# GATB/leon

Hardware: AMD Instinct MI355X
Metric: compressed input MB/s (DNA encode path) (higher is better)
Workload: dtype u64

## Files before the change

### leon_amd/csrc/capi.hip

```cpp
#include "../../include/leon_dna.h"
#include "kernels.h"
#include "host_rc.h"
#include "staging.h"
#include "host_blocks.h"

#include "prim.h"

#include <algorithm>
#include <atomic>
#include <chrono>
#include <cstdio>
#include <cstdlib>
#include <cstring>
#include <functional>
#include <mutex>
#include <string>
#include <thread>
#include <vector>

using namespace leon;

namespace {

thread_local std::string g_create_error;
}
namespace leon { void set_create_error(const std::string& msg) { g_create_error = msg; } }
namespace {

const bool g_trace_alloc = getenv("LEON_TRACE_ALLOC") != nullptr;

struct DevBuf {
    void* p = nullptr;
    size_t cap = 0;
    hipError_t ensure(size_t bytes) {
        if (bytes <= cap) return hipSuccess;
        auto t0 = std::chrono::steady_clock::now();
        if (p) { hipError_t e = hipFree(p); p = nullptr; cap = 0; if (e != hipSuccess) return e; }
        size_t want = bytes + bytes / 8 + 256;
        hipError_t e = hipMalloc(&p, want);
        if (e != hipSuccess) { (void)hipGetLastError(); leon_device_trim(); e = hipMalloc(&p, want); }
        if (e == hipSuccess) cap = want;
        if (g_trace_alloc) {
            const double ms = std::chrono::duration<double, std::milli>(std::chrono::steady_clock::now() - t0).count();
            if (ms >= 1.0) fprintf(stderr, "[leon alloc] %.1f MB in %.1f ms\n", want / 1e6, ms);
        }
        return e;
    }
    void release() { if (p) (void)hipFree(p); p = nullptr; cap = 0; }
    template <typename T> T* as() const { return (T*)p; }
};
struct TmpBuf : DevBuf {
    TmpBuf() = default;
    TmpBuf(const TmpBuf&) = delete;
    TmpBuf& operator=(const TmpBuf&) = delete;
    ~TmpBuf() { release(); }
};

uint64_t splitmix_rv(uint32_t idx) {
    uint64_t s = 0x4C454F4EULL + (uint64_t)(idx + 1) * 0x9E3779B97F4A7C15ULL;
    s = (s ^ (s >> 30)) * 0xBF58476D1CE4E5B9ULL;
    s = (s ^ (s >> 27)) * 0x94D049BB133111EBULL;
    return s ^ (s >> 31);
}
uint64_t hash_seed0() {
    const uint64_t r0 = 0xAAAAAAAA55555555ULL, r3 = 0xB5B5B5B54B4B4B4BULL;
    return r0 * r3;
}

__global__ void k_iota(uint32_t* v, uint64_t n) {
    for (uint64_t i = blockIdx.x * (uint64_t)blockDim.x + threadIdx.x; i < n; i += (uint64_t)gridDim.x * blockDim.x) v[i] = (uint32_t)i;
}

}

inline hipError_t spin_sync(hipStream_t s) {
    static const bool spin = [] { const char* e = getenv("LEON_SPIN_SYNC"); return !(e && e[0] == '0'); }();
    if (!spin) return hipStreamSynchronize(s);
    const auto t0 = std::chrono::steady_clock::now();
    for (uint32_t i = 0;; i++) {
        const hipError_t e = hipStreamQuery(s);
        if (e != hipErrorNotReady) return e;
        for (int k = 0; k < 32; k++) __builtin_ia32_pause();
        if ((i & 255) == 255 && std::chrono::steady_clock::now() - t0 > std::chrono::milliseconds(20)) break;
    }
    (void)hipGetLastError();
    return hipStreamSynchronize(s);
}

struct leon_dna_ctx {
    leon_dna_cfg cfg{};
    int device = 0;
    hipStream_t stream = nullptr;
    uint64_t* h_rb = nullptr;
    std::string err;
    uint8_t* d_bloom = nullptr;
    uint64_t bloom_nchar = 0;
    BloomDev B{};
    uint16_t* d_rv16 = nullptr;
    DictDev D{};
    uint64_t dict_cap = 0;
    uint64_t n_keys = 0;
    unsigned long long* d_nkeys = nullptr;
    uint64_t n_anchors = 0;
    DevBuf anchor_kmers;
    AnchorDictWorker* anchor_worker = nullptr;
    double anchor_wait_ms = 0;
    std::vector<uint8_t> dict_device_out;
    uint64_t next_read = 0, next_block = 0;
    uint32_t shard_rank = 0, shard_world = 1;
    uint32_t xch_mode = LEON_XCH_OFF;
    leon_exchange_fn xch_fn = nullptr; void* xch_user = nullptr;
    leon_gather_fn gather_fn = nullptr; void* gather_user = nullptr;
    DevBuf xch_slot, xch_off, xch_evoff, xch_events, xch_send, xch_split, xch_res;
    DevBuf resolve_trace;
    DevBuf round_hist;
    DevBuf wcache;
    DevBuf chain_cnt, chain_own, chain_ins, chain_rows, chain_ent, chain_trace, chain_dep, chain_xdep, chain_om, chain_late;
    std::vector<hipEvent_t> chain_ev;
    DevBuf hb_recs[2], hb_recoff, hb_state;
    uint64_t* h_recs = nullptr; size_t h_recs_cap = 0;
    hipStream_t copy_stream = nullptr;
    std::vector<hipEvent_t> hb_ev;
    std::vector<HostBlockCoder> hb_coders;
    uint64_t* h_anchor[2] = {nullptr, nullptr}; size_t h_anchor_cap = 0;
    bool partial_seen = false, finished = false;
    uint64_t hdr_next_read = 0, hdr_next_block = 0;
    bool hdr_partial_seen = false;
    DevBuf hdr_first;
    const uint64_t* walk_keys = nullptr;
    uint32_t fbits_log2 = FBITS_LOG2_DEFAULT;
    bool poisoned = false;
    DevBuf in_bases, in_off, slot_off, packed, nmask, rlen, ncount;
    DevBuf status, hit_pos, hit_slot, cand_pos, cand_slot, anchor_pos, anchor_addr, flags, sort_key, ins_flag, rank;
    DevBuf ulist0, ulist1, counters, cub_tmp, sort_key2, perm, perm2, events, prev, sym_off, syms;
    DevBuf blk_begin, out_off, out_size, rc_out, rc_scratch, dst_off, payload, errflag, nerr, wbits, fbits, pbits;
    void* h_payload = nullptr; size_t h_payload_cap = 0;
    uint64_t last_n = 0, last_bases = 0;
    const void* last_d_bases = nullptr; const void* last_d_off = nullptr;
    DevBuf dc_cache;
    DevBuf dc_out, dc_pay, dc_len, dc_pool, dc_scr;
    PathCache dc_pc{};
    uint64_t dc_bloom_fp = 0;
    bool dc_filled = false;
    leon_dna_stats stats{};
    hipEvent_t ev[12]{};
    std::vector<hipEvent_t> pack_ev;
};

namespace {

int fail(leon_dna_ctx* c, int code, const std::string& msg) {
    if (c) c->err = msg; else g_create_error = msg;
    return code;
}
#define HIPCHK(c, call)                                                                         \
    do {                                                                                        \
        hipError_t e_ = (call);                                                                 \
        if (e_ != hipSuccess)                                                                   \
            return fail((c), LEON_E_HIP, std::string(#call) + ": " + hipGetErrorString(e_));    \
    } while (0)

void dict_free(DictDev& D) {
    if (D.slots) (void)hipFree(D.slots);
    if (D.tent && D.tstride == 1) (void)hipFree(D.tent);
    if (D.addr) (void)hipFree(D.addr);
    D = DictDev{};
}
int dict_alloc(leon_dna_ctx* c, DictDev& D, uint64_t cap) {
    const uint32_t W = kmer_words(c->cfg.kmer_size);
    D = DictDev{};
    hipError_t e = hipMalloc((void**)&D.slots, cap * 16 * W);
    if (e == hipSuccess && W == 1) { D.tstride = 1; e = hipMalloc((void**)&D.tent, cap * 8); }
    if (e == hipSuccess) e = hipMalloc((void**)&D.addr, cap * 4);
    if (e != hipSuccess) {
        dict_free(D);
        return fail(c, LEON_E_HIP, std::string("anchor dictionary allocation: ") + hipGetErrorString(e));
    }
    if (W == 2) { D.tent = D.slots + 3; D.tstride = 4; }
    D.mask = cap - 1;
    D.n_keys = c->d_nkeys;
    D.wbits = c->wbits.as<uint32_t>();
    D.fbits = c->fbits.as<uint32_t>();
    D.pbits = c->pbits.as<uint32_t>();
    D.fwshift = 32 - (c->fbits_log2 - 6);
    minimizer_geometry(c->cfg.kmer_size, D.mm_m, D.mm_P, D.mm_c);
    D.err = c->errflag.as<int>() + 2;
    launch_dict_init(c->stream, D, cap, W);
    return LEON_OK;
}
int dict_reserve(leon_dna_ctx* c, uint64_t keys) {
    uint64_t need = 1024;
    while (need < 4 * keys) need <<= 1;
    if (need <= c->dict_cap) return LEON_OK;
    if (need > (1ull << 32)) return fail(c, LEON_E_OVERFLOW, "anchor dictionary would exceed 2^32 slots");
    DictDev nd{};
    HIPCHK(c, hipMemsetAsync(c->d_nkeys, 0, 8, c->stream));
    int rc = dict_alloc(c, nd, need);
    if (rc) return rc;
    if (c->dict_cap) {
        launch_dict_rehash(c->stream, c->D, c->dict_cap, nd, c->cfg.kmer_size);
        HIPCHK(c, hipStreamSynchronize(c->stream));
        dict_free(c->D);
    }
    c->D = nd;
    c->dict_cap = need;
    return LEON_OK;
}

ReadsDev reads_view(leon_dna_ctx* c, const uint64_t* d_off, uint64_t n) {
    ReadsDev R{};
    R.packed = c->packed.as<uint32_t>(); R.nmask = c->nmask.as<uint32_t>(); R.slot_off = c->slot_off.as<uint64_t>();
    R.base_off = d_off; R.len = c->rlen.as<uint32_t>(); R.n_count = c->ncount.as<uint32_t>();
    R.n = n; R.k = c->cfg.kmer_size;
    return R;
}

struct Upload {
    static constexpr uint64_t kPiece = kStagePiece;
    std::atomic<uint64_t> bytes_done{0};
    std::atomic<int> failed{0};
    std::atomic<int> cancel{0};
    std::atomic<uint64_t> next_piece{0};
    std::vector<std::atomic<uint8_t>> piece_done;
    std::mutex mu;
    uint64_t prefix = 0, n_bytes = 0;
    std::vector<std::thread> th;
    explicit Upload(uint64_t bytes) : piece_done((bytes + kPiece - 1) / kPiece), n_bytes(bytes) { for (auto& f : piece_done) f.store(0); }
    void publish(uint64_t piece) {
        piece_done[piece].store(1, std::memory_order_release);
        std::lock_guard<std::mutex> g(mu);
        while (prefix < piece_done.size() && piece_done[prefix].load(std::memory_order_acquire)) prefix++;
        bytes_done.store(std::min(n_bytes, prefix * kPiece), std::memory_order_release);
    }
    ~Upload() { for (auto& t : th) if (t.joinable()) t.join(); }
};
constexpr uint32_t kRbHostChainsErr = 500;
int ensure_cub(leon_dna_ctx* c, size_t bytes) { HIPCHK(c, c->cub_tmp.ensure(bytes)); return LEON_OK; }
template <typename F> int run_prim(leon_dna_ctx* c, F&& call) {
    size_t bytes = 0;
    HIPCHK(c, call(nullptr, bytes));
    if (int rc = ensure_cub(c, bytes)) return rc;
    HIPCHK(c, call(c->cub_tmp.p, bytes));
    return LEON_OK;
}

int ensure_pack_bufs(leon_dna_ctx* c, uint64_t n, uint64_t n_slots) {
    HIPCHK(c, c->packed.ensure((n_slots * 2 + 16) * 4)); HIPCHK(c, c->nmask.ensure((n_slots + 4) * 4));
    HIPCHK(c, c->rlen.ensure(n * 4)); HIPCHK(c, c->ncount.ensure(n * 4));
    return LEON_OK;
}
int ensure_resolve_bufs(leon_dna_ctx* c, uint64_t n, uint64_t W) {
    HIPCHK(c, c->status.ensure(n));
    HIPCHK(c, c->hit_pos.ensure(n * 4)); HIPCHK(c, c->hit_slot.ensure(n * 4));
    HIPCHK(c, c->cand_pos.ensure(n * 4)); HIPCHK(c, c->cand_slot.ensure(n * 4));
    HIPCHK(c, c->anchor_pos.ensure(n * 4)); HIPCHK(c, c->anchor_addr.ensure(n * 4));
    HIPCHK(c, c->flags.ensure(n)); HIPCHK(c, c->sort_key.ensure(n * 8));
    HIPCHK(c, c->ins_flag.ensure(W * 4)); HIPCHK(c, c->rank.ensure(W * 4));
    HIPCHK(c, c->ulist0.ensure(W * 4)); HIPCHK(c, c->ulist1.ensure(W * 4));
    return LEON_OK;
}
int ensure_block_bufs(leon_dna_ctx* c, uint64_t nbl) {
// ... 224 lines not shown
        launch_rc_encode(s, c->syms.as<uint8_t>(), c->blk_begin.as<uint64_t>(), nbl, c->rc_out.as<uint8_t>(), c->out_off.as<uint64_t>(),
                         c->out_size.as<uint64_t>(), c->rc_scratch.as<uint32_t>(), c->errflag.as<int>(), max_block_syms, small_sizes, counts_apart);
        HIPCHK(c, hipGetLastError());
        HIPCHK(c, hipEventRecord(c->ev[7], s));
        int errflag = 0;
        HIPCHK(c, hipMemcpyAsync(out.sizes.data(), c->out_size.p, nbl * 8, hipMemcpyDeviceToHost, s));
        HIPCHK(c, hipMemcpyAsync(&errflag, c->errflag.p, 4, hipMemcpyDeviceToHost, s));
        HIPCHK(c, hipStreamSynchronize(s));
        if (errflag == 3) return fail(c, LEON_E_STATE, "a numeric value's byte count above 8 in the symbol stream (internal error)");
        if (errflag) return fail(c, LEON_E_OVERFLOW, errflag == 2 ? std::string("a ") + unit + " block has 2^32 symbols or more"
                                                                  : std::string("range coder output exceeded its 3 bytes/symbol bound"));
    }
    for (uint64_t b = 0; b < nbl; b++) out.dst[b + 1] = out.dst[b] + out.sizes[b];
    const uint64_t payload_bytes = out.payload_bytes = out.dst[nbl];
    if (!out.host_chains) {
        HIPCHK(c, c->payload.ensure(payload_bytes + 16));
        HIPCHK(c, hipMemcpyAsync(c->dst_off.p, out.dst.data(), (nbl + 1) * 8, hipMemcpyHostToDevice, s));
        launch_gather_payload(s, c->rc_out.as<uint8_t>(), c->out_off.as<uint64_t>(), c->dst_off.as<uint64_t>(), c->out_size.as<uint64_t>(),
                              nbl, c->payload.as<uint8_t>());
        if (int rc = ensure_host_payload(c, payload_bytes + 16, payload_bytes + payload_bytes / 4 + 4096)) return rc;
        HIPCHK(c, hipMemcpyAsync(c->h_payload, c->payload.p, payload_bytes, hipMemcpyDeviceToHost, s));
    }
    HIPCHK(c, hipEventRecord(c->ev[8], s));
    HIPCHK(c, hipStreamSynchronize(s));
    return LEON_OK;
}

int deliver_blocks(leon_dna_ctx* c, const CodedBlocks& out, const Share& sh, uint64_t n, uint64_t first_block, leon_block_sink sink, void* user) {
    const uint64_t rpb = c->cfg.reads_per_block;
    for (uint64_t b = 0; b < sh.nbl; b++) {
        const uint32_t nr = (uint32_t)std::min<uint64_t>(rpb, n - (sh.lb0 + b) * rpb);
        const uint8_t* pay = out.host_chains ? c->hb_coders[b].data() : (const uint8_t*)c->h_payload + out.dst[b];
        if (sink(user, first_block + sh.lb0 + b, pay, out.sizes[b], nr)) {
            c->poisoned = true;
            return fail(c, LEON_E_SINK, "block sink returned non-zero");
        }
    }
    return LEON_OK;
}
}

extern "C" {

int leon_dna_abi_version(void) { return LEON_DNA_ABI_VERSION; }

const char* leon_last_error(const leon_dna_ctx* ctx) { return ctx ? ctx->err.c_str() : g_create_error.c_str(); }

int leon_dna_ctx_create(const leon_dna_cfg* cfg, leon_dna_ctx** out) {
    if (!cfg || !out) return fail(nullptr, LEON_E_INVALID, "null argument");
    *out = nullptr;
    if (cfg->struct_size != sizeof(leon_dna_cfg)) return fail(nullptr, LEON_E_INVALID, "leon_dna_cfg.struct_size mismatch");
    if (cfg->kmer_size < 3 || cfg->kmer_size > 63)
        return fail(nullptr, LEON_E_INVALID, "kmer_size must be in 3..63 (one 64-bit word below 32, two words from 32 to 63)");
    if (cfg->reads_per_block == 0) return fail(nullptr, LEON_E_INVALID, "reads_per_block must be > 0");
    if (cfg->bloom_n_hash < 1 || cfg->bloom_n_hash > 10) return fail(nullptr, LEON_E_INVALID, "bloom_n_hash must be in 1..10");
    if (cfg->bloom_block_nbits < 4 || cfg->bloom_block_nbits > 16)
        return fail(nullptr, LEON_E_INVALID, "bloom_block_nbits must be in 4..16");
    {
        const uint64_t blk0 = 1ull << cfg->bloom_block_nbits;
        uint64_t tai0 = cfg->bloom_tai + 2 * blk0;
        if ((tai0 & (tai0 - 1)) == 0) tai0--;
        if (tai0 <= 2 * blk0 || cfg->bloom_tai > (1ull << 46)) return fail(nullptr, LEON_E_INVALID, "bloom_tai out of range (1 .. 2^46 bits)");
    }
    int ndev = 0;
    if (hipGetDeviceCount(&ndev) != hipSuccess || ndev == 0)
        return fail(nullptr, LEON_E_NO_DEVICE, "no HIP device: the DNA encode path has no CPU fallback");
    if (cfg->device_id < 0 || cfg->device_id >= ndev) return fail(nullptr, LEON_E_INVALID, "device_id out of range");
    leon_dna_ctx* c = new leon_dna_ctx();
    c->cfg = *cfg;
    c->cfg.random_values = nullptr;
    if (c->cfg.resolve_window == 0) c->cfg.resolve_window = 1ull << 21;
    c->device = cfg->device_id;
#define CREATE_CHK(call)                                                                                         \
    do {                                                                                                         \
        hipError_t e_ = (call);                                                                                  \
        if (e_ != hipSuccess) {                                                                                  \
            int r_ = fail(nullptr, LEON_E_HIP, std::string(#call) + ": " + hipGetErrorString(e_));               \
            leon_dna_ctx_destroy(c);                                                                             \
            return r_;                                                                                           \
        }                                                                                                        \
    } while (0)
    CREATE_CHK(hipSetDevice(c->device));
    CREATE_CHK(hipStreamCreateWithFlags(&c->stream, hipStreamNonBlocking));
    CREATE_CHK(hipHostMalloc((void**)&c->h_rb, 4096, hipHostMallocDefault));
    for (auto& e : c->ev) CREATE_CHK(hipEventCreate(&e));
    uint64_t blk = 1ull << cfg->bloom_block_nbits;
    uint64_t tai = cfg->bloom_tai + 2 * blk;
    c->bloom_nchar = 1 + tai / 8;
    if ((tai & (tai - 1)) == 0) tai--;
    uint64_t reduced = tai - 2 * blk;
    CREATE_CHK(hipMalloc((void**)&c->d_bloom, c->bloom_nchar + 16));
    CREATE_CHK(hipMemsetAsync(c->d_bloom, 0, c->bloom_nchar + 16, c->stream));
    uint16_t rv16[256];
    for (uint32_t i = 0; i < 256; i++) rv16[i] = (uint16_t)((cfg->random_values ? cfg->random_values[i] : splitmix_rv(i)) & 0xFFFF);
    CREATE_CHK(hipMalloc((void**)&c->d_rv16, sizeof(rv16)));
    CREATE_CHK(hipMemcpy(c->d_rv16, rv16, sizeof(rv16), hipMemcpyHostToDevice));
    uint32_t k = cfg->kmer_size;
    c->B.bits = c->d_bloom; c->B.reduced_tai = reduced; c->B.mod_magic = ~0ull / reduced; c->B.seed0 = hash_seed0();
    c->B.k = k; c->B.n_hash = cfg->bloom_n_hash; c->B.block_mask = (uint32_t)(blk - 1);
    CREATE_CHK(hipMalloc((void**)&c->d_nkeys, 8));
    CREATE_CHK(hipMemset(c->d_nkeys, 0, 8));
    CREATE_CHK(c->counters.ensure(64));
    CREATE_CHK(c->errflag.ensure(16));
    CREATE_CHK(hipMemsetAsync(c->errflag.p, 0, 16, c->stream));
    CREATE_CHK(c->wbits.ensure((1ull << WBITS_LOG2) / 8));
    CREATE_CHK(c->pbits.ensure((1ull << WBITS_LOG2) / 8));
    if (const char* e = getenv("LEON_FBITS_LOG2")) {
        const int v = atoi(e);
        if (v >= 12 && v <= (int)FBITS_LOG2_MAX) c->fbits_log2 = (uint32_t)v;
    }
    CREATE_CHK(c->fbits.ensure((1ull << c->fbits_log2) / 8));
    CREATE_CHK(hipMemsetAsync(c->fbits.p, 0, (1ull << c->fbits_log2) / 8, c->stream));
    CREATE_CHK(hipStreamSynchronize(c->stream));
#undef CREATE_CHK
    c->anchor_worker = new AnchorDictWorker(cfg->kmer_size);
    *out = c;
    return LEON_OK;
}

void leon_dna_ctx_destroy(leon_dna_ctx* c) {
    if (!c) return;
    delete c->anchor_worker;
    (void)hipSetDevice(c->device);
    if (c->stream) (void)hipStreamSynchronize(c->stream);
    dict_free(c->D);
    DevBuf* bufs[] = { &c->anchor_kmers, &c->in_bases, &c->in_off, &c->slot_off, &c->packed, &c->nmask, &c->rlen, &c->ncount,
                       &c->status, &c->hit_pos, &c->hit_slot, &c->cand_pos, &c->cand_slot, &c->anchor_pos, &c->anchor_addr,
                       &c->flags, &c->sort_key, &c->ins_flag, &c->rank, &c->ulist0, &c->ulist1, &c->counters, &c->cub_tmp,
                       &c->sort_key2, &c->perm, &c->perm2, &c->events, &c->prev, &c->sym_off, &c->syms, &c->blk_begin,
                       &c->out_off, &c->out_size, &c->rc_out, &c->rc_scratch, &c->dst_off, &c->payload, &c->errflag, &c->nerr, &c->wbits, &c->fbits, &c->pbits, &c->hdr_first, &c->dc_cache, &c->dc_out, &c->dc_pay, &c->dc_len, &c->dc_pool, &c->dc_scr,
                       &c->xch_slot, &c->xch_off, &c->xch_evoff, &c->xch_events, &c->xch_send, &c->xch_split, &c->xch_res, &c->round_hist, &c->resolve_trace, &c->hb_recs[0], &c->hb_recs[1], &c->hb_recoff, &c->hb_state };
    for (DevBuf* b : bufs) b->release();
    if (c->d_bloom) (void)hipFree(c->d_bloom);
    if (c->d_rv16) (void)hipFree(c->d_rv16);
    if (c->d_nkeys) (void)hipFree(c->d_nkeys);
    if (c->h_payload) (void)hipHostFree(c->h_payload);
    if (c->h_rb) (void)hipHostFree(c->h_rb);
    for (auto& b : c->h_anchor) if (b) (void)hipHostFree(b);
    if (c->h_recs) (void)hipHostFree(c->h_recs);
    for (auto& e : c->hb_ev) (void)hipEventDestroy(e);
    if (c->copy_stream) (void)hipStreamDestroy(c->copy_stream);
    for (auto& e : c->ev) if (e) (void)hipEventDestroy(e);
    for (auto& e : c->pack_ev) (void)hipEventDestroy(e);
    for (auto& e : c->chain_ev) (void)hipEventDestroy(e);
    if (c->stream) (void)hipStreamDestroy(c->stream);
    delete c;
}

int leon_dna_bloom_nbytes(const leon_dna_ctx* c, uint64_t* n) {
    if (!c || !n) return LEON_E_INVALID;
    *n = c->bloom_nchar;
    return LEON_OK;
}
int leon_dna_bloom_upload(leon_dna_ctx* c, const uint8_t* bits, uint64_t n) {
    if (!c || !bits) return LEON_E_INVALID;
    if (n != c->bloom_nchar) return fail(c, LEON_E_INVALID, "bloom_upload: size differs from leon_dna_bloom_nbytes");
    HIPCHK(c, hipSetDevice(c->device));
    HIPCHK(c, staged_h2d(c->device, c->d_bloom, bits, n));
    return LEON_OK;
}
int leon_dna_bloom_download(leon_dna_ctx* c, uint8_t* bits, uint64_t n) {
    if (!c || !bits) return LEON_E_INVALID;
    if (n != c->bloom_nchar) return fail(c, LEON_E_INVALID, "bloom_download: size differs from leon_dna_bloom_nbytes");
    HIPCHK(c, hipSetDevice(c->device));
    HIPCHK(c, hipStreamSynchronize(c->stream));
    HIPCHK(c, staged_d2h(c->device, bits, c->d_bloom, n));
    return LEON_OK;
}
int leon_dna_bloom_clear(leon_dna_ctx* c) {
    if (!c) return LEON_E_INVALID;
    HIPCHK(c, hipSetDevice(c->device));
    HIPCHK(c, hipMemsetAsync(c->d_bloom, 0, c->bloom_nchar + 16, c->stream));
    HIPCHK(c, hipStreamSynchronize(c->stream));
    return LEON_OK;
}
int leon_dna_bloom_insert_device(leon_dna_ctx* c, const uint64_t* d_kmers, uint64_t n) {
    if (!c || (!d_kmers && n)) return LEON_E_INVALID;
    HIPCHK(c, hipSetDevice(c->device));
    launch_bloom_insert(c->stream, c->B, c->d_rv16, d_kmers, n);
    HIPCHK(c, hipGetLastError());
    HIPCHK(c, hipStreamSynchronize(c->stream));
    return LEON_OK;
}
int leon_dna_bloom_insert(leon_dna_ctx* c, const uint64_t* kmers, uint64_t n) {
    if (!c || (!kmers && n)) return LEON_E_INVALID;
    if (!n) return LEON_OK;
    HIPCHK(c, hipSetDevice(c->device));
    TmpBuf tmp;
    const uint64_t bytes = n * 8 * kmer_words(c->cfg.kmer_size);
    HIPCHK(c, tmp.ensure(bytes));
    HIPCHK(c, hipMemcpy(tmp.p, kmers, bytes, hipMemcpyHostToDevice));
    return leon_dna_bloom_insert_device(c, tmp.as<uint64_t>(), n);
}
int leon_dna_bloom_device_ptr(leon_dna_ctx* c, void** p, uint64_t* n) {
    if (!c || !p || !n) return LEON_E_INVALID;
    *p = c->d_bloom; *n = c->bloom_nchar;
    return LEON_OK;
}
int leon_dna_bloom_upload_device(leon_dna_ctx* c, const uint8_t* d_bits, uint64_t n) {
    if (!c || !d_bits) return LEON_E_INVALID;
    if (n != c->bloom_nchar) return fail(c, LEON_E_INVALID, "bloom_upload_device: size differs from leon_dna_bloom_nbytes");
    HIPCHK(c, hipSetDevice(c->device));
    HIPCHK(c, hipMemcpyAsync(c->d_bloom, d_bits, n, hipMemcpyDeviceToDevice, c->stream));
    HIPCHK(c, hipStreamSynchronize(c->stream));
    return LEON_OK;
}
int leon_dna_bloom_download_device(leon_dna_ctx* c, uint8_t* d_bits, uint64_t n) {
    if (!c || !d_bits) return LEON_E_INVALID;
    if (n != c->bloom_nchar) return fail(c, LEON_E_INVALID, "bloom_download_device: size differs from leon_dna_bloom_nbytes");
    HIPCHK(c, hipSetDevice(c->device));
    HIPCHK(c, hipMemcpyAsync(d_bits, c->d_bloom, n, hipMemcpyDeviceToDevice, c->stream));
    HIPCHK(c, hipStreamSynchronize(c->stream));
    return LEON_OK;
}
static int bloom_query(leon_dna_ctx* c, const uint64_t* kmers, uint64_t n, int mode, uint8_t* out) {
    if (!c || ((!kmers || !out) && n)) return LEON_E_INVALID;
    if (!n) return LEON_OK;
    HIPCHK(c, hipSetDevice(c->device));
    TmpBuf dk, dout;
    const uint64_t bytes = n * 8 * kmer_words(c->cfg.kmer_size);
    HIPCHK(c, dk.ensure(bytes));
    HIPCHK(c, dout.ensure(n));
    HIPCHK(c, hipMemcpy(dk.p, kmers, bytes, hipMemcpyHostToDevice));
    launch_bloom_query(c->stream, c->B, c->d_rv16, dk.as<uint64_t>(), n, mode, dout.as<uint8_t>());
    HIPCHK(c, hipGetLastError());
    HIPCHK(c, hipStreamSynchronize(c->stream));
    HIPCHK(c, hipMemcpy(out, dout.p, n, hipMemcpyDeviceToHost));
    return LEON_OK;
}
int leon_dna_bloom_contains4(leon_dna_ctx* c, const uint64_t* kmers, uint64_t n, int right, uint8_t* out) {
    return bloom_query(c, kmers, n, right ? 2 : 1, out);
}
int leon_dna_bloom_contains(leon_dna_ctx* c, const uint64_t* kmers, uint64_t n, uint8_t* out) {
    return bloom_query(c, kmers, n, 0, out);
}

static uint64_t first_window(uint64_t window) { return std::min<uint64_t>(window, 1ull << 17); }
static uint64_t group_end(uint64_t a, uint64_t n, uint64_t window) {
    if (a == 0) return std::min(n, first_window(window));
    return std::min(n, a + 8 * std::min<uint64_t>(window, 1ull << 20));
}

namespace {

struct EncodeKnobs {
    uint32_t rounds_ahead, rounds_max;
    uint32_t chain_chunk;
    bool xch_lookups, walk_cache;
    long walk_cache_log2, walk_hop_log2;
    bool trace_step, trace_resolve, trace_chain;
};
long env_num(const char* name, long dflt) { const char* e = getenv(name); return e ? atol(e) : dflt; }
EncodeKnobs read_encode_knobs() {
    const char* rounds = getenv("LEON_RESOLVE_ROUNDS");
    const long ahead = env_num("LEON_RESOLVE_ROUNDS", 0), most = rounds && strchr(rounds, ':') ? atol(strchr(rounds, ':') + 1) : 0;
    const long chunk = env_num("LEON_CHAIN_CHUNK", 0), hop = env_num("LEON_WALK_HOP_LOG2", 4);
    EncodeKnobs K{};
    K.rounds_ahead = ahead >= 1 && ahead <= 32 ? (uint32_t)ahead : 3u;
    K.rounds_max = std::max<uint32_t>(K.rounds_ahead, most >= 1 && most <= 62 ? (uint32_t)most : 9u);
    K.chain_chunk = chunk >= 1 && chunk <= (1l << CHAIN_LOG2) ? (uint32_t)chunk : 1u << CHAIN_LOG2;
    K.xch_lookups = env_num("LEON_XCH_LOOKUPS", 1) != 0; K.walk_cache = env_num("LEON_WALK_CACHE", 1) != 0;
    K.walk_cache_log2 = env_num("LEON_WALK_CACHE_LOG2", 0); K.walk_hop_log2 = hop >= 1 && hop <= 8 ? hop : 4;
    K.trace_step = getenv("LEON_TRACE_STEP"); K.trace_resolve = getenv("LEON_TRACE_RESOLVE"); K.trace_chain = getenv("LEON_TRACE_CHAIN");
    return K;
}

struct EncodeBatch {
    leon_dna_ctx* const c;
    const uint8_t* const d_bases; const uint64_t* const d_off; const uint64_t n, first_read_index; const leon_block_sink sink; void* const user;
    Upload* const up; const uint64_t* const up_off;
    const uint64_t* const walk_keys = c->walk_keys;
    const EncodeKnobs knobs = read_encode_knobs();
    const std::chrono::steady_clock::time_point t_enter = std::chrono::steady_clock::now();
    const hipStream_t s = c->stream;
    const uint32_t rpb = c->cfg.reads_per_block, k = c->cfg.kmer_size;
    uint64_t n_blocks = 0, off_first = 0, off_last = 0, n_slots = 0, W = 0, KW = 0;
    ReadsDev R{}; ResolveDev V{};
    uint64_t packed_upto = 0; uint32_t n_pack_ev = 0;
    static constexpr uint32_t kRoundsMore = 2, kHist = 64;
    uint32_t* counters = nullptr; uint32_t* lists[2] = {nullptr, nullptr}; uint32_t* d_hist = nullptr; unsigned long long* d_trace = nullptr;
    size_t scan_tmp = 0;
    struct Pending { int buf = -1; uint64_t n = 0; } pending;
    int anchor_buf = 0; bool share_lookups = false;
    uint32_t hint = 0;
    uint32_t n_chain_ev = 0;
    float lk_call_ms = 0, lk_emul_ms = 0;
    Share sh{}; uint64_t nl_bases = 0; bool by_anchor = false;
    WalkCache wc{nullptr, 0, 28, 0};
    std::vector<uint64_t> slice_at, rank_r0, send_counts, send_at; size_t scan_n = 0;
    void mark(const char* what) const {
        if (knobs.trace_step) fprintf(stderr, "[leon step] %-34s %8.2f ms\n", what, std::chrono::duration<double, std::milli>(std::chrono::steady_clock::now() - t_enter).count());
    }
    float ms(int a, int b) const { float v = 0; (void)hipEventElapsedTime(&v, c->ev[a], c->ev[b]); return v; }
    int start() {
        c->stats = leon_dna_stats{}; c->walk_keys = nullptr;
        HIPCHK(c, hipMemcpyAsync(c->h_rb + 0, d_off, 8, hipMemcpyDeviceToHost, s));
        HIPCHK(c, hipMemcpyAsync(c->h_rb + 1, d_off + n, 8, hipMemcpyDeviceToHost, s));
        HIPCHK(c, spin_sync(s));
        off_first = c->h_rb[0]; off_last = c->h_rb[1];
        if (off_last < off_first) return fail(c, LEON_E_INVALID, "offsets are not monotonic");
        n_blocks = (n + rpb - 1) / rpb;
        HIPCHK(c, hipEventRecord(c->ev[0], s));
        HIPCHK(c, c->slot_off.ensure((n + 1) * 8));
        uint64_t* slot_off = c->slot_off.as<uint64_t>();
        HIPCHK(c, hipMemsetAsync(c->counters.as<uint32_t>() + 4, 0, 4, s));
        launch_read_slots(s, d_off, n, slot_off, c->counters.as<uint32_t>() + 4);
        if (int rc = run_prim(c, [&](void* t, size_t& b) { return prim::ExclusiveSum(t, b, slot_off, slot_off, n + 1, s); })) return rc;
        HIPCHK(c, hipMemcpyAsync(c->h_rb + 0, slot_off + n, 8, hipMemcpyDeviceToHost, s));
        HIPCHK(c, hipMemcpyAsync(c->h_rb + 1, c->counters.as<uint32_t>() + 4, 4, hipMemcpyDeviceToHost, s));
        HIPCHK(c, spin_sync(s));
        n_slots = c->h_rb[0];
        if ((uint32_t)c->h_rb[1]) return fail(c, LEON_E_INVALID, "offsets are not monotonic (or a read is longer than 2^31 bases)");
        mark("offsets checked, slots scanned");
        if (int rc = ensure_pack_bufs(c, n, n_slots)) return rc;
        HIPCHK(c, hipMemsetAsync(c->packed.as<uint32_t>() + n_slots * 2, 0, 64, s));
        if (int rc = pack_next_group()) return rc;
        HIPCHK(c, hipEventRecord(c->ev[1], s));
        R = reads_view(c, d_off, n);
        W = std::min<uint64_t>(c->cfg.resolve_window, n);
        if (int rc = ensure_resolve_bufs(c, n, W)) return rc;
        V.status = c->status.as<uint8_t>(); V.hit_pos = c->hit_pos.as<uint32_t>(); V.hit_slot = c->hit_slot.as<uint32_t>();
        V.cand_pos = c->cand_pos.as<uint32_t>(); V.cand_slot = c->cand_slot.as<uint32_t>();
        V.anchor_pos = c->anchor_pos.as<int32_t>(); V.anchor_addr = c->anchor_addr.as<uint32_t>(); V.flags = c->flags.as<uint8_t>();
        V.sort_key = c->sort_key.as<uint64_t>(); V.ins_flag = c->ins_flag.as<uint32_t>();
        counters = c->counters.as<uint32_t>(); lists[0] = c->ulist0.as<uint32_t>(); lists[1] = c->ulist1.as<uint32_t>();
        HIPCHK(c, prim::ExclusiveSum(nullptr, scan_tmp, V.ins_flag, c->rank.as<uint32_t>(), W, s));
        return ensure_cub(c, scan_tmp);
    }
    int pack_next_group() {
        const uint64_t a = packed_upto, b = group_end(a, n, c->cfg.resolve_window);
        if (up) {
            const uint64_t want = up_off[b];
            if (want < up_off[0] || want > up_off[n] || want < up_off[a]) return fail(c, LEON_E_INVALID, "offsets are not monotonic");
            while (up->bytes_done.load(std::memory_order_acquire) < want - up_off[0] && !up->failed.load()) std::this_thread::yield();
            if (up->failed.load()) return fail(c, LEON_E_HIP, "upload of the read bases failed");
        }
        if (int rc = event_pair(c, c->pack_ev, n_pack_ev)) return rc;
        HIPCHK(c, hipEventRecord(c->pack_ev[2 * n_pack_ev], s));
        launch_pack(s, d_bases, d_off + a, c->slot_off.as<uint64_t>() + a, b - a, c->packed.as<uint32_t>(), c->nmask.as<uint32_t>(),
                    c->rlen.as<uint32_t>() + a, c->ncount.as<uint32_t>() + a);
        HIPCHK(c, hipEventRecord(c->pack_ev[2 * n_pack_ev + 1], s));
        n_pack_ev++;
        packed_upto = b;
        return LEON_OK;
    }
    int resolve() {
        KW = kmer_words(k);
        HIPCHK(c, c->round_hist.ensure(kHist * 4)); d_hist = c->round_hist.as<uint32_t>();
        if (c->h_anchor_cap < W * 8 * KW) {
            for (auto& b : c->h_anchor) { if (b) HIPCHK(c, hipHostFree(b)); b = nullptr; }
            c->h_anchor_cap = 0;
            for (auto& b : c->h_anchor) HIPCHK(c, hipHostMalloc((void**)&b, W * 8 * KW + 64, hipHostMallocDefault));
            c->h_anchor_cap = W * 8 * KW;
        }
        if (knobs.trace_resolve) { HIPCHK(c, c->resolve_trace.ensure(12 * 8)); d_trace = c->resolve_trace.as<unsigned long long>(); HIPCHK(c, hipMemsetAsync(d_trace, 0, 12 * 8, s)); }
        share_lookups = c->shard_world > 1 && knobs.xch_lookups && ((c->xch_mode == LEON_XCH_BY_ANCHOR && c->gather_fn) || c->xch_mode == LEON_XCH_EMULATE);
        hint = (uint32_t)std::min<uint64_t>(W, 1u << 20);
        for (uint64_t w0 = 0, w1 = 0; w0 < n; w0 = w1) {
            w1 = std::min(n, w0 + (w0 == 0 ? first_window(W) : W));
            if (int rc = resolve_window(w0, w1)) return rc;
            while (w1 < n && packed_upto < std::min(n, w1 + W)) { if (int rc = pack_next_group()) return rc; }
            c->stats.resolve_windows++;
        }
        if (pending.buf >= 0) { HIPCHK(c, spin_sync(s)); hand_over(); }
        if (knobs.trace_resolve) {
            unsigned long long t[12];
            HIPCHK(c, hipMemcpy(t, d_trace, sizeof t, hipMemcpyDeviceToHost));
            const char* cls[3] = {"found an anchor of the dictionary", "went on to propose its own", "no anchor at all"};
            for (int j = 0; j < 3; j++)
                if (t[4 * j]) fprintf(stderr, "[leon resolve] k_lookup_cand, reads that %-34s: %10llu reads, per read %.1f filter probes, %.1f dictionary probes behind a filter maybe, %.1f k-mers through the bloom\n",
                                      cls[j], t[4 * j], (double)t[4 * j + 1] / t[4 * j], (double)t[4 * j + 2] / t[4 * j], (double)t[4 * j + 3] / t[4 * j]);
        }
        HIPCHK(c, hipGetLastError());
        HIPCHK(c, hipEventRecord(c->ev[2], s));
        mark("resolution launched to its end");
        return LEON_OK;
    }
    int resolve_window(uint64_t w0, uint64_t w1) {
        if (int rc = dict_reserve(c, c->n_keys + (w1 - w0))) return rc;
        HIPCHK(c, hipMemsetAsync(counters, 0, 8, s));
        HIPCHK(c, hipMemsetAsync(c->wbits.p, 0, (1ull << WBITS_LOG2) / 8, s));
        HIPCHK(c, hipMemsetAsync(c->pbits.p, 0, (1ull << WBITS_LOG2) / 8, s));
        if (!share_lookups) launch_lookup_cand(s, R, c->B, c->d_rv16, c->D, V, w0, w1, first_read_index, lists[0], counters, d_trace);
        else if (int rc = look_up_shared(w0, w1)) return rc;
        HIPCHK(c, hipMemcpyAsync(d_hist, counters, 4, hipMemcpyDeviceToDevice, s));
        uint32_t cnt0 = 0;
        if (int rc = fixpoint_rounds(w0, w1, cnt0)) return rc;
        hint = std::max<uint32_t>(2 * cnt0, 4096);
        if (cnt0 > 0) { if (int rc = settle(w0, w1)) return rc; }
        launch_finalize_reads(s, R, c->D, V, w0, w1);
        return LEON_OK;
    }
    int look_up_shared(uint64_t w0, uint64_t w1) {
        const uint32_t Wn = c->shard_world; const uint64_t P = (w1 - w0 + Wn - 1) / Wn;
        auto run_of = [&](uint32_t r, uint64_t& a, uint64_t& b) { a = std::min(w1, w0 + (uint64_t)r * P); b = std::min(w1, a + P); };
        HIPCHK(c, c->xch_res.ensure((uint64_t)Wn * P * 8)); uint64_t* xres = c->xch_res.as<uint64_t>();
        uint64_t s0 = 0, s1 = 0; run_of(c->shard_rank, s0, s1);
        launch_lookup_cand(s, R, c->B, c->d_rv16, c->D, V, s0, s1, first_read_index, lists[0], counters, d_trace, xres, w0, false);
        HIPCHK(c, hipStreamSynchronize(s));
        const auto t_l0 = std::chrono::steady_clock::now();
        if (c->xch_mode == LEON_XCH_BY_ANCHOR) {
            if (c->gather_fn(c->gather_user, xres, P * 8, Wn)) return fail(c, LEON_E_STATE, "the gather callback returned non-zero");
            HIPCHK(c, hipSetDevice(c->device));
            lk_call_ms += ms_since(t_l0);
        } else {
            for (uint32_t r = 0; r < Wn; r++) {
                if (r == c->shard_rank) continue;
                uint64_t a = 0, b = 0; run_of(r, a, b);
                launch_lookup_cand(s, R, c->B, c->d_rv16, c->D, V, a, b, first_read_index, lists[0], counters, nullptr, xres, w0, true);
            }
            HIPCHK(c, hipStreamSynchronize(s));
            lk_emul_ms += ms_since(t_l0);
        }
        launch_lookup_apply(s, R, c->D, V, w0, w1, s0, s1, first_read_index, xres, lists[0], counters);
        return LEON_OK;
    }
    int fixpoint_rounds(uint64_t w0, uint64_t w1, uint32_t& cnt0) {
        int cur = 0;
        uint32_t n_hist = 1;
        bool first_wait = true;
        for (uint32_t ahead = knobs.rounds_ahead;; ahead = kRoundsMore) {
            for (uint32_t r = 0; r < ahead && n_hist < kHist; r++) {
                const int nxt = cur ^ 1;
                const uint32_t h = std::max<uint32_t>(hint >> (2 * (n_hist - 1) < 31 ? 2 * (n_hist - 1) : 31), 4096);
                HIPCHK(c, hipMemsetAsync(counters + nxt, 0, 4, s));
                launch_check(s, R, c->D, V, first_read_index, lists[cur], counters + cur, h, lists[nxt], counters + nxt);
                HIPCHK(c, hipMemcpyAsync(d_hist + n_hist, counters + nxt, 4, hipMemcpyDeviceToDevice, s));
                launch_reset_tent(s, c->D, V, lists[cur], counters + cur, h);
                launch_propose(s, c->D, V, first_read_index, lists[nxt], counters + nxt, h);
                cur = nxt; n_hist++;
            }
            HIPCHK(c, hipMemcpyAsync(c->h_rb + 8, d_hist, n_hist * 4, hipMemcpyDeviceToHost, s));
            HIPCHK(c, hipMemcpyAsync(c->h_rb + 1, c->D.err, 4, hipMemcpyDeviceToHost, s));
            HIPCHK(c, spin_sync(s));
            if (first_wait) { hand_over(); first_wait = false; }
            if (const int derr = (int)(uint32_t)c->h_rb[1]) {
                HIPCHK(c, hipMemsetAsync(c->D.err, 0, 4, s));
                return fail(c, LEON_E_STATE, derr == 2 ? "the look-ups gathered from the other ranks do not fit this rank's reads or dictionary (were all ranks fed the same batches?)"
                                                       : "anchor dictionary: a two-word key stayed half-written (a stalled wave); batch abandoned");
            }
            const uint32_t* hist = reinterpret_cast<const uint32_t*>(c->h_rb + 8);
            cnt0 = hist[0];
            for (uint32_t r = 1; r < n_hist; r++)
                if (hist[r - 1] > 0 && hist[r] >= hist[r - 1]) return fail(c, LEON_E_STATE, "anchor resolution made no progress (internal error)");
            const uint32_t cnt = hist[n_hist - 1];
            const bool halving = n_hist >= 2 && 2ull * hist[n_hist - 1] <= hist[n_hist - 2];
            if (cnt == 0 || !halving || n_hist - 1 >= knobs.rounds_max || n_hist + kRoundsMore > kHist) {
                for (uint32_t r = 1; r < n_hist; r++) if (hist[r - 1] > 0) c->stats.resolve_rounds++;
                return cnt ? chain_tail(cnt, w0, w1, lists[cur ^ 1]) : LEON_OK;
            }
        }
    }
    int chain_tail(uint32_t left, uint64_t w0, uint64_t w1, uint32_t* clist) {
        if (int rc = event_pair(c, c->chain_ev, n_chain_ev)) return rc;
        HIPCHK(c, hipEventRecord(c->chain_ev[2 * n_chain_ev], s));
        uint32_t* rank = c->rank.as<uint32_t>();
        launch_chain_flags(s, V, w0, w1, V.ins_flag);
        HIPCHK(c, prim::ExclusiveSum(c->cub_tmp.p, scan_tmp, V.ins_flag, rank, w1 - w0, s));
        launch_chain_compact(s, V, w0, w1, rank, clist);
        const uint32_t CH = knobs.chain_chunk;
        unsigned long long* d_ctrace = nullptr;
        if (knobs.trace_chain) { HIPCHK(c, c->chain_trace.ensure(8 * 8)); d_ctrace = c->chain_trace.as<unsigned long long>(); HIPCHK(c, hipMemsetAsync(d_ctrace, 0, 8 * 8, s)); }
        for (uint32_t c0 = 0; c0 < left; c0 += CH) {
            const uint32_t nc = std::min(CH, left - c0), nG = (nc + 63) / 64;
            if (c0) launch_chain_repropose(s, c->D, V, first_read_index, clist + (c0 - CH), left - (c0 - CH), clist + c0, left - c0);
            HIPCHK(c, c->chain_cnt.ensure((uint64_t)nc * 4)); HIPCHK(c, c->chain_own.ensure((uint64_t)nc * 4));
            HIPCHK(c, c->chain_ins.ensure(((uint64_t)nG + 1) * 8)); HIPCHK(c, c->chain_rows.ensure(((uint64_t)nG + 1) * 8));
            HIPCHK(c, c->chain_dep.ensure((uint64_t)nc * 8)); HIPCHK(c, c->chain_xdep.ensure((uint64_t)nc * 8));
            HIPCHK(c, c->chain_om.ensure((uint64_t)nG * 64 * 8)); HIPCHK(c, c->chain_late.ensure((uint64_t)nG * 8));
            uint64_t* rows = c->chain_rows.as<uint64_t>();
            uint32_t* cnt = c->chain_cnt.as<uint32_t>(); uint32_t* own = c->chain_own.as<uint32_t>();
            unsigned long long* om = c->chain_om.as<unsigned long long>(); unsigned long long* late = c->chain_late.as<unsigned long long>();
            unsigned long long* dep = c->chain_dep.as<unsigned long long>(); unsigned long long* xdep = c->chain_xdep.as<unsigned long long>();
            size_t rows_tmp = 0;
            HIPCHK(c, prim::ExclusiveSum(nullptr, rows_tmp, rows, rows, nG + 1, s));
            if (rows_tmp > c->cub_tmp.cap) { HIPCHK(c, hipStreamSynchronize(s)); if (int rc = ensure_cub(c, std::max(rows_tmp, scan_tmp))) return rc; }
            launch_chain_prep(s, false, R, c->D, V, first_read_index, w0, clist + c0, nc, c0, rank, cnt, own, nullptr, nullptr, nullptr, nullptr, nullptr, nullptr);
            launch_chain_tables(s, cnt, own, nc, rows, om, late);
            HIPCHK(c, prim::ExclusiveSum(c->cub_tmp.p, rows_tmp, rows, rows, nG + 1, s));
            HIPCHK(c, hipMemcpyAsync(c->h_rb + 0, rows + nG, 8, hipMemcpyDeviceToHost, s));
            HIPCHK(c, spin_sync(s));
            const uint64_t total_rows = c->h_rb[0];
            HIPCHK(c, c->chain_ent.ensure(std::max<uint64_t>(total_rows, 1) * 64 * 4)); uint32_t* ent = c->chain_ent.as<uint32_t>();
            launch_chain_prep(s, true, R, c->D, V, first_read_index, w0, clist + c0, nc, c0, rank, cnt, own, rows, ent, om, late, dep, xdep);
            if (launch_chain_seq(s, nc, cnt, own, dep, xdep, rows, ent, c->chain_ins.as<unsigned long long>(), d_ctrace))
                return fail(c, LEON_E_HIP, "the sequential resolution pass could not be launched (its LDS request was refused)");
            launch_chain_apply(s, c->D, V, first_read_index, clist + c0, nc, c->chain_ins.as<unsigned long long>(), k);
            HIPCHK(c, hipGetLastError());
        }
        { const uint32_t c_last = (left - 1) / CH * CH; launch_chain_repropose(s, c->D, V, first_read_index, clist + c_last, left - c_last, nullptr, 0); }
        HIPCHK(c, hipEventRecord(c->chain_ev[2 * n_chain_ev + 1], s));
        n_chain_ev++;
        c->stats.resolve_chain_reads += left; c->stats.resolve_chain_windows++;
        if (knobs.trace_chain) {
            unsigned long long t[8];
            HIPCHK(c, hipStreamSynchronize(s));
            HIPCHK(c, hipMemcpy(t, d_ctrace, sizeof t, hipMemcpyDeviceToHost));
            float cms = 0; (void)hipEventElapsedTime(&cms, c->chain_ev[2 * n_chain_ev - 2], c->chain_ev[2 * n_chain_ev - 1]);
            fprintf(stderr, "[leon chain] window [%llu, %llu): %u reads left by the rounds; %llu steps of 64, %.2f ballot iterations and %.1f entry rows per step, %llu inserters; %.2f ms; per step the settler waited %.0f (tester: %.0f), settled + published %.0f ticks of s_memtime\n",
                    (unsigned long long)w0, (unsigned long long)w1, left, t[0], t[0] ? (double)t[1] / t[0] : 0.0, t[0] ? (double)t[2] / t[0] : 0.0, t[3], cms,
                    t[0] ? (double)t[4] / t[0] : 0.0, t[0] ? (double)t[5] / t[0] : 0.0, t[0] ? (double)t[6] / t[0] : 0.0);
        }
        return LEON_OK;
    }
    int settle(uint64_t w0, uint64_t w1) {
        launch_final_pos(s, R, c->D, V, w0, w1, first_read_index);
        launch_ins_flags(s, V, w0, w1);
        HIPCHK(c, prim::ExclusiveSum(c->cub_tmp.p, scan_tmp, V.ins_flag, c->rank.as<uint32_t>(), w1 - w0, s));
        HIPCHK(c, hipMemcpyAsync(c->h_rb + 0, c->rank.as<uint32_t>() + (w1 - w0 - 1), 4, hipMemcpyDeviceToHost, s));
        HIPCHK(c, hipMemcpyAsync(c->h_rb + 1, V.ins_flag + (w1 - w0 - 1), 4, hipMemcpyDeviceToHost, s));
        HIPCHK(c, hipMemcpyAsync(c->h_rb + 2, c->d_nkeys, 8, hipMemcpyDeviceToHost, s));
        HIPCHK(c, spin_sync(s));
        const uint64_t n_new = (uint64_t)(uint32_t)c->h_rb[0] + (uint32_t)c->h_rb[1];
        c->n_keys = c->h_rb[2];
        if (c->n_anchors + n_new > 0xFFFFFFFFull) return fail(c, LEON_E_OVERFLOW, "more than 2^32 anchors");
        if ((c->n_anchors + n_new) * 8 * KW > c->anchor_kmers.cap) {
            TmpBuf nb;
            HIPCHK(c, nb.ensure(std::max<uint64_t>((c->n_anchors + n_new) * 2, 1024) * 8 * KW));
            if (c->n_anchors) HIPCHK(c, hipMemcpyAsync(nb.p, c->anchor_kmers.p, c->n_anchors * 8 * KW, hipMemcpyDeviceToDevice, s));
            HIPCHK(c, hipStreamSynchronize(s));
            std::swap(static_cast<DevBuf&>(nb).p, c->anchor_kmers.p);
            std::swap(static_cast<DevBuf&>(nb).cap, c->anchor_kmers.cap);
        }
        launch_assign_addr(s, c->D, V, w0, w1, c->rank.as<uint32_t>(), c->n_anchors, c->anchor_kmers.as<uint64_t>(), k);
        if (n_new && c->shard_rank == 0 && !(c->cfg.flags & LEON_F_DICT_ON_DEVICE)) {
            HIPCHK(c, hipMemcpyAsync(c->h_anchor[anchor_buf], c->anchor_kmers.as<uint64_t>() + c->n_anchors * KW, n_new * 8 * KW, hipMemcpyDeviceToHost, s));
            pending.buf = anchor_buf; pending.n = n_new;
            anchor_buf ^= 1;
            if (w0 == 0) {
                HIPCHK(c, spin_sync(s));
                hand_over();
                mark("first window's anchors to the chain");
            }
        }
        c->n_anchors += n_new;
        return LEON_OK;
    }
    void hand_over() {
        if (pending.buf < 0) return;
        std::vector<uint64_t> fresh(c->h_anchor[pending.buf], c->h_anchor[pending.buf] + pending.n * KW);
        c->anchor_worker->push(std::move(fresh));
        pending.buf = -1;
    }
    int take_share() {
        sh = share_of(c, n);
        uint64_t off_r0 = off_first, off_r1 = off_last;
        if (c->shard_world > 1) {
            HIPCHK(c, hipMemcpy(&off_r0, d_off + sh.r0, 8, hipMemcpyDeviceToHost));
            HIPCHK(c, hipMemcpy(&off_r1, d_off + sh.r0 + sh.nl, 8, hipMemcpyDeviceToHost));
        }
        nl_bases = off_r1 - off_r0;
        R.ev_origin = sh.r0;
        c->stats.n_reads = sh.nl; c->stats.n_bases = nl_bases; c->stats.n_blocks = sh.nbl; c->stats.n_anchors = c->n_anchors;
        c->last_n = n; c->last_bases = nl_bases; c->last_d_bases = d_bases; c->last_d_off = d_off;
        by_anchor = c->shard_world > 1 && c->xch_mode != LEON_XCH_OFF;
        return LEON_OK;
    }
    int walk() {
        HIPCHK(c, c->events.ensure(nl_bases + 16));
        HIPCHK(c, hipMemsetAsync(c->events.p, 0, nl_bases + 16, s));
        start_walk_cache();
        HIPCHK(c, c->perm.ensure(n * 4));
        hipLaunchKernelGGL(k_iota, dim3((uint32_t)std::min<uint64_t>((n + 255) / 256, 8192)), dim3(256), 0, s, c->perm.as<uint32_t>(), n);
        return by_anchor ? walk_by_anchor() : walk_share();
    }
    void start_walk_cache() {
        uint64_t buckets = knobs.walk_cache ? walk_cache_buckets(c) : 0;
        if (!buckets) return;
        if (knobs.walk_cache_log2 >= 10 && knobs.walk_cache_log2 <= 31) buckets = 1ull << knobs.walk_cache_log2;
        size_t free_b = 0, total_b = 0;
        if (hipMemGetInfo(&free_b, &total_b) == hipSuccess) while (buckets > 1024 && buckets * 64 > c->wcache.cap && buckets * 64 > free_b / 8) buckets >>= 1;
        if (c->wcache.ensure(buckets * 64) != hipSuccess) { (void)hipGetLastError(); return; }
        wc.slots = c->wcache.as<uint64_t>(); wc.bucket_mask = buckets - 1; wc.hop_shift = 32 - knobs.walk_hop_log2;
        launch_walk_cache_init(s, wc, k);
    }
    int walk_share() {
        const uint64_t r0 = sh.r0, nl = sh.nl;
        HIPCHK(c, c->sort_key2.ensure(nl * 8)); HIPCHK(c, c->perm2.ensure(nl * 4));
        const uint64_t* walk_key = walk_keys ? walk_keys + r0 : V.sort_key + r0;
        const unsigned key_bits = walk_keys ? 48u : 33u;
        auto sort = [&](void* t, size_t& b) { return prim::SortPairs(t, b, walk_key, c->sort_key2.as<uint64_t>(), c->perm.as<uint32_t>() + r0, c->perm2.as<uint32_t>(), nl, 0, key_bits, s); };
        if (int rc = run_prim(c, sort)) return rc;
        HIPCHK(c, hipEventRecord(c->ev[3], s));
        HIPCHK(c, hipEventRecord(c->ev[4], s));
        launch_walk(s, R, c->B, c->d_rv16, V.anchor_pos, V.flags, c->perm2.as<uint32_t>(), nl, c->events.as<uint8_t>(), nullptr, wc);
        HIPCHK(c, hipEventRecord(c->ev[5], s));
        c->stats.walk_launches = 1; c->stats.walk_reads = nl;
        return LEON_OK;
    }
    int walk_by_anchor() {
        const uint32_t Wd = c->shard_world, me = c->shard_rank;
        if (Wd + 2 > 4096 / 8) return fail(c, LEON_E_INVALID, "set_exchange: world too large");
        if (int rc = cut_slices()) return rc;
        HIPCHK(c, hipMemsetAsync(c->errflag.as<int>() + 1, 0, 4, s));
        const auto t_x0 = std::chrono::steady_clock::now();
        if (int rc = walk_slice(me, true)) return rc;
        HIPCHK(c, hipStreamSynchronize(s));
        float walk_own = 0; (void)hipEventElapsedTime(&walk_own, c->ev[4], c->ev[5]);
        c->stats.xch_words_sent = send_at[Wd];
        if (c->xch_mode == LEON_XCH_BY_ANCHOR) {
            const uint64_t* d_recv = nullptr; uint64_t recv_total = 0;
            const auto t_call = std::chrono::steady_clock::now();
            if (c->xch_fn(c->xch_user, c->xch_send.as<uint64_t>(), send_counts.data(), Wd, &d_recv, &recv_total))
                return fail(c, LEON_E_STATE, "the exchange callback returned non-zero");
            c->stats.ms_exchange_call = ms_since(t_call);
            if (recv_total && !d_recv) return fail(c, LEON_E_STATE, "the exchange callback returned no buffer");
            c->stats.xch_words_received = recv_total;
            HIPCHK(c, hipSetDevice(c->device));
            launch_ev_scatter(s, d_recv, recv_total, c->events.as<uint8_t>(), nl_bases, c->errflag.as<int>() + 1);
            HIPCHK(c, hipStreamSynchronize(s));
            c->stats.ms_exchange = ms_since(t_x0) - walk_own;
        } else {
            auto keep_own = [&] { launch_ev_scatter(s, c->xch_send.as<uint64_t>() + send_at[me], send_counts[me], c->events.as<uint8_t>(), nl_bases, c->errflag.as<int>() + 1);
                                  c->stats.xch_words_received += send_counts[me]; };
            keep_own();
            HIPCHK(c, hipStreamSynchronize(s));
            c->stats.ms_exchange = ms_since(t_x0) - walk_own;
            const auto t_e0 = std::chrono::steady_clock::now();
            for (uint32_t sl = 0; sl < Wd; sl++) {
                if (sl == me) continue;
                if (int rc = walk_slice(sl, false)) return rc;
                keep_own();
            }
            HIPCHK(c, hipStreamSynchronize(s));
            c->stats.ms_emulated = ms_since(t_e0);
        }
        c->stats.ms_exchange_call += lk_call_ms; c->stats.ms_exchange += lk_call_ms; c->stats.ms_gather_call = lk_call_ms;
        c->stats.ms_emulated += lk_emul_ms; c->stats.ms_emulated_lookups = lk_emul_ms;
        HIPCHK(c, hipEventRecord(c->ev[9], s));
        int xerr = 0;
        HIPCHK(c, hipMemcpy(&xerr, c->errflag.as<int>() + 1, 4, hipMemcpyDeviceToHost));
        if (xerr) return fail(c, LEON_E_STATE, "the exchange delivered a word that lies outside this rank's blocks");
        return LEON_OK;
    }
    int cut_slices() {
        const uint32_t Wd = c->shard_world;
        HIPCHK(c, c->sort_key2.ensure(n * 8)); HIPCHK(c, c->perm2.ensure(n * 4));
        auto sort = [&](void* t, size_t& b) { return prim::SortPairs(t, b, V.sort_key, c->sort_key2.as<uint64_t>(), c->perm.as<uint32_t>(), c->perm2.as<uint32_t>(), n, 0, 33, s); };
        if (int rc = run_prim(c, sort)) return rc;
        unsigned long long* d_cnt = reinterpret_cast<unsigned long long*>(c->counters.as<uint32_t>() + 10);
        launch_lower_bound(s, c->sort_key2.as<uint64_t>(), n, 1ull << 32, d_cnt);
        HIPCHK(c, hipMemcpyAsync(c->h_rb + 0, d_cnt, 8, hipMemcpyDeviceToHost, s));
        HIPCHK(c, spin_sync(s));
        const uint64_t n_anch = c->h_rb[0];
        HIPCHK(c, c->xch_slot.ensure(n * 4)); HIPCHK(c, c->xch_off.ensure((n + 1) * 8));
        HIPCHK(c, prim::ExclusiveSum(nullptr, scan_n, c->xch_off.as<uint64_t>(), c->xch_off.as<uint64_t>(), n + 1, s));
        if (int rc = ensure_cub(c, scan_n)) return rc;
        HIPCHK(c, c->xch_split.ensure((Wd + 1) * 8));
        launch_slice_weights(s, c->sort_key2.as<uint64_t>(), n_anch, c->xch_off.as<uint64_t>());
        HIPCHK(c, prim::ExclusiveSum(c->cub_tmp.p, scan_n, c->xch_off.as<uint64_t>(), c->xch_off.as<uint64_t>(), n_anch + 1, s));
        launch_slice_splits(s, c->xch_off.as<uint64_t>(), n_anch, Wd, c->xch_split.as<unsigned long long>());
        HIPCHK(c, hipMemcpyAsync(c->h_rb + 0, c->xch_split.p, (Wd + 1) * 8, hipMemcpyDeviceToHost, s));
        HIPCHK(c, hipEventRecord(c->ev[3], s));
        HIPCHK(c, spin_sync(s));
        slice_at.assign(c->h_rb, c->h_rb + Wd + 1);
        rank_r0.resize(Wd + 1);
        for (uint32_t d = 0; d <= Wd; d++) rank_r0[d] = std::min<uint64_t>(n, block_start(n_blocks, d, Wd) * rpb);
        send_counts.assign(Wd, 0);
        send_at.assign(Wd + 1, 0);
        return LEON_OK;
    }
    int walk_slice(uint32_t sl, bool timed) {
        const uint32_t Wd = c->shard_world;
        const uint64_t s0 = slice_at[sl], s1 = slice_at[sl + 1], ns = s1 - s0;
        const uint32_t* slice = c->perm2.as<uint32_t>() + s0;
        HIPCHK(c, c->xch_evoff.ensure((ns + 1) * 8));
        uint64_t* evoff = c->xch_evoff.as<uint64_t>();
        HIPCHK(c, hipMemsetAsync(c->xch_slot.p, 0xFF, n * 4, s));
        launch_slice_reads(s, R, slice, ns, evoff, c->xch_slot.as<uint32_t>());
        if (int rc = run_prim(c, [&](void* t, size_t& b) { return prim::ExclusiveSum(t, b, evoff, evoff, ns + 1, s); })) return rc;
        HIPCHK(c, hipMemcpyAsync(c->h_rb + 0, evoff + ns, 8, hipMemcpyDeviceToHost, s));
        HIPCHK(c, spin_sync(s));
        const uint64_t slice_bases = c->h_rb[0];
        HIPCHK(c, c->xch_events.ensure(slice_bases + 16));
        HIPCHK(c, hipMemsetAsync(c->xch_events.p, 0, slice_bases + 16, s));
        if (timed) HIPCHK(c, hipEventRecord(c->ev[4], s));
        launch_walk(s, R, c->B, c->d_rv16, V.anchor_pos, V.flags, slice, ns, c->xch_events.as<uint8_t>(), evoff, wc);
        if (timed) { HIPCHK(c, hipEventRecord(c->ev[5], s)); c->stats.walk_launches = 1; c->stats.walk_reads = ns; }
        launch_ev_words(s, R, c->xch_slot.as<uint32_t>(), evoff, c->xch_events.as<uint8_t>(), n, rpb, n_blocks, Wd, c->xch_off.as<uint64_t>(), nullptr);
        HIPCHK(c, prim::ExclusiveSum(c->cub_tmp.p, scan_n, c->xch_off.as<uint64_t>(), c->xch_off.as<uint64_t>(), n + 1, s));
        for (uint32_t d = 0; d <= Wd; d++) HIPCHK(c, hipMemcpyAsync(c->h_rb + 1 + d, c->xch_off.as<uint64_t>() + rank_r0[d], 8, hipMemcpyDeviceToHost, s));
        HIPCHK(c, spin_sync(s));
        for (uint32_t d = 0; d <= Wd; d++) send_at[d] = c->h_rb[1 + d];
        for (uint32_t d = 0; d < Wd; d++) send_counts[d] = send_at[d + 1] - send_at[d];
        HIPCHK(c, c->xch_send.ensure(send_at[Wd] * 8 + 64));
        launch_ev_words(s, R, c->xch_slot.as<uint32_t>(), evoff, c->xch_events.as<uint8_t>(), n, rpb, n_blocks, Wd, c->xch_off.as<uint64_t>(),
                        c->xch_send.as<uint64_t>());
        HIPCHK(c, hipGetLastError());
        return LEON_OK;
    }
    int code(CodedBlocks& out) {
        HIPCHK(c, c->prev.ensure(n * 8));
        HIPCHK(c, c->nerr.ensure(sh.nl * 8));
        launch_prev_anchored(s, V.anchor_pos, n, rpb, sh.lb0, sh.nbl, c->prev.as<int64_t>());
        auto symbols = [&](uint8_t* syms) {
            launch_symbols(s, R, V.anchor_pos, V.anchor_addr, V.flags, c->prev.as<int64_t>(), c->events.as<uint8_t>(), sh.r0, sh.nl,
                           c->sym_off.as<uint64_t>(), c->nerr.as<uint32_t>(), syms);
        };
        return code_blocks(c, sh, symbols, SMALL_SIZES_DNA, true, "read", out);
    }
    int finish(int last_ev, const CodedBlocks* out = nullptr) {
        leon_dna_stats& st = c->stats;
        const float pack2 = pairs_ms(c->pack_ev, 1, n_pack_ev);
        st.ms_pack = ms(0, 1) + pack2; st.ms_resolve = ms(1, 2) - pack2; st.ms_resolve_chain = pairs_ms(c->chain_ev, 0, n_chain_ev);
        if (last_ev >= 5) { st.ms_sort = ms(2, 3); st.ms_walk = ms(4, 5); }
        if (out) {
            st.n_symbols = out->n_syms; st.payload_bytes = out->payload_bytes;
            st.ms_symbols = by_anchor ? ms(9, 6) : ms(5, 6); st.ms_rangecoder = ms(6, 7); st.ms_d2h = ms(7, 8);
        }
        st.ms_total = ms(0, last_ev);
        if (out) { if (int rc = deliver_blocks(c, *out, sh, n, c->next_block, sink, user)) return rc; }
        c->next_read += n;
        c->next_block += n_blocks;
        if (n % rpb) c->partial_seen = true;
        c->poisoned = false;
        return LEON_OK;
    }
};


}

static int encode_batch_impl(leon_dna_ctx* c, const uint8_t* d_bases, const uint64_t* d_off, uint64_t n,
                             uint64_t first_read_index, leon_block_sink sink, void* user, Upload* up, const uint64_t* up_off) {
    if (!c) return LEON_E_INVALID;
    if (c->finished) return fail(c, LEON_E_STATE, "encode_batch after finish");
    if (first_read_index != c->next_read) return fail(c, LEON_E_STATE, "first_read_index does not continue the stream");
    if (c->partial_seen && n) return fail(c, LEON_E_STATE, "a batch with a partial block must be the last one");
    if (n == 0) return LEON_OK;
    if (!d_bases || !d_off || !sink) return fail(c, LEON_E_INVALID, "null argument");
    if (n > 0xFFFFFFF0ull) return fail(c, LEON_E_INVALID, "more than 2^32 reads in one batch");
    HIPCHK(c, hipSetDevice(c->device));
    EncodeBatch B{c, d_bases, d_off, n, first_read_index, sink, user, up, up_off};
    if (int rc = B.start()) return rc;
    c->poisoned = true;
    if (int rc = B.resolve()) return rc;
    if (int rc = B.take_share()) return rc;
    if (B.sh.nl == 0 && !(B.by_anchor && c->xch_mode == LEON_XCH_BY_ANCHOR)) {
        HIPCHK(c, hipStreamSynchronize(c->stream));
        return B.finish(2);
    }
    if (int rc = B.walk()) return rc;
    if (B.sh.nl == 0) return B.finish(5);
    CodedBlocks out;
    if (int rc = B.code(out)) return rc;
    return B.finish(8, &out);
}

static int encode_batch_guarded(leon_dna_ctx* c, const uint8_t* d_bases, const uint64_t* d_off, uint64_t n,
                                uint64_t first_read_index, leon_block_sink sink, void* user, Upload* up, const uint64_t* up_off = nullptr) {
    if (!c) return LEON_E_INVALID;
    if (c->poisoned) return fail(c, LEON_E_STATE, "an earlier batch failed part-way: the stream is unusable until leon_dna_reset_stream");
    if (c->dc_pc.slots) {
        (void)hipStreamSynchronize(c->stream);
        c->dc_cache.release(); c->dc_pc = PathCache{}; c->dc_filled = false;
    }
    for (DevBuf* b : { &c->dc_out, &c->dc_pay, &c->dc_len, &c->dc_pool, &c->dc_scr }) b->release();
    const int rc = encode_batch_impl(c, d_bases, d_off, n, first_read_index, sink, user, up, up_off);
    if (rc != LEON_OK && c->poisoned) c->err += kPoisonedNote;
    return rc;
}

int leon_dna_encode_batch_device(leon_dna_ctx* c, const uint8_t* d_bases, const uint64_t* d_off, uint64_t n,
                                 uint64_t first_read_index, leon_block_sink sink, void* user) {
    return encode_batch_guarded(c, d_bases, d_off, n, first_read_index, sink, user, nullptr);
}

int leon_dna_encode_batch(leon_dna_ctx* c, const uint8_t* bases, const uint64_t* off, uint64_t n, uint64_t first_read_index,
                          leon_block_sink sink, void* user) {
    if (!c) return LEON_E_INVALID;
    if (n == 0) return leon_dna_encode_batch_device(c, nullptr, nullptr, 0, first_read_index, sink, user);
    if (!bases || !off) return fail(c, LEON_E_INVALID, "null argument");
    if (off[n] < off[0]) return fail(c, LEON_E_INVALID, "offsets are not monotonic");
    HIPCHK(c, hipSetDevice(c->device));
    const uint64_t nb = off[n] - off[0];
    HIPCHK(c, c->in_bases.ensure(nb + 64));
    HIPCHK(c, c->in_off.ensure((n + 1) * 8));
    HIPCHK(c, staged_h2d(c->device, c->in_off.p, off, (n + 1) * 8));
    if (off[0]) {
        launch_rebase_offsets(c->stream, c->in_off.as<uint64_t>(), n + 1, off[0]);
        HIPCHK(c, hipStreamSynchronize(c->stream));
    }
    Upload up(nb);
    const int dev = c->device;
    uint8_t* dst = c->in_bases.as<uint8_t>();
    const uint8_t* src = bases + off[0];
    const uint32_t n_workers = (uint32_t)std::max<uint64_t>(1, std::min<uint64_t>(stage_threads(), up.piece_done.size()));
    for (uint32_t w = 0; w < n_workers; w++)
        up.th.emplace_back([&up, dev, dst, src, nb] {
            StageLane L(dev);
            uint64_t held[2] = {~0ull, ~0ull};
            bool ok = L.ok;
            for (uint32_t turn = 0; ok && !up.cancel.load(); turn ^= 1) {
                if (held[turn] != ~0ull) {
                    if (hipEventSynchronize(L.ev[turn]) != hipSuccess) { ok = false; break; }
                    up.publish(held[turn]); held[turn] = ~0ull;
                }
                const uint64_t piece = up.next_piece.fetch_add(1);
                if (piece >= up.piece_done.size()) break;
                const uint64_t a = piece * Upload::kPiece, m = std::min<uint64_t>(Upload::kPiece, nb - a);
                memcpy(L.buf[turn], src + a, m);
                if (hipMemcpyAsync(dst + a, L.buf[turn], m, hipMemcpyHostToDevice, L.st) != hipSuccess || hipEventRecord(L.ev[turn], L.st) != hipSuccess) { ok = false; break; }
                held[turn] = piece;
            }
            for (int t = 0; t < 2 && ok; t++)
                if (held[t] != ~0ull) { if (hipEventSynchronize(L.ev[t]) != hipSuccess) ok = false; else up.publish(held[t]); }
            if (!ok && !up.cancel.load()) up.failed.store(1);
        });
    static const bool trace_up = getenv("LEON_TRACE_UPLOAD") != nullptr;
    const auto t_up0 = std::chrono::steady_clock::now();
    std::thread watcher;
    if (trace_up) watcher = std::thread([&up, nb, t_up0] {
        while (up.bytes_done.load() < nb && !up.failed.load() && !up.cancel.load()) std::this_thread::sleep_for(std::chrono::milliseconds(1));
        const double ms = std::chrono::duration<double, std::milli>(std::chrono::steady_clock::now() - t_up0).count();
        fprintf(stderr, "[leon upload] %.1f MB in %.1f ms = %.1f GB/s\n", nb / 1e6, ms, nb / 1e6 / ms);
    });
    const int rc = encode_batch_guarded(c, dst, c->in_off.as<uint64_t>(), n, first_read_index, sink, user, &up, off);
    if (rc != LEON_OK) up.cancel.store(1);
    for (auto& t : up.th) t.join();
    if (watcher.joinable()) watcher.join();
    return rc;
}


int leon_dna_reserve(leon_dna_ctx* c, uint64_t max_reads, uint64_t max_bases) {
    if (!c) return LEON_E_INVALID;
    if (max_reads == 0) return LEON_OK;
    if (max_reads > 0xFFFFFFF0ull) return fail(c, LEON_E_INVALID, "more than 2^32 reads in one batch");
    HIPCHK(c, hipSetDevice(c->device));
// ... 178 lines not shown
                const uint64_t begin[2] = { 0, nsym }, off[2] = { 0, ((3 * nsym + 7) & ~7ull) + 64 };
                HIPCHK(c, dout.ensure(off[1] + 64)); HIPCHK(c, dscr.ensure(rc_model_scratch_bytes(1)));
                HIPCHK(c, hipMemcpy(dbegin.p, begin, 16, hipMemcpyHostToDevice));
                HIPCHK(c, hipMemcpy(doff.p, off, 16, hipMemcpyHostToDevice));
                launch_anchor_symbols(s, c->anchor_kmers.as<uint64_t>(), c->n_anchors, c->cfg.kmer_size, dsyms.as<uint8_t>());
                HIPCHK(c, hipMemsetAsync(c->errflag.p, 0, 4, s));
                launch_rc_encode(s, dsyms.as<uint8_t>(), dbegin.as<uint64_t>(), 1, dout.as<uint8_t>(), doff.as<uint64_t>(), dsize.as<uint64_t>(),
                                 dscr.as<uint32_t>(), c->errflag.as<int>(), nsym);
                HIPCHK(c, hipGetLastError());
                HIPCHK(c, hipStreamSynchronize(s));
                uint64_t sz = 0; int errflag = 0;
                HIPCHK(c, hipMemcpy(&sz, dsize.p, 8, hipMemcpyDeviceToHost));
                HIPCHK(c, hipMemcpy(&errflag, c->errflag.p, 4, hipMemcpyDeviceToHost));
                if (errflag) return fail(c, LEON_E_OVERFLOW, "dictionary stream: device range coder bound hit");
                c->dict_device_out.resize(sz);
                if (sz) HIPCHK(c, hipMemcpy(c->dict_device_out.data(), dout.p, sz, hipMemcpyDeviceToHost));
            }
            c->finished = true;
        }
        c->anchor_wait_ms = std::chrono::duration<double, std::milli>(std::chrono::steady_clock::now() - t0).count();
        *payload = c->dict_device_out.data();
        *size = c->dict_device_out.size();
        *n_anchors = c->n_anchors;
        return LEON_OK;
    }
    c->anchor_worker->drain();
    c->anchor_wait_ms = std::chrono::duration<double, std::milli>(std::chrono::steady_clock::now() - t0).count();
    if (getenv("LEON_TRACE_STEP")) fprintf(stderr, "[leon step] dictionary chain busy %.1f ms, of which %.1f ms waiting for its helpers' records\n",
                                           c->anchor_worker->busy_ms(), c->anchor_worker->starved_ms());
    if (!c->finished) {
        if (c->shard_rank == 0) c->anchor_worker->coder().flush();
        c->finished = true;
    }
    *payload = c->anchor_worker->coder().data();
    *size = c->shard_rank == 0 ? c->anchor_worker->coder().size() : 0;
    *n_anchors = c->n_anchors;
    return LEON_OK;
}

int leon_dna_debug_walk_order(leon_dna_ctx* c, const uint64_t* d_keys) {
    if (!c) return LEON_E_INVALID;
    c->walk_keys = d_keys;
    return LEON_OK;
}

int leon_dna_set_shard(leon_dna_ctx* c, uint32_t rank, uint32_t world) {
    if (!c) return LEON_E_INVALID;
    if (world == 0 || rank >= world) return fail(c, LEON_E_INVALID, "set_shard: need rank < world");
    if (c->next_read) return fail(c, LEON_E_STATE, "set_shard must precede the first batch of a stream");
    c->shard_rank = rank; c->shard_world = world;
    return LEON_OK;
}

int leon_dna_set_exchange(leon_dna_ctx* c, uint32_t mode, leon_exchange_fn fn, void* user) {
    if (!c) return LEON_E_INVALID;
    if (mode > LEON_XCH_EMULATE) return fail(c, LEON_E_INVALID, "set_exchange: unknown mode");
    if (mode == LEON_XCH_BY_ANCHOR && !fn) return fail(c, LEON_E_INVALID, "set_exchange: LEON_XCH_BY_ANCHOR needs the exchange callback");
    if (c->next_read) return fail(c, LEON_E_STATE, "set_exchange must precede the first batch of a stream");
    c->xch_mode = mode; c->xch_fn = fn; c->xch_user = user;
    return LEON_OK;
}

int leon_dna_set_gather(leon_dna_ctx* c, leon_gather_fn fn, void* user) {
    if (!c) return LEON_E_INVALID;
    if (c->next_read) return fail(c, LEON_E_STATE, "set_gather must precede the first batch of a stream");
    c->gather_fn = fn; c->gather_user = user;
    return LEON_OK;
}

int leon_dna_reset_stream(leon_dna_ctx* c) {
    if (!c) return LEON_E_INVALID;
    static const bool trace_step = getenv("LEON_TRACE_STEP") != nullptr;
    const auto t_enter = std::chrono::steady_clock::now();
    struct Done { bool on; std::chrono::steady_clock::time_point t0; ~Done() { if (on) fprintf(stderr, "[leon step] %-34s %8.2f ms\n", "reset_stream", std::chrono::duration<double, std::milli>(std::chrono::steady_clock::now() - t0).count()); } } done{trace_step, t_enter};
    c->anchor_worker->reset();
    HIPCHK(c, hipSetDevice(c->device));
    HIPCHK(c, spin_sync(c->stream));
    HIPCHK(c, hipMemsetAsync(c->fbits.p, 0, (1ull << c->fbits_log2) / 8, c->stream));
    if (c->dict_cap) {
        HIPCHK(c, hipMemsetAsync(c->d_nkeys, 0, 8, c->stream));
        launch_dict_init(c->stream, c->D, c->dict_cap, kmer_words(c->cfg.kmer_size));
        HIPCHK(c, spin_sync(c->stream));
    }
    c->n_keys = 0; c->n_anchors = 0;
    c->next_read = 0; c->next_block = 0; c->partial_seen = false; c->finished = false; c->poisoned = false;
    c->hdr_next_read = 0; c->hdr_next_block = 0; c->hdr_partial_seen = false;
    c->last_n = 0; c->last_bases = 0; c->last_d_bases = c->last_d_off = nullptr;
    return LEON_OK;
}

int leon_dna_get_stats(const leon_dna_ctx* c, leon_dna_stats* out) {
    if (!c || !out) return LEON_E_INVALID;
    *out = c->stats;
    out->n_anchors = c->n_anchors;
    out->ms_anchor_wait = (float)c->anchor_wait_ms;
    out->ms_chain_busy = c->finished ? (float)c->anchor_worker->busy_ms() : 0.f;
    return LEON_OK;
}

int leon_host_anchor_dict_decode(const uint8_t* payload, uint64_t size, uint64_t n_anchors, uint32_t k, uint64_t* out) {
    if ((!payload && size) || (!out && n_anchors)) return fail(nullptr, LEON_E_INVALID, "null argument");
    if (k < 3 || k > 63) return fail(nullptr, LEON_E_INVALID, "kmer_size must be in 3..63");
    if (!decode_anchor_dict(payload, size, n_anchors, k, out)) return fail(nullptr, LEON_E_INVALID, "anchor dictionary stream does not decode");
    return LEON_OK;
}

static int decode_blocks_impl(leon_dna_ctx* c, const uint64_t* anchors, uint64_t n_anchors, const uint8_t* payloads,
                              const uint64_t* payload_off, const uint32_t* block_n_reads, const uint64_t* block_n_bases,
                              uint64_t n_blocks, uint8_t* out_bases, uint64_t out_cap, uint32_t* out_len, uint8_t* d_user_bases,
                              uint32_t* d_user_len) {
    if (!c) return LEON_E_INVALID;
    if (n_blocks == 0) return LEON_OK;
    const bool to_device = d_user_bases != nullptr;
    if (!payloads || !payload_off || !block_n_reads || !block_n_bases || (!to_device && (!out_bases || !out_len)) || (to_device && !d_user_len) ||
        (!anchors && n_anchors))
        return fail(c, LEON_E_INVALID, "null argument");
    HIPCHK(c, hipSetDevice(c->device));
    hipStream_t s = c->stream;
    static const bool trace = getenv("LEON_TRACE_DECODE") != nullptr;
    auto t_prev = std::chrono::steady_clock::now();
    auto lap = [&](const char* what) {
        if (!trace) return;
        (void)hipStreamSynchronize(s);
        const auto now = std::chrono::steady_clock::now();
        fprintf(stderr, "[leon decode] %-28s %8.1f ms\n", what, std::chrono::duration<double, std::milli>(now - t_prev).count());
        t_prev = now;
    };
    const uint32_t W = kmer_words(c->cfg.kmer_size);
    std::vector<uint64_t> read0(n_blocks + 1, 0), out0(n_blocks + 1, 0);
    for (uint64_t b = 0; b < n_blocks; b++) {
        if (payload_off[b + 1] < payload_off[b]) return fail(c, LEON_E_INVALID, "payload offsets are not monotonic");
        read0[b + 1] = read0[b] + block_n_reads[b];
        out0[b + 1] = out0[b] + block_n_bases[b];
        if (out0[b + 1] < out0[b] || out0[b + 1] > out_cap) return fail(c, LEON_E_INVALID, "output capacity below the sum of block_n_bases");
    }
    if (out0[n_blocks] > out_cap) return fail(c, LEON_E_INVALID, "output capacity below the sum of block_n_bases");
    const uint64_t pay_bytes = payload_off[n_blocks] - payload_off[0];
    TmpBuf d_anchors, d_off, d_nreads, d_read0, d_out0, d_err;
    DevBuf &d_pay = c->dc_pay, &d_out = c->dc_out, &d_len = c->dc_len, &d_scr = c->dc_scr, &d_pool = c->dc_pool;
    HIPCHK(c, d_anchors.ensure(std::max<uint64_t>(n_anchors * W, 1) * 8));
    HIPCHK(c, d_pay.ensure(pay_bytes + 1024));
    HIPCHK(c, d_off.ensure((n_blocks + 1) * 8)); HIPCHK(c, d_nreads.ensure(n_blocks * 4));
    HIPCHK(c, d_read0.ensure((n_blocks + 1) * 8)); HIPCHK(c, d_out0.ensure((n_blocks + 1) * 8));
    HIPCHK(c, d_out.ensure(out0[n_blocks] + 64)); HIPCHK(c, d_len.ensure(std::max<uint64_t>(read0[n_blocks], 1) * 4));
    HIPCHK(c, d_scr.ensure(decode_scratch_bytes(n_blocks))); HIPCHK(c, d_err.ensure(256));
    const uint64_t pool_words = std::min<uint64_t>(std::max<uint64_t>(out0[n_blocks] / 2, 1ull << 20), 1ull << 28);
    HIPCHK(c, d_pool.ensure(pool_words * 4 + 16));
    lap("buffers");
    bool cache_is_new = false;
    {
        uint64_t want_buckets = std::max<uint64_t>(c->cfg.bloom_tai / 12 * (W == 2 ? 2 : 1), 1024);
        size_t free_b = 0, total_b = 0;
        HIPCHK(c, hipMemGetInfo(&free_b, &total_b));
        uint64_t budget = (uint64_t)(free_b + c->dc_cache.cap) * 2 / 5;
        if (const char* e = getenv("LEON_DC_CACHE_MB")) budget = (uint64_t)std::max<long long>(0, atoll(e)) << 20;
        uint64_t buckets = 1024;
        while (buckets < want_buckets) buckets <<= 1;
        while (buckets > 1024 && buckets * 64 > budget) buckets >>= 1;
        if (buckets * 64 > budget) buckets = 0;
        uint64_t* d_fp = d_err.as<uint64_t>() + 1;
        HIPCHK(c, hipMemsetAsync(d_fp, 0, 8, s));
        launch_bloom_fingerprint(s, c->d_bloom, c->bloom_nchar, d_fp);
        uint64_t fp = 0;
        HIPCHK(c, hipMemcpyAsync(&fp, d_fp, 8, hipMemcpyDeviceToHost, s));
        HIPCHK(c, hipStreamSynchronize(s));
        if (!buckets) { c->dc_cache.release(); c->dc_pc = PathCache{}; c->dc_filled = false; }
        else if (!c->dc_pc.slots || c->dc_pc.bucket_mask != buckets - 1 || !c->dc_filled || fp != c->dc_bloom_fp) {
// ... 619 lines not shown
```

### leon_amd/csrc/dna_kernels.hip

```cpp
#include "kernels.h"

namespace leon {

static inline uint32_t grid_for(uint64_t items, uint32_t per_block, uint32_t cap = 256 * 32) {
    uint64_t g = (items + per_block - 1) / per_block;
    if (g < 1) g = 1;
    if (g > cap) g = cap;
    return (uint32_t)g;
}
#define DISPATCH_K(k, CALL) do { if ((k) >= 32) { typedef u128 K; CALL; } else { typedef uint64_t K; CALL; } } while (0)

template <typename K>
__global__ void __launch_bounds__(256) k_bloom_insert(BloomDev B, const uint16_t* rv16g, const uint64_t* kmers, uint64_t n) {
    __shared__ uint16_t rv16[256];
    load_rv16(rv16, rv16g);
    uint32_t* words = (uint32_t*)B.bits;
    for (uint64_t i = blockIdx.x * (uint64_t)blockDim.x + threadIdx.x; i < n; i += (uint64_t)gridDim.x * blockDim.x) {
        BloomKeys Kk;
        const uint32_t pv = bloom_item_keys<K>(B, rv16, load_kmer<K>(kmers + i * KT<K>::W), Kk);
        for (uint32_t h = 0; h < B.n_hash; h++) {
            uint64_t pos = Kk.racine + Kk.key[h] + pv;
            atomicOr(&words[pos >> 5], 1u << (pos & 31));
        }
    }
// ... 29 lines not shown
        slots[i] = (len + 31) / 32;
    }
}
__global__ void k_rebase_offsets(uint64_t* off, uint64_t n, uint64_t base) {
    for (uint64_t i = blockIdx.x * (uint64_t)blockDim.x + threadIdx.x; i < n; i += (uint64_t)gridDim.x * blockDim.x) off[i] -= base;
}
void launch_rebase_offsets(hipStream_t s, uint64_t* off, uint64_t n, uint64_t base) {
    hipLaunchKernelGGL(k_rebase_offsets, dim3(grid_for(n, 256)), dim3(256), 0, s, off, n, base);
}
void launch_read_slots(hipStream_t s, const uint64_t* off, uint64_t n, uint64_t* slots, uint32_t* bad) {
    hipLaunchKernelGGL(k_read_slots, dim3(grid_for(n + 1, 256)), dim3(256), 0, s, off, n, slots, bad);
}

constexpr uint32_t PACK_READS = 256;
constexpr uint32_t PACK_MAP = 4096;
__global__ void __launch_bounds__(256) k_pack(const uint8_t* bases, const uint64_t* off, const uint64_t* slot_off, uint64_t n,
                                             uint32_t* packed, uint32_t* nmask, uint32_t* len_out, uint32_t* ncount) {
    __shared__ uint64_t so[PACK_READS + 1], bo[PACK_READS + 1];
    __shared__ uint32_t nn[PACK_READS];
    __shared__ uint8_t rmap[PACK_MAP];
    const uint64_t r0 = blockIdx.x * (uint64_t)PACK_READS;
    const uint32_t nr = (uint32_t)(n - r0 < PACK_READS ? n - r0 : PACK_READS);
    for (uint32_t t = threadIdx.x; t <= nr; t += blockDim.x) { so[t] = slot_off[r0 + t]; bo[t] = off[r0 + t]; }
    for (uint32_t t = threadIdx.x; t < PACK_READS; t += blockDim.x) nn[t] = 0;
    __syncthreads();
    const uint64_t s0 = so[0];
    const uint64_t total_dw = 2 * (so[nr] - s0);
    const bool mapped = so[nr] - s0 <= PACK_MAP;
    if (mapped) {
        for (uint32_t t = threadIdx.x; t < nr; t += blockDim.x) for (uint64_t q = so[t]; q < so[t + 1]; q++) rmap[q - s0] = (uint8_t)t;
        __syncthreads();
    }
    uint16_t* nmask16 = (uint16_t*)nmask;
    for (uint64_t d = threadIdx.x; d < total_dw; d += blockDim.x) {
        const uint64_t slot = s0 + (d >> 1);
        uint32_t lo = 0, hi = nr;
        if (mapped) lo = rmap[d >> 1];
        else while (hi - lo > 1) { const uint32_t mid = (lo + hi) >> 1; if (so[mid] <= slot) lo = mid; else hi = mid; }
        const uint32_t r = lo;
        const uint32_t len = (uint32_t)(bo[r + 1] - bo[r]);
        const uint32_t j0 = (uint32_t)(2 * s0 + d - 2 * so[r]) * 16;
        const uint8_t* src = bases + bo[r];
        uint32_t fours[4] = {0x41414141u, 0x41414141u, 0x41414141u, 0x41414141u};
        if (j0 + 16 <= len) __builtin_memcpy(fours, src + j0, 16);
        else {
#pragma unroll
            for (uint32_t q4 = 0; q4 < 4; q4++) {
                const uint32_t p0 = j0 + 4 * q4;
                uint32_t four = 0x41414141u;
                if (p0 + 4 <= len) __builtin_memcpy(&four, src + p0, 4);
                else if (p0 < len) { for (uint32_t j = 0; p0 + j < len; j++) four = (four & ~(0xFFu << (8 * j))) | ((uint32_t)src[p0 + j] << (8 * j)); }
                fours[q4] = four;
            }
        }
        uint32_t word = 0, nb = 0;
#pragma unroll
        for (uint32_t q4 = 0; q4 < 4; q4++) {
            const uint32_t four = fours[q4];
            auto eq = [&](uint32_t letter) { const uint32_t x = four ^ (letter * 0x01010101u); return ~(((x & 0x7F7F7F7Fu) + 0x7F7F7F7Fu) | x) & 0x80808080u; };
            const uint32_t ok = (eq('A') | eq('C') | eq('G') | eq('T')) >> 7;
            const uint32_t codes = (four >> 1) & 0x03030303u & (ok * 3u);
            word |= ((codes * 0x40100401u) >> 24) << (24 - 8 * q4);
            nb |= (((ok ^ 0x01010101u) * 0x01020408u) >> 24) << (4 * q4);
        }
        packed[2 * s0 + d] = word;
        nmask16[2 * s0 + d] = (uint16_t)nb;
        if (nb) atomicAdd(&nn[r], (uint32_t)__popc(nb));
    }
    __syncthreads();
    for (uint32_t t = threadIdx.x; t < nr; t += blockDim.x) { len_out[r0 + t] = (uint32_t)(bo[t + 1] - bo[t]); ncount[r0 + t] = nn[t]; }
}
void launch_pack(hipStream_t s, const uint8_t* bases, const uint64_t* off, const uint64_t* slot_off, uint64_t n,
                 uint32_t* packed, uint32_t* nmask, uint32_t* len, uint32_t* ncount) {
    if (!n) return;
    hipLaunchKernelGGL(k_pack, dim3((uint32_t)((n + PACK_READS - 1) / PACK_READS)), dim3(256), 0, s, bases, off, slot_off, n, packed, nmask, len, ncount);
}


template <typename K> struct DS;
template <> struct DS<uint64_t> { static constexpr uint32_t STRIDE = 2, CLAIM = 0, FIN = 1; };
template <> struct DS<u128> { static constexpr uint32_t STRIDE = 4, CLAIM = 1, FIN = 2; };
template <typename K> __device__ inline uint64_t* slot_ptr(const DictDev& D, uint64_t slot) { return D.slots + slot * DS<K>::STRIDE; }
template <typename K> __device__ inline uint64_t* fin_ptr(const DictDev& D, uint64_t slot) { return slot_ptr<K>(D, slot) + DS<K>::FIN; }
__device__ inline uint64_t* tent_ptr(const DictDev& D, uint64_t slot) { return D.tent + slot * D.tstride; }

__global__ void k_dict_init(DictDev D, uint64_t cap, uint32_t W) {
    for (uint64_t i = blockIdx.x * (uint64_t)blockDim.x + threadIdx.x; i < cap; i += (uint64_t)gridDim.x * blockDim.x) {
        if (W == 2) { D.slots[4 * i] = KEY_EMPTY; D.slots[4 * i + 1] = KEY_EMPTY; D.slots[4 * i + 2] = IDX_INF; D.slots[4 * i + 3] = IDX_INF; }
        else { D.slots[2 * i] = KEY_EMPTY; D.slots[2 * i + 1] = IDX_INF; D.tent[i] = IDX_INF; }
        D.addr[i] = 0;
    }
}
void launch_dict_init(hipStream_t s, DictDev D, uint64_t cap, uint32_t W) {
    hipLaunchKernelGGL(k_dict_init, dim3(grid_for(cap, 256)), dim3(256), 0, s, D, cap, W);
}

__device__ inline uint32_t dict_find(const DictDev& D, uint64_t key, uint64_t& fin) {
    uint64_t slot = key_hash(key) & D.mask;
    for (;;) {
        const ulonglong2 v = *(const ulonglong2*)(D.slots + 2 * slot);
        if (v.x == key) { fin = v.y; return (uint32_t)slot; }
        if (v.x == KEY_EMPTY) return 0xFFFFFFFFu;
        slot = (slot + 1) & D.mask;
    }
}
__device__ inline uint32_t dict_find(const DictDev& D, u128 key, uint64_t& fin) {
    const uint64_t klo = (uint64_t)key, khi = (uint64_t)(key >> 64);
    uint64_t slot = key_hash(key) & D.mask;
    for (;;) {
        const ulonglong2 v = *(const ulonglong2*)(D.slots + 4 * slot);
        if (v.y == KEY_EMPTY) return 0xFFFFFFFFu;
        if (v.y == khi && v.x == klo) { fin = D.slots[4 * slot + 2]; return (uint32_t)slot; }
        slot = (slot + 1) & D.mask;
    }
}
__device__ inline uint32_t fold32(uint64_t x) { return (uint32_t)x ^ (uint32_t)(x >> 32); }
__device__ inline uint32_t fold32(u128 x) { return fold32((uint64_t)x) ^ (fold32((uint64_t)(x >> 64)) * 0x85EBCA6Bu); }
template <typename K> __device__ inline uint32_t window_bit(K key) { return ((fold32(key) ^ 0x5bd1e995u) * 0xCC9E2D51u) >> (32 - WBITS_LOG2); }
__device__ inline uint32_t mmer_hash(uint32_t x, uint32_t m) {
    const uint32_t y = rev2bit32(x) >> (32 - 2 * m);
    const uint32_t h = (y < x ? y : x) * 0x9E3779B1u;
    return h ^ (h >> 15);
}
template <typename K> __device__ inline uint32_t mmer_of(K km, uint32_t k, uint32_t m, uint32_t t) {
    const uint32_t x = (uint32_t)(km >> (2 * (k - m - t)));
    return m == 16 ? x : x & ((1u << (2 * m)) - 1u);
}
__device__ inline uint32_t filter_word(const DictDev& D, uint32_t hmin) { return (hmin * 0x85EBCA6Bu) >> D.fwshift; }
template <typename K> __device__ inline uint64_t filter_bits(K key) {
    const uint32_t h = fold32(key) * 0x9E3779B1u;
    return (1ull << (h >> 26)) | (1ull << ((h >> 20) & 63u));
}
template <typename K> __device__ inline uint32_t key_minimizer_wave(const DictDev& D, K key, uint32_t k, uint32_t lane) {
    uint32_t h = 0xFFFFFFFFu;
    if (lane < D.mm_P) h = mmer_hash(mmer_of(key, k, D.mm_m, D.mm_c + lane), D.mm_m);
    for (int d = 1; d < 32; d <<= 1) { const uint32_t o = (uint32_t)__shfl_xor((int)h, d); h = o < h ? o : h; }
    return h;
}
struct MinLevels { uint32_t L0, L1, L2, L3, L4; };
#define LEON_ROW_SHR(x, n) ((uint32_t)__builtin_amdgcn_update_dpp((int)0xFFFFFFFF, (int)(x), 0x110 + (n), 0xF, 0xF, false))
#define LEON_ROW_SHL(x, n) ((uint32_t)__builtin_amdgcn_update_dpp((int)0xFFFFFFFF, (int)(x), 0x100 + (n), 0xF, 0xF, false))
__device__ inline uint32_t umin3(uint32_t a, uint32_t b, uint32_t c) { const uint32_t t = a < b ? a : b; return t < c ? t : c; }
__device__ inline MinLevels sliding_levels(uint32_t L0, const MinLevels& prev) {
    MinLevels c;
    c.L0 = L0;
    c.L1 = umin3(c.L0, LEON_ROW_SHR(c.L0, 1), LEON_ROW_SHL(prev.L0, 15));
    c.L2 = umin3(c.L1, LEON_ROW_SHR(c.L1, 2), LEON_ROW_SHL(prev.L1, 14));
    c.L3 = umin3(c.L2, LEON_ROW_SHR(c.L2, 4), LEON_ROW_SHL(prev.L2, 12));
    c.L4 = umin3(c.L3, LEON_ROW_SHR(c.L3, 8), LEON_ROW_SHL(prev.L3, 8));
    return c;
}
__device__ inline uint32_t window_minimum(const MinLevels& c, const MinLevels& prev, uint32_t P) {
    return P == 32 ? (c.L4 < prev.L4 ? c.L4 : prev.L4) : P == 16 ? c.L4 : P == 8 ? c.L3 : P == 4 ? c.L2 : P == 2 ? c.L1 : c.L0;
}
template <bool SPIN> __device__ inline uint32_t dict_find_or_insert(const DictDev& D, uint64_t key, bool& created) {
    uint64_t slot = key_hash(key) & D.mask;
    for (;;) {
        uint64_t* pk = D.slots + 2 * slot;
        uint64_t cur = *pk;
        if (cur == key) return (uint32_t)slot;
        if (cur == KEY_EMPTY) {
            uint64_t old = atomicCAS((unsigned long long*)pk, (unsigned long long)KEY_EMPTY, (unsigned long long)key);
            if (old == KEY_EMPTY) { created = true; return (uint32_t)slot; }
            if (old == key) return (uint32_t)slot;
        }
        slot = (slot + 1) & D.mask;
    }
}
template <bool SPIN> __device__ inline uint32_t dict_find_or_insert(const DictDev& D, u128 key, bool& created) {
    const uint64_t klo = (uint64_t)key, khi = (uint64_t)(key >> 64);
    uint64_t slot = key_hash(key) & D.mask;
    for (;;) {
        uint64_t* plo = D.slots + 4 * slot;
        uint64_t* phi = plo + 1;
        uint64_t hi = __hip_atomic_load(phi, __ATOMIC_RELAXED, __HIP_MEMORY_SCOPE_AGENT);
        if (hi == KEY_EMPTY) {
            hi = atomicCAS((unsigned long long*)phi, (unsigned long long)KEY_EMPTY, (unsigned long long)KEY_LOCKED);
            if (hi == KEY_EMPTY) {
                (void)__hip_atomic_exchange(plo, klo, __ATOMIC_RELAXED, __HIP_MEMORY_SCOPE_AGENT);
                (void)__hip_atomic_exchange(phi, khi, __ATOMIC_RELAXED, __HIP_MEMORY_SCOPE_AGENT);
                created = true;
                return (uint32_t)slot;
            }
        }
        if (SPIN) {
            uint32_t spin = 0;
            for (; hi == KEY_LOCKED && spin < (1u << 22); spin++) {
                __builtin_amdgcn_s_sleep(1);
                hi = __hip_atomic_load(phi, __ATOMIC_RELAXED, __HIP_MEMORY_SCOPE_AGENT);
            }
            if (hi == KEY_LOCKED) { atomicExch(D.err, 1); return (uint32_t)slot; }
        }
        if (hi == khi) {
            uint64_t lo = __hip_atomic_load(plo, __ATOMIC_RELAXED, __HIP_MEMORY_SCOPE_AGENT);
            if (SPIN && lo == KEY_EMPTY && klo != KEY_EMPTY) {
                for (uint32_t spin = 0; lo == KEY_EMPTY && spin < (1u << 16); spin++) {
                    __builtin_amdgcn_s_sleep(1);
                    lo = __hip_atomic_load(plo, __ATOMIC_RELAXED, __HIP_MEMORY_SCOPE_AGENT);
                }
                if (lo == KEY_EMPTY) { atomicExch(D.err, 1); return (uint32_t)slot; }
            }
            if (lo == klo) return (uint32_t)slot;
        }
        slot = (slot + 1) & D.mask;
    }
}
template <typename K> __device__ inline K dict_key(const DictDev& D, uint32_t slot);
template <> __device__ inline uint64_t dict_key<uint64_t>(const DictDev& D, uint32_t slot) { return D.slots[2 * (uint64_t)slot]; }
template <> __device__ inline u128 dict_key<u128>(const DictDev& D, uint32_t slot) { return ((u128)D.slots[4 * (uint64_t)slot + 1] << 64) | D.slots[4 * (uint64_t)slot]; }

template <typename K> __global__ void k_dict_rehash(DictDev from, uint64_t from_cap, DictDev to) {
    const uint64_t stride = (uint64_t)gridDim.x * blockDim.x;
    for (uint64_t i0 = blockIdx.x * (uint64_t)blockDim.x; i0 < from_cap; i0 += stride) {
        const uint64_t i = i0 + threadIdx.x;
        bool created = false;
        if (i < from_cap && from.slots[i * DS<K>::STRIDE + DS<K>::CLAIM] != KEY_EMPTY) {
            uint32_t s = dict_find_or_insert<false>(to, dict_key<K>(from, (uint32_t)i), created);
            *fin_ptr<K>(to, s) = *fin_ptr<K>(from, i); *tent_ptr(to, s) = IDX_INF; to.addr[s] = from.addr[i];
        }
        const unsigned long long cm = __ballot(created);
        if (cm && lane_id() == (uint32_t)__builtin_ctzll(cm)) atomicAdd(to.n_keys, (unsigned long long)__popcll(cm));
    }
}
void launch_dict_rehash(hipStream_t s, DictDev from, uint64_t from_cap, DictDev to, uint32_t k) {
    DISPATCH_K(k, hipLaunchKernelGGL(k_dict_rehash<K>, dim3(grid_for(from_cap, 256)), dim3(256), 0, s, from, from_cap, to));
}

template <typename K> __device__ inline K canon_at(const uint32_t* pk, uint32_t p, uint32_t k) {
    const K km = kmer_at<K>(pk, p, k);
    const K rc = revcomp(km, k);
    return rc < km ? rc : km;
}

template <typename K> __device__ inline K fwd_from_words16(uint32_t words, uint32_t gbase, uint32_t base, uint32_t p, uint32_t k);
template <> __device__ inline uint64_t fwd_from_words16<uint64_t>(uint32_t words, uint32_t gbase, uint32_t base, uint32_t p, uint32_t k) {
    const int d = (int)(gbase + (p >> 4) - (base >> 4));
    return kmer_from3((uint32_t)__shfl((int)words, d), (uint32_t)__shfl((int)words, d + 1), (uint32_t)__shfl((int)words, d + 2), p & 15, k);
}
template <> __device__ inline u128 fwd_from_words16<u128>(uint32_t words, uint32_t gbase, uint32_t base, uint32_t p, uint32_t k) {
    const int d = (int)(gbase + (p >> 4) - (base >> 4));
    return kmer_from5((uint32_t)__shfl((int)words, d), (uint32_t)__shfl((int)words, d + 1), (uint32_t)__shfl((int)words, d + 2),
                      (uint32_t)__shfl((int)words, d + 3), (uint32_t)__shfl((int)words, d + 4), p & 15, k);
}
template <typename K> __device__ inline K canon_from_words16(uint32_t words, uint32_t gbase, uint32_t base, uint32_t p, uint32_t k) {
    const K km = fwd_from_words16<K>(words, gbase, base, p, k);
    const K rc = revcomp(km, k);
    return rc < km ? rc : km;
}

template <typename K, bool TRACE>
__global__ void __launch_bounds__(256, (KT<K>::W == 2 ? 5 : 8)) k_lookup_cand(ReadsDev R, BloomDev B, const uint16_t* rv16g, DictDev D, ResolveDev V,
                                                    uint64_t w0, uint64_t w1, uint64_t first_global,
                                                    uint32_t* ulist, uint32_t* ucount, unsigned long long* trace,
                                                    uint64_t* xres, uint64_t xbase, uint32_t dry) {
    __shared__ uint16_t rv16[256];
    load_rv16(rv16, rv16g);
    const uint32_t lane = lane_id(), k = R.k;
    const uint32_t grp = lane >> 4, l = lane & 15, gbase = grp * 16;
    const uint64_t wave = (blockIdx.x * (uint64_t)blockDim.x + threadIdx.x) >> 6;
    const uint64_t nwaves = ((uint64_t)gridDim.x * blockDim.x) >> 6;
    enum : uint32_t { PH_LOOKUP = 0, PH_SEG_A = 1, PH_SEG_B = 2, PH_SEG_C = 3, PH_DONE = 4 };
    __shared__ uint32_t lists[4][64];
    uint32_t* my_list = lists[threadIdx.x >> 6];
    uint32_t n_list = 0, n_created = 0;
    auto flush_list = [&]() {
        if (n_list) {
            uint32_t at = 0;
            if (lane == 0) at = atomicAdd(ucount, n_list);
            at = (uint32_t)__shfl((int)at, 0);
            __builtin_amdgcn_wave_barrier();
            if (lane < n_list) ulist[at + lane] = my_list[lane];
            __builtin_amdgcn_wave_barrier();
        }
        if (n_created && lane == 0) atomicAdd(D.n_keys, (unsigned long long)n_created);
        n_list = 0; n_created = 0;
    };
    uint32_t t_filter = 0, t_dict = 0, t_bloom = 0;
    unsigned long long tr[12] = {0, 0, 0, 0, 0, 0, 0, 0, 0, 0, 0, 0};
    auto trace_done = [&](uint32_t cls) { if (TRACE && l == 0) { tr[cls * 4] += 1; tr[cls * 4 + 1] += t_filter; tr[cls * 4 + 2] += t_dict; tr[cls * 4 + 3] += t_bloom; } t_filter = t_dict = t_bloom = 0; };
    uint64_t i = w0 + 4 * wave + grp;
    bool have = false, started = false, exhausted = false;
    uint32_t len = 0, nk = 0, iMin = 0, iMax = 0, phase = PH_DONE, base = 0, limit = 0;
    uint64_t g = 0;
    const uint32_t* pk = R.packed;
    const uint32_t mm_m = D.mm_m, mm_P = D.mm_P, mm_c = D.mm_c;
    const uint64_t* const fwords = (const uint64_t*)D.fbits;
    MinLevels prev = {~0u, ~0u, ~0u, ~0u, ~0u};
    for (;;) {
        if (phase == PH_DONE && !exhausted) {
            if (started) i += 4 * nwaves;
            started = true;
            have = i < w1;
            exhausted = !have;
            if (have) {
                len = R.len[i];
                g = first_global + i;
                pk = R.packed + 2 * R.slot_off[i];
                nk = len >= k ? len - k + 1 : 0;
                iMin = nk / 2; iMax = nk / 2 + 10 > nk ? nk : nk / 2 + 10;
                base = 0; limit = nk;
                if (nk) phase = PH_LOOKUP;
                else { if (l == 0) { if (!dry) V.status[i] = ST_NOANCHOR; if (xres) xres[i - xbase] = ST_NOANCHOR; } trace_done(2); }
            }
        }
        if (!__any(have)) break;
        {
            const bool active = phase != PH_DONE;
            if (active && base >= limit) {
                if (phase == PH_LOOKUP) { phase = PH_SEG_A; base = iMin; limit = iMax; }
                else if (phase == PH_SEG_A) { phase = PH_SEG_B; base = 0; limit = iMin; }
                else if (phase == PH_SEG_B) { phase = PH_SEG_C; base = iMax; limit = nk; }
                else { phase = PH_DONE; if (l == 0) { if (!dry) V.status[i] = ST_NOANCHOR; if (xres) xres[i - xbase] = ST_NOANCHOR; } trace_done(2); }
            }
            const bool run = phase != PH_DONE && base < limit;
            const uint32_t p = base + l;
            const bool valid = run && p < limit;
            const uint32_t words = (run && l < 8) ? pk[(base >> 4) + l] : 0u;
            const K km = fwd_from_words16<K>(words, gbase, base, valid ? p : (run ? limit - 1 : 0), k);
            const K rck = revcomp(km, k);
            const K cn = rck < km ? rck : km;
            const bool look = run && phase == PH_LOOKUP;
            if (look && base == 0) {
                prev = MinLevels{~0u, ~0u, ~0u, ~0u, ~0u};
                for (int r = mm_P == 32 ? 1 : 0; r >= 0; r--) {
                    const int x = (int)(mm_c + mm_P - 1) - 16 * (r + 1) + (int)l;
                    const uint32_t xc = x > 0 ? (uint32_t)x : 0u;
                    const uint32_t w0 = (uint32_t)__shfl((int)words, (int)(gbase + (xc >> 4))), w1 = (uint32_t)__shfl((int)words, (int)(gbase + (xc >> 4) + 1));
                    const uint32_t mm = (uint32_t)((((((uint64_t)w0) << 32) | w1) << (2 * (xc & 15))) >> (64 - 2 * mm_m));
                    prev = sliding_levels(x >= (int)mm_c && xc + mm_m <= len ? mmer_hash(mm, mm_m) : ~0u, prev);
                }
            }
            const MinLevels cur = sliding_levels(look && valid ? mmer_hash(mmer_of(km, k, mm_m, mm_c + mm_P - 1), mm_m) : ~0u, prev);
            const uint32_t hmin = window_minimum(cur, prev, mm_P);
            if (look) prev = cur;
            bool hit = false; uint32_t slot = 0xFFFFFFFFu;
            if (valid) {
                if (phase == PH_LOOKUP) {
                    const uint64_t fb = filter_bits(cn);
                    const bool maybe = (fwords[filter_word(D, hmin)] & fb) == fb;
                    if (maybe) { uint64_t fin = IDX_INF; slot = dict_find(D, cn, fin); hit = slot != 0xFFFFFFFFu && fin < g; }
                    if (TRACE) {
                        const uint32_t nf = (uint32_t)__popcll(__ballot(true) >> gbase & 0xFFFFull), nd = (uint32_t)__popcll(__ballot(maybe) >> gbase & 0xFFFFull);
                        t_filter += nf; t_dict += nd;
                    }
                }
                else { hit = bloom_contains<K>(B, rv16, cn); if (TRACE) t_bloom += (uint32_t)__popcll(__ballot(true) >> gbase & 0xFFFFull); }
            }
            const unsigned long long bal = __ballot(hit);
            const uint32_t gb = (uint32_t)(bal >> gbase) & 0xFFFFu;
            bool want_insert = false; uint32_t cpos = 0;
            if (run) {
                if (gb) {
                    const uint32_t f = (uint32_t)__builtin_ctz(gb);
                    const uint32_t hs = __shfl(slot, (int)(gbase + f));
                    if (phase == PH_LOOKUP) {
                        if (l == 0) {
                            if (!dry) { V.status[i] = ST_HIT; V.hit_pos[i] = base + f; V.hit_slot[i] = hs; }
                            if (xres) xres[i - xbase] = ((uint64_t)(base + f) << 8) | ST_HIT;
                        }
                        trace_done(0);
                    } else {
                        want_insert = (l == 0) && !dry; cpos = base + f;
                        if (l == 0 && xres) xres[i - xbase] = ((uint64_t)cpos << 8) | ST_UNRESOLVED;
                        trace_done(1);
                    }
                    phase = PH_DONE;
                } else base += 16;
            }
            bool created = false;
            uint32_t sl = 0;
            for (uint32_t q = 0; q < 4; q++) {
                if (want_insert && grp == q) {
                    const K ck = canon_at<K>(pk, cpos, k);
                    sl = dict_find_or_insert<true>(D, ck, created);
                    atomicMin((unsigned long long*)tent_ptr(D, sl), (unsigned long long)g);
                    const uint32_t pb = window_bit(ck);
                    atomicOr(&D.pbits[pb >> 5], 1u << (pb & 31));
                    V.status[i] = ST_UNRESOLVED; V.cand_pos[i] = cpos; V.cand_slot[i] = sl;
                }
            }
            const unsigned long long wm = __ballot(want_insert);
            if (wm) {
                if (want_insert) my_list[n_list + (uint32_t)__popcll(wm & ((1ull << lane) - 1))] = (uint32_t)i;
                n_list += (uint32_t)__popcll(wm);
                n_created += (uint32_t)__popcll(__ballot(created));
                if (n_list > 64 - 4) flush_list();
            }
        }
    }
    flush_list();
    if (TRACE) {
        for (uint32_t j = 0; j < 12; j++) {
            unsigned long long v = tr[j];
            for (int d = 1; d < 64; d <<= 1) v += __shfl_xor(v, d);
            if (lane == 0 && v) atomicAdd(trace + j, v);
        }
    }
}
void launch_lookup_cand(hipStream_t s, ReadsDev R, BloomDev B, const uint16_t* rv16, DictDev D, ResolveDev V,
                        uint64_t w0, uint64_t w1, uint64_t first_global, uint32_t* ulist, uint32_t* ucount, unsigned long long* trace,
                        uint64_t* xres, uint64_t xbase, bool dry) {
    if (w1 <= w0) return;
    if (trace && !dry) { DISPATCH_K(R.k, hipLaunchKernelGGL((k_lookup_cand<K, true>), dim3(grid_for(w1 - w0, 16, 256 * 16)), dim3(256), 0, s, R, B, rv16, D, V, w0, w1,
                                                           first_global, ulist, ucount, trace, xres, xbase, 0u)); return; }
    const uint32_t per_cu = [] { const char* e = getenv("LEON_LOOKUP_BLOCKS_PER_CU"); const int v = e ? atoi(e) : 0; return v > 0 && v <= 1024 ? (uint32_t)v : 16u; }();
    DISPATCH_K(R.k, hipLaunchKernelGGL((k_lookup_cand<K, false>), dim3(grid_for(w1 - w0, 16, 256 * per_cu)), dim3(256), 0, s, R, B, rv16, D, V, w0, w1,
                                       first_global, ulist, ucount, trace, xres, xbase, dry ? 1u : 0u));
}

template <typename K>
__global__ void __launch_bounds__(256) k_lookup_apply(ReadsDev R, DictDev D, ResolveDev V, uint64_t w0, uint64_t w1, uint64_t s0, uint64_t s1,
                                                     uint64_t first_global, const uint64_t* xres, uint32_t* ulist, uint32_t* ucount) {
    __shared__ uint32_t wave_n[4], wave_new[4], block_at;
    const uint32_t lane = lane_id(), wv = threadIdx.x >> 6, k = R.k;
    const uint64_t before = s0 - w0, n_out = (w1 - w0) - (s1 - s0);
    for (uint64_t e0 = blockIdx.x * (uint64_t)blockDim.x; e0 < n_out; e0 += (uint64_t)gridDim.x * blockDim.x) {
        const uint64_t e = e0 + threadIdx.x;
        const bool have = e < n_out;
        const uint64_t i = !have ? w0 : (e < before ? w0 + e : s1 + (e - before));
        const uint64_t x = have ? xres[i - w0] : (uint64_t)ST_NOANCHOR;
        const uint32_t st = (uint32_t)(x & 0xFFu), pos = (uint32_t)(x >> 8);
        const uint64_t g = first_global + i;
        const uint32_t* pk = R.packed + 2 * R.slot_off[i];
        const bool sane = have && (st == ST_NOANCHOR || ((st == ST_HIT || st == ST_UNRESOLVED) && R.len[i] >= k && pos <= R.len[i] - k));
        if (have && !sane) atomicExch(D.err, 2);
        if (sane && st == ST_NOANCHOR) V.status[i] = ST_NOANCHOR;
        if (sane && st == ST_HIT) {
            uint64_t fin = IDX_INF;
            const uint32_t slot = dict_find(D, canon_at<K>(pk, pos, k), fin);
            if (slot == 0xFFFFFFFFu || !(fin < g)) atomicExch(D.err, 2);
            else { V.status[i] = ST_HIT; V.hit_pos[i] = pos; V.hit_slot[i] = slot; }
        }
        const bool want = sane && st == ST_UNRESOLVED;
        bool created = false;
        auto propose = [&]() {
            const K ck = canon_at<K>(pk, pos, k);
            const uint32_t sl = dict_find_or_insert<true>(D, ck, created);
            atomicMin((unsigned long long*)tent_ptr(D, sl), (unsigned long long)g);
            const uint32_t pb = window_bit(ck);
            atomicOr(&D.pbits[pb >> 5], 1u << (pb & 31));
            V.status[i] = ST_UNRESOLVED; V.cand_pos[i] = pos; V.cand_slot[i] = sl;
        };
        const unsigned long long wm = __ballot(want);
        if (KT<K>::W == 1) { if (want) propose(); }
        else {
            for (unsigned long long m = wm; m; m &= m - 1) if (lane == (uint32_t)__builtin_ctzll(m)) propose();
        }
        const unsigned long long cm = __ballot(created);
        if (lane == 0) { wave_n[wv] = (uint32_t)__popcll(wm); wave_new[wv] = (uint32_t)__popcll(cm); }
        __syncthreads();
        if (threadIdx.x == 0) {
            const uint32_t tot = wave_n[0] + wave_n[1] + wave_n[2] + wave_n[3], fresh = wave_new[0] + wave_new[1] + wave_new[2] + wave_new[3];
            block_at = tot ? atomicAdd(ucount, tot) : 0u;
            if (fresh) atomicAdd(D.n_keys, (unsigned long long)fresh);
        }
        __syncthreads();
        if (want) {
            uint32_t at = block_at + (uint32_t)__popcll(wm & ((1ull << lane) - 1));
            for (uint32_t w = 0; w < wv; w++) at += wave_n[w];
            ulist[at] = (uint32_t)i;
        }
        __syncthreads();
    }
}
void launch_lookup_apply(hipStream_t s, ReadsDev R, DictDev D, ResolveDev V, uint64_t w0, uint64_t w1, uint64_t s0, uint64_t s1,
                         uint64_t first_global, const uint64_t* xres, uint32_t* ulist, uint32_t* ucount) {
    if (w1 - w0 <= s1 - s0) return;
    DISPATCH_K(R.k, hipLaunchKernelGGL(k_lookup_apply<K>, dim3(grid_for((w1 - w0) - (s1 - s0), 256, 256 * 16)), dim3(256), 0, s, R, D, V, w0, w1, s0, s1,
                                       first_global, xres, ulist, ucount));
}

template <typename K>
__global__ void __launch_bounds__(256) k_check(ReadsDev R, DictDev D, ResolveDev V, uint64_t first_global,
                                              const uint32_t* ulist, const uint32_t* ucount,
                                              uint32_t* next_list, uint32_t* next_count) {
    const uint32_t lane = lane_id(), k = R.k;
    const uint32_t grp = lane >> 4, l = lane & 15, gbase = grp * 16;
    const uint64_t wave = (blockIdx.x * (uint64_t)blockDim.x + threadIdx.x) >> 6;
    const uint64_t nwaves = ((uint64_t)gridDim.x * blockDim.x) >> 6;
    const uint32_t count = *ucount;
    __shared__ uint32_t lists[4][64];
    uint32_t* my_list = lists[threadIdx.x >> 6];
    uint32_t n_list = 0;
    auto flush_list = [&]() {
        if (!n_list) return;
        uint32_t at = 0;
        if (lane == 0) at = atomicAdd(next_count, n_list);
        at = (uint32_t)__shfl((int)at, 0);
        __builtin_amdgcn_wave_barrier();
        if (lane < n_list) next_list[at + lane] = my_list[lane];
        __builtin_amdgcn_wave_barrier();
        n_list = 0;
    };
    for (uint64_t e0 = 4 * wave; e0 < count; e0 += 4 * nwaves) {
        const uint64_t e = e0 + grp;
        const bool have = e < count;
        const uint32_t i = have ? ulist[e] : 0u;
        const uint64_t g = first_global + i;
        const uint32_t nk = have ? R.len[i] - k + 1 : 0u;
        const uint32_t* pk = R.packed + 2 * (have ? R.slot_off[i] : 0);
        bool anyfin = false, anyblock = false;
        uint32_t base = 0;
        bool done = !have;
        while (__any(!done)) {
            const bool run = !done;
            const uint32_t p = base + l;
            const bool valid = run && p < nk;
            const uint32_t words = (run && l < 8) ? pk[(base >> 4) + l] : 0u;
            const K cn = canon_from_words16<K>(words, gbase, base, valid ? p : (run ? nk - 1 : 0), k);
            bool f = false, t = false;
            if (valid) {
                const uint32_t pb = window_bit(cn);
                if ((D.pbits[pb >> 5] >> (pb & 31)) & 1u) {
                    uint64_t fin = IDX_INF;
                    const uint32_t slot = dict_find(D, cn, fin);
                    if (slot != 0xFFFFFFFFu) {
                        f = fin < g;
                        t = *tent_ptr(D, slot) < g;
                    }
                }
            }
            const uint32_t fq = (uint32_t)(__ballot(f) >> gbase) & 0xFFFFu, tq = (uint32_t)(__ballot(t) >> gbase) & 0xFFFFu;
            if (run) {
                anyfin = anyfin || fq != 0;
                anyblock = anyblock || tq != 0;
                base += 16;
                done = anyfin || base >= nk;
            }
        }
        const bool blocked = have && !anyfin && anyblock;
        const unsigned long long bm = __ballot(blocked && l == 0);
        if (bm) {
            if (blocked && l == 0) my_list[n_list + (uint32_t)__popcll(bm & ((1ull << lane) - 1))] = i;
            n_list += (uint32_t)__popcll(bm);
            if (n_list > 64 - 4) flush_list();
        }
        const bool inserter = have && !anyfin && !anyblock;
        if (have && l == 0) {
            if (anyfin) V.status[i] = ST_HITNEW;
            else if (inserter) {
                V.status[i] = ST_INSERTER;
                const uint32_t slot = V.cand_slot[i];
                __hip_atomic_store(fin_ptr<K>(D, slot), g, __ATOMIC_RELAXED, __HIP_MEMORY_SCOPE_AGENT);
                const uint32_t wb = window_bit(dict_key<K>(D, slot));
                atomicOr(&D.wbits[wb >> 5], 1u << (wb & 31));
            }
        }
        for (unsigned long long im = __ballot(inserter && l == 0); im; im &= im - 1) {
            const uint32_t src = (uint32_t)__builtin_ctzll(im);
            const uint32_t ii = (uint32_t)__shfl((int)i, (int)src);
            const K key = dict_key<K>(D, V.cand_slot[ii]);
            const uint32_t hmin = key_minimizer_wave(D, key, k, lane);
            if (lane == 0) atomicOr((unsigned long long*)D.fbits + filter_word(D, hmin), (unsigned long long)filter_bits(key));
        }
    }
    flush_list();
}
void launch_check(hipStream_t s, ReadsDev R, DictDev D, ResolveDev V, uint64_t first_global, const uint32_t* ulist,
                  const uint32_t* ucount, uint32_t max_count, uint32_t* next_list, uint32_t* next_count) {
    if (!max_count) return;
    DISPATCH_K(R.k, hipLaunchKernelGGL(k_check<K>, dim3(grid_for(max_count, 16, 256 * 16)), dim3(256), 0, s, R, D, V, first_global, ulist,
                                       ucount, next_list, next_count));
}

__global__ void k_reset_tent(DictDev D, ResolveDev V, const uint32_t* list, const uint32_t* count) {
    uint32_t n = *count;
    for (uint64_t e = blockIdx.x * (uint64_t)blockDim.x + threadIdx.x; e < n; e += (uint64_t)gridDim.x * blockDim.x)
        *tent_ptr(D, V.cand_slot[list[e]]) = IDX_INF;
}
void launch_reset_tent(hipStream_t s, DictDev D, ResolveDev V, const uint32_t* list, const uint32_t* count, uint32_t max_count) {
    if (!max_count) return;
    hipLaunchKernelGGL(k_reset_tent, dim3(grid_for(max_count, 256)), dim3(256), 0, s, D, V, list, count);
}
__global__ void k_propose(DictDev D, ResolveDev V, uint64_t first_global, const uint32_t* list, const uint32_t* count) {
    uint32_t n = *count;
    for (uint64_t e = blockIdx.x * (uint64_t)blockDim.x + threadIdx.x; e < n; e += (uint64_t)gridDim.x * blockDim.x) {
        uint32_t i = list[e];
        atomicMin((unsigned long long*)tent_ptr(D, V.cand_slot[i]), (unsigned long long)(first_global + i));
    }
}
void launch_propose(hipStream_t s, DictDev D, ResolveDev V, uint64_t first_global, const uint32_t* list,
                    const uint32_t* count, uint32_t max_count) {
    if (!max_count) return;
    hipLaunchKernelGGL(k_propose, dim3(grid_for(max_count, 256)), dim3(256), 0, s, D, V, first_global, list, count);
}

template <typename K>
__global__ void __launch_bounds__(256) k_final_pos(ReadsDev R, DictDev D, ResolveDev V, uint64_t w0, uint64_t w1, uint64_t first_global) {
    const uint32_t lane = lane_id(), k = R.k;
    const uint32_t grp = lane >> 4, l = lane & 15, gbase = grp * 16;
    const uint64_t wave = (blockIdx.x * (uint64_t)blockDim.x + threadIdx.x) >> 6;
    const uint64_t nwaves = ((uint64_t)gridDim.x * blockDim.x) >> 6;
    for (uint64_t i0 = w0 + 4 * wave; i0 < w1; i0 += 4 * nwaves) {
        const uint64_t i = i0 + grp;
        const bool have = i < w1;
        const uint8_t st = have ? V.status[i] : (uint8_t)ST_NOANCHOR;
        const bool mine = st == ST_HIT || st == ST_HITNEW;
        const uint64_t g = first_global + i;
        const uint32_t limit = !mine ? 0u : (st == ST_HIT ? V.hit_pos[i] : R.len[i] - k + 1);
        const uint32_t* pk = R.packed + 2 * (mine ? R.slot_off[i] : 0);
        uint32_t base = 0;
        bool done = limit == 0;
        while (__any(!done)) {
            const bool run = !done;
            const uint32_t p = base + l;
            const bool valid = run && p < limit;
            const uint32_t words = (run && l < 8) ? pk[(base >> 4) + l] : 0u;
            const K cn = canon_from_words16<K>(words, gbase, base, valid ? p : (run ? limit - 1 : 0), k);
            bool hit = false; uint32_t slot = 0xFFFFFFFFu;
            if (valid) {
                const uint32_t wb = window_bit(cn);
                if ((D.wbits[wb >> 5] >> (wb & 31)) & 1u) {
                    uint64_t fin = IDX_INF;
                    slot = dict_find(D, cn, fin);
                    hit = slot != 0xFFFFFFFFu && fin < g;
                }
            }
            const unsigned long long bal = __ballot(hit);
            const uint32_t gb = (uint32_t)(bal >> gbase) & 0xFFFFu;
            if (run) {
                if (gb) {
                    const uint32_t f = (uint32_t)__builtin_ctz(gb);
                    const uint32_t hs = __shfl(slot, (int)(gbase + f));
                    if (l == 0) { V.hit_pos[i] = base + f; V.hit_slot[i] = hs; }
                    done = true;
                } else { base += 16; done = base >= limit; }
            }
        }
    }
}
void launch_final_pos(hipStream_t s, ReadsDev R, DictDev D, ResolveDev V, uint64_t w0, uint64_t w1, uint64_t first_global) {
    if (w1 <= w0) return;
    DISPATCH_K(R.k, hipLaunchKernelGGL(k_final_pos<K>, dim3(grid_for(w1 - w0, 16, 256 * 16)), dim3(256), 0, s, R, D, V, w0, w1, first_global));
}

__global__ void k_ins_flags(ResolveDev V, uint64_t w0, uint64_t w1) {
    for (uint64_t i = w0 + blockIdx.x * (uint64_t)blockDim.x + threadIdx.x; i < w1; i += (uint64_t)gridDim.x * blockDim.x)
        V.ins_flag[i - w0] = V.status[i] == ST_INSERTER ? 1u : 0u;
}
void launch_ins_flags(hipStream_t s, ResolveDev V, uint64_t w0, uint64_t w1) {
    if (w1 <= w0) return;
    hipLaunchKernelGGL(k_ins_flags, dim3(grid_for(w1 - w0, 256)), dim3(256), 0, s, V, w0, w1);
}
template <typename K>
__global__ void k_assign_addr(DictDev D, ResolveDev V, uint64_t w0, uint64_t w1, const uint32_t* rank, uint64_t addr_base,
                              uint64_t* anchor_kmers) {
    for (uint64_t i = w0 + blockIdx.x * (uint64_t)blockDim.x + threadIdx.x; i < w1; i += (uint64_t)gridDim.x * blockDim.x) {
        if (V.status[i] != ST_INSERTER) continue;
        uint64_t a = addr_base + rank[i - w0];
        uint32_t slot = V.cand_slot[i];
        D.addr[slot] = (uint32_t)a;
        store_kmer(anchor_kmers + a * KT<K>::W, dict_key<K>(D, slot));
        V.hit_pos[i] = V.cand_pos[i];
        V.hit_slot[i] = slot;
    }
}
void launch_assign_addr(hipStream_t s, DictDev D, ResolveDev V, uint64_t w0, uint64_t w1, const uint32_t* rank,
                        uint64_t addr_base, uint64_t* anchor_kmers, uint32_t k) {
    if (w1 <= w0) return;
    DISPATCH_K(k, hipLaunchKernelGGL(k_assign_addr<K>, dim3(grid_for(w1 - w0, 256)), dim3(256), 0, s, D, V, w0, w1, rank, addr_base, anchor_kmers));
}
template <typename K>
__global__ void k_finalize_reads(ReadsDev R, DictDev D, ResolveDev V, uint64_t w0, uint64_t w1) {
    uint32_t k = R.k;
    for (uint64_t i = w0 + blockIdx.x * (uint64_t)blockDim.x + threadIdx.x; i < w1; i += (uint64_t)gridDim.x * blockDim.x) {
        uint8_t st = V.status[i];
        if (st == ST_NOANCHOR) {
            V.anchor_pos[i] = -1; V.anchor_addr[i] = 0; V.flags[i] = 0; V.sort_key[i] = 1ull << 32;
            continue;
        }
        uint32_t pos = V.hit_pos[i];
        uint32_t addr = D.addr[V.hit_slot[i]];
        const uint32_t* pk = R.packed + 2 * R.slot_off[i];
        const K km = kmer_at<K>(pk, pos, k);
        uint32_t rev = revcomp(km, k) < km ? 1u : 0u;
        V.anchor_pos[i] = (int32_t)pos; V.anchor_addr[i] = addr;
        V.flags[i] = (uint8_t)(rev | (st == ST_INSERTER ? 2u : 0u));
        V.sort_key[i] = addr;
    }
}
void launch_finalize_reads(hipStream_t s, ReadsDev R, DictDev D, ResolveDev V, uint64_t w0, uint64_t w1) {
    if (w1 <= w0) return;
    DISPATCH_K(R.k, hipLaunchKernelGGL(k_finalize_reads<K>, dim3(grid_for(w1 - w0, 256)), dim3(256), 0, s, R, D, V, w0, w1));
}

__global__ void k_chain_flags(const uint8_t* status, uint64_t w0, uint64_t w1, uint32_t* flag) {
    for (uint64_t i = w0 + blockIdx.x * (uint64_t)blockDim.x + threadIdx.x; i < w1; i += (uint64_t)gridDim.x * blockDim.x)
        flag[i - w0] = status[i] == ST_UNRESOLVED ? 1u : 0u;
}
__global__ void k_chain_compact(const uint8_t* status, uint64_t w0, uint64_t w1, const uint32_t* rank, uint32_t* list) {
    for (uint64_t i = w0 + blockIdx.x * (uint64_t)blockDim.x + threadIdx.x; i < w1; i += (uint64_t)gridDim.x * blockDim.x)
        if (status[i] == ST_UNRESOLVED) list[rank[i - w0]] = (uint32_t)i;
}
void launch_chain_flags(hipStream_t s, ResolveDev V, uint64_t w0, uint64_t w1, uint32_t* flag) {
    if (w1 <= w0) return;
    hipLaunchKernelGGL(k_chain_flags, dim3(grid_for(w1 - w0, 256)), dim3(256), 0, s, V.status, w0, w1, flag);
}
void launch_chain_compact(hipStream_t s, ResolveDev V, uint64_t w0, uint64_t w1, const uint32_t* rank, uint32_t* list) {
    if (w1 <= w0) return;
    hipLaunchKernelGGL(k_chain_compact, dim3(grid_for(w1 - w0, 256)), dim3(256), 0, s, V.status, w0, w1, rank, list);
}
__global__ void k_chain_reset(DictDev D, ResolveDev V, const uint32_t* list, uint32_t n) {
    for (uint64_t e = blockIdx.x * (uint64_t)blockDim.x + threadIdx.x; e < n; e += (uint64_t)gridDim.x * blockDim.x)
        *tent_ptr(D, V.cand_slot[list[e]]) = IDX_INF;
}
__global__ void k_chain_propose(DictDev D, ResolveDev V, uint64_t first_global, const uint32_t* list, uint32_t n) {
    for (uint64_t e = blockIdx.x * (uint64_t)blockDim.x + threadIdx.x; e < n; e += (uint64_t)gridDim.x * blockDim.x) {
        const uint32_t i = list[e];
        atomicMin((unsigned long long*)tent_ptr(D, V.cand_slot[i]), (unsigned long long)(first_global + i));
    }
}
void launch_chain_repropose(hipStream_t s, DictDev D, ResolveDev V, uint64_t first_global, const uint32_t* reset_list, uint32_t n_reset,
                            const uint32_t* list, uint32_t n) {
    if (n_reset) hipLaunchKernelGGL(k_chain_reset, dim3(grid_for(n_reset, 256)), dim3(256), 0, s, D, V, reset_list, n_reset);
    if (n) hipLaunchKernelGGL(k_chain_propose, dim3(grid_for(n, 256)), dim3(256), 0, s, D, V, first_global, list, n);
}

template <typename K, bool FILL>
__global__ void __launch_bounds__(256) k_chain_prep(ReadsDev R, DictDev D, ResolveDev V, uint64_t first_global, uint64_t w0,
                                                   const uint32_t* list, uint32_t n, uint32_t c0, const uint32_t* rank,
                                                   uint32_t* cnt, uint32_t* own, const uint64_t* gbase, uint32_t* ent,
                                                   const unsigned long long* om, const unsigned long long* late, unsigned long long* dep_out,
                                                   unsigned long long* xdep_out) {
    const uint32_t lane = lane_id(), k = R.k;
    const uint32_t grp = lane >> 4, l = lane & 15, gbase16 = grp * 16;
    const uint64_t wave = (blockIdx.x * (uint64_t)blockDim.x + threadIdx.x) >> 6;
    const uint64_t nwaves = ((uint64_t)gridDim.x * blockDim.x) >> 6;
    for (uint64_t e0 = 4 * wave; e0 < n; e0 += 4 * nwaves) {
        const uint64_t e = e0 + grp;
        const bool have = e < n;
        const uint32_t i = have ? list[e] : 0u;
        const uint64_t g = first_global + i;
        const uint32_t nk = have ? R.len[i] - k + 1 : 0u;
        const uint32_t* pk = R.packed + 2 * (have ? R.slot_off[i] : 0);
        const uint32_t g0 = (uint32_t)e & ~63u, le = (uint32_t)e & 63u;
        const uint32_t p0 = g0 >= 64 ? g0 - 64 : 0u;
        uint32_t total = 0;
        bool dead = false;
        bool done = !have;
        uint64_t at = 0;
        unsigned long long dep = 0ull, xdep = 0ull, late_below = 0ull, late_prev = 0ull;
        if (FILL) {
            done = !have || (cnt[e] >> 31);
            at = have ? gbase[e >> 6] * 64 + le : 0;
            late_below = have ? late[e >> 6] & ((1ull << le) - 1ull) : 0ull;
            late_prev = have && g0 >= 64 ? late[(e >> 6) - 1] : 0ull;
        }
        uint32_t base = 0;
        while (__any(!done)) {
            const bool run = !done;
            const uint32_t p = base + l;
            const bool valid = run && p < nk;
            const uint32_t words = (run && l < 8) ? pk[(base >> 4) + l] : 0u;
            const K cn = canon_from_words16<K>(words, gbase16, base, valid ? p : (run ? nk - 1 : 0), k);
            bool f = false, t = false;
            uint32_t kid = 0;
            if (valid) {
                const uint32_t pb = window_bit(cn);
                if ((D.pbits[pb >> 5] >> (pb & 31)) & 1u) {
                    uint64_t fin = IDX_INF;
                    const uint32_t slot = dict_find(D, cn, fin);
                    if (slot != 0xFFFFFFFFu) {
                        f = fin < g;
                        const uint64_t tv = *tent_ptr(D, slot);
                        t = tv < g;
                        if (t) kid = rank[tv - first_global - w0] - c0;
                    }
                }
            }
            const bool outer = t && kid < p0;
            const uint32_t fq = (uint32_t)(__ballot(f) >> gbase16) & 0xFFFFu, oq = (uint32_t)(__ballot(outer) >> gbase16) & 0xFFFFu;
            if (FILL) {
                if (outer) ent[at + 64ull * (total + (uint32_t)__popc(oq & ((1u << l) - 1u)))] = kid;
                if (t && kid >= g0) dep |= om[kid];
                else if (t) {
                    if (kid >= p0) xdep |= om[kid];
                    for (unsigned long long m = late_prev; m; m &= m - 1) {
                        const uint32_t a = (uint32_t)__builtin_ctzll(m);
                        if (own[p0 + a] == kid) xdep |= 1ull << a;
                    }
                    for (unsigned long long m = late_below; m; m &= m - 1) {
                        const uint32_t a = (uint32_t)__builtin_ctzll(m);
                        if (own[g0 + a] == kid) dep |= 1ull << a;
                    }
                }
            } else dead = dead || fq != 0;
            if (run) {
                total += (uint32_t)__popc(oq);
                base += 16;
                done = dead || base >= nk;
            }
        }
        if (FILL) {
            for (int d = 1; d < 16; d <<= 1) { dep |= (unsigned long long)__shfl_xor((long long)dep, d); xdep |= (unsigned long long)__shfl_xor((long long)xdep, d); }
            if (have && l == 0) { const bool dd = (cnt[e] >> 31) != 0; dep_out[e] = dd ? 0ull : dep & ((1ull << le) - 1ull); xdep_out[e] = dd ? 0ull : xdep; }
        } else if (have && l == 0) {
            cnt[e] = dead ? 0x80000000u : total;
            own[e] = rank[*tent_ptr(D, V.cand_slot[i]) - first_global - w0] - c0;
        }
    }
}
void launch_chain_prep(hipStream_t s, bool fill, ReadsDev R, DictDev D, ResolveDev V, uint64_t first_global, uint64_t w0, const uint32_t* list,
                       uint32_t n, uint32_t c0, const uint32_t* rank, uint32_t* cnt, uint32_t* own, const uint64_t* gbase, uint32_t* ent,
                       const unsigned long long* om, const unsigned long long* late, unsigned long long* dep, unsigned long long* xdep) {
    if (!n) return;
    if (fill) DISPATCH_K(R.k, hipLaunchKernelGGL((k_chain_prep<K, true>), dim3(grid_for(n, 16, 256 * 16)), dim3(256), 0, s, R, D, V, first_global, w0, list, n, c0, rank, cnt, own, gbase, ent, om, late, dep, xdep));
    else DISPATCH_K(R.k, hipLaunchKernelGGL((k_chain_prep<K, false>), dim3(grid_for(n, 16, 256 * 16)), dim3(256), 0, s, R, D, V, first_global, w0, list, n, c0, rank, cnt, own, gbase, ent, om, late, dep, xdep));
}
__global__ void __launch_bounds__(256) k_chain_tables(const uint32_t* cnt, const uint32_t* own, uint32_t n, uint64_t* rows, unsigned long long* om, unsigned long long* late) {
    __shared__ unsigned long long tab[4][64];
    const uint32_t lane = lane_id(), wv = threadIdx.x >> 6;
    const uint64_t wave = (blockIdx.x * (uint64_t)blockDim.x + threadIdx.x) >> 6, nwaves = ((uint64_t)gridDim.x * blockDim.x) >> 6;
    const uint64_t nG = ((uint64_t)n + 63) / 64;
    for (uint64_t G = wave; G <= nG; G += nwaves) {
        const uint64_t e = G * 64 + lane;
        const bool have = G < nG && e < n;
        const uint32_t cd = have ? cnt[e] : 0x80000000u, o = have ? own[e] : 0u;
        const uint32_t g0 = (uint32_t)G * 64;
        uint32_t c = (cd >> 31) ? 0u : cd;
        for (int d = 1; d < 64; d <<= 1) { const uint32_t x = (uint32_t)__shfl_xor((int)c, d); c = x > c ? x : c; }
        if (lane == 0) rows[G] = c;
        if (G < nG) {
            tab[wv][lane] = 0ull;
            __builtin_amdgcn_wave_barrier();
            if (have && o >= g0) atomicOr(&tab[wv][o - g0], 1ull << lane);
            __builtin_amdgcn_wave_barrier();
            om[G * 64 + lane] = tab[wv][lane];
            const unsigned long long lm = __ballot(have && !(cd >> 31) && o < g0);
            if (lane == 0) late[G] = lm;
        }
    }
}
void launch_chain_tables(hipStream_t s, const uint32_t* cnt, const uint32_t* own, uint32_t n, uint64_t* rows, unsigned long long* om, unsigned long long* late) {
    hipLaunchKernelGGL(k_chain_tables, dim3(grid_for((n + 63) / 64 + 1, 4)), dim3(256), 0, s, cnt, own, n, rows, om, late);
}

struct ChainSlot { uint32_t own[64], cnt[64], dep_lo[64], dep_hi[64], xdep_lo[64], xdep_hi[64], hit[64], ent[CHAIN_EL][64]; uint64_t gb; uint32_t rows, pad; };
constexpr uint32_t CHAIN_BITS_WORDS = 1u << (CHAIN_LOG2 - 5);
size_t chain_seq_lds_bytes() { return CHAIN_BITS_WORDS * 4 + CHAIN_DEPTH * sizeof(ChainSlot) + (2 * CHAIN_DEPTH + 2) * 4; }
template <bool TRACE>
__global__ void __launch_bounds__(512) k_chain_seq(uint32_t n, const uint32_t* cnt, const uint32_t* own, const unsigned long long* depv, const unsigned long long* xdepv,
                                                  const uint64_t* gbase , const uint32_t* ent, unsigned long long* insmask ,
                                                  unsigned long long* trace ) {
    extern __shared__ uint32_t chain_lds[];
    uint32_t* bits = chain_lds;
    ChainSlot* ring = reinterpret_cast<ChainSlot*>(chain_lds + CHAIN_BITS_WORDS);
    uint32_t* ready = reinterpret_cast<uint32_t*>(ring + CHAIN_DEPTH);
    uint32_t* tested = ready + CHAIN_DEPTH;
    uint32_t* settled = tested + CHAIN_DEPTH;
    const uint32_t lane = lane_id(), wv = threadIdx.x >> 6;
    const uint32_t nG = (n + 63) / 64;
    for (uint32_t w = threadIdx.x; w < CHAIN_BITS_WORDS; w += blockDim.x) bits[w] = 0u;
    if (threadIdx.x < 2 * CHAIN_DEPTH) ready[threadIdx.x] = 0u;
    if (threadIdx.x == 0) *settled = 0u;
    __syncthreads();
    auto flag = [](uint32_t* f) { return __hip_atomic_load(f, __ATOMIC_RELAXED, __HIP_MEMORY_SCOPE_WORKGROUP); };
    auto raise = [](uint32_t* f, uint32_t v) { __atomic_signal_fence(__ATOMIC_SEQ_CST); __hip_atomic_store(f, v, __ATOMIC_RELAXED, __HIP_MEMORY_SCOPE_WORKGROUP); };
    if (wv >= 2) {
        if (wv == 4 || wv == 5) return;
        for (uint32_t G = wv < 4 ? wv - 2 : wv - 4; G < nG; G += 4) {
            const uint32_t e = G * 64 + lane;
            const uint64_t gb = gbase[G];
            const uint32_t rows = (uint32_t)(gbase[G + 1] - gb);
            const uint32_t o = e < n ? own[e] : 0u, cd = e < n ? cnt[e] : 0x80000000u;
            const unsigned long long dp = e < n ? depv[e] : 0ull, xd = e < n ? xdepv[e] : 0ull;
            constexpr uint32_t PASS = 32;
            uint32_t v[PASS];
#pragma unroll
            for (uint32_t j = 0; j < PASS; j++) v[j] = j < rows ? ent[(gb + j) * 64 + lane] : 0u;
            while (G >= flag(settled) + CHAIN_DEPTH) __builtin_amdgcn_s_sleep(2);
            __atomic_signal_fence(__ATOMIC_SEQ_CST);
            ChainSlot& S = ring[G % CHAIN_DEPTH];
            S.own[lane] = o; S.cnt[lane] = cd; S.dep_lo[lane] = (uint32_t)dp; S.dep_hi[lane] = (uint32_t)(dp >> 32);
            S.xdep_lo[lane] = (uint32_t)xd; S.xdep_hi[lane] = (uint32_t)(xd >> 32);
            if (lane == 0) { S.gb = gb; S.rows = rows; }
#pragma unroll
            for (uint32_t j = 0; j < PASS; j++) if (j < rows) S.ent[j][lane] = v[j];
            for (uint32_t p0 = PASS; p0 < rows && p0 < CHAIN_EL; p0 += PASS) {
#pragma unroll
                for (uint32_t j = 0; j < PASS; j++) v[j] = p0 + j < rows ? ent[(gb + p0 + j) * 64 + lane] : 0u;
#pragma unroll
                for (uint32_t j = 0; j < PASS; j++) if (p0 + j < rows) S.ent[p0 + j][lane] = v[j];
            }
            raise(&ready[G % CHAIN_DEPTH], G + 1);
        }
        return;
    }
    if (wv == 1) {
        for (uint32_t G = 0; G < nG; G++) {
            while (flag(&ready[G % CHAIN_DEPTH]) != G + 1) __builtin_amdgcn_s_sleep(0);
// ... 764 lines not shown
```

### leon_amd/csrc/kernels.h

```cpp
#pragma once
#include <hip/hip_runtime.h>
#include <stdint.h>
#include "leon_device.h"

namespace leon {

struct ReadsDev {
    const uint32_t* packed;
    const uint32_t* nmask;
    const uint64_t* slot_off;
    const uint64_t* base_off;
    const uint32_t* len;
    const uint32_t* n_count;
    uint64_t n;
    uint64_t ev_origin;
    uint32_t k, pad;
};

struct DictDev {
    uint64_t* slots;
    uint64_t* tent;
    uint64_t tstride;
    uint32_t* addr;
    uint64_t mask;
    unsigned long long* n_keys;
    uint32_t* wbits;
    uint32_t* fbits;
    uint32_t* pbits;
    uint32_t fwshift;
    uint32_t mm_m, mm_P, mm_c;
    int* err;
};
constexpr uint32_t WBITS_LOG2 = 23;
inline void minimizer_geometry(uint32_t k, uint32_t& m, uint32_t& P, uint32_t& c) {
    if (k <= 16) { m = k; P = 1; c = 0; return; }
    for (m = 16;; m--) {
        const uint32_t w = k - m + 1;
        P = 1;
        while (P * 2 <= w && P < 32) P *= 2;
        if (((w - P) & 1) == 0) { c = (w - P) / 2; return; }
    }
}
constexpr uint32_t FBITS_LOG2_MAX = 31;
constexpr uint32_t FBITS_LOG2_DEFAULT = 28;

enum : uint8_t { ST_NOANCHOR = 0, ST_HIT = 1, ST_UNRESOLVED = 2, ST_INSERTER = 3, ST_HITNEW = 4 };

struct ResolveDev {
    uint8_t* status;
    uint32_t* hit_pos; uint32_t* hit_slot;
    uint32_t* cand_pos; uint32_t* cand_slot;
    int32_t* anchor_pos; uint32_t* anchor_addr; uint8_t* flags; uint64_t* sort_key;
    uint32_t* ins_flag;
};

void launch_bloom_insert(hipStream_t s, BloomDev B, const uint16_t* rv16, const uint64_t* kmers, uint64_t n);
void launch_bloom_query(hipStream_t s, BloomDev B, const uint16_t* rv16, const uint64_t* kmers, uint64_t n,
                        int mode , uint8_t* out);
void launch_rebase_offsets(hipStream_t s, uint64_t* off, uint64_t n, uint64_t base);
void launch_read_slots(hipStream_t s, const uint64_t* base_off, uint64_t n, uint64_t* slots, uint32_t* bad );
void launch_pack(hipStream_t s, const uint8_t* bases, const uint64_t* base_off, const uint64_t* slot_off, uint64_t n,
                 uint32_t* packed, uint32_t* nmask, uint32_t* len, uint32_t* n_count);
void launch_dict_init(hipStream_t s, DictDev D, uint64_t cap, uint32_t W);
void launch_dict_rehash(hipStream_t s, DictDev from, uint64_t from_cap, DictDev to, uint32_t k);
void launch_lookup_cand(hipStream_t s, ReadsDev R, BloomDev B, const uint16_t* rv16, DictDev D, ResolveDev V,
                        uint64_t w0, uint64_t w1, uint64_t first_global, uint32_t* ulist, uint32_t* ucount,
                        unsigned long long* trace = nullptr ,
                        uint64_t* xres = nullptr ,
                        uint64_t xbase = 0, bool dry = false );
void launch_lookup_apply(hipStream_t s, ReadsDev R, DictDev D, ResolveDev V, uint64_t w0, uint64_t w1, uint64_t s0, uint64_t s1,
                         uint64_t first_global, const uint64_t* xres, uint32_t* ulist, uint32_t* ucount);
void launch_check(hipStream_t s, ReadsDev R, DictDev D, ResolveDev V, uint64_t first_global,
                  const uint32_t* ulist, const uint32_t* ucount, uint32_t max_count, uint32_t* next_list, uint32_t* next_count);
void launch_reset_tent(hipStream_t s, DictDev D, ResolveDev V, const uint32_t* list, const uint32_t* count, uint32_t max_count);
void launch_propose(hipStream_t s, DictDev D, ResolveDev V, uint64_t first_global, const uint32_t* list,
                    const uint32_t* count, uint32_t max_count);
void launch_final_pos(hipStream_t s, ReadsDev R, DictDev D, ResolveDev V, uint64_t w0, uint64_t w1, uint64_t first_global);
void launch_ins_flags(hipStream_t s, ResolveDev V, uint64_t w0, uint64_t w1);
void launch_assign_addr(hipStream_t s, DictDev D, ResolveDev V, uint64_t w0, uint64_t w1, const uint32_t* rank,
                        uint64_t addr_base, uint64_t* anchor_kmers, uint32_t k);
constexpr uint32_t CHAIN_LOG2 = 19;
constexpr uint32_t CHAIN_EL = 96;
constexpr uint32_t CHAIN_DEPTH = 3;
void launch_chain_flags(hipStream_t s, ResolveDev V, uint64_t w0, uint64_t w1, uint32_t* flag);
void launch_chain_compact(hipStream_t s, ResolveDev V, uint64_t w0, uint64_t w1, const uint32_t* rank, uint32_t* list);
void launch_chain_repropose(hipStream_t s, DictDev D, ResolveDev V, uint64_t first_global, const uint32_t* reset_list, uint32_t n_reset,
                            const uint32_t* list, uint32_t n);
void launch_chain_prep(hipStream_t s, bool fill, ReadsDev R, DictDev D, ResolveDev V, uint64_t first_global, uint64_t w0, const uint32_t* list,
                       uint32_t n, uint32_t c0, const uint32_t* rank, uint32_t* cnt, uint32_t* own, const uint64_t* gbase, uint32_t* ent,
                       const unsigned long long* om, const unsigned long long* late, unsigned long long* dep, unsigned long long* xdep);
void launch_chain_tables(hipStream_t s, const uint32_t* cnt, const uint32_t* own, uint32_t n, uint64_t* rows ,
                         unsigned long long* om , unsigned long long* late );
int launch_chain_seq(hipStream_t s, uint32_t n, const uint32_t* cnt, const uint32_t* own, const unsigned long long* dep, const unsigned long long* xdep,
                     const uint64_t* gbase, const uint32_t* ent, unsigned long long* ins , unsigned long long* trace );
void launch_chain_apply(hipStream_t s, DictDev D, ResolveDev V, uint64_t first_global, const uint32_t* list, uint32_t n, const unsigned long long* ins, uint32_t k);
void launch_anchor_symbols(hipStream_t s, const uint64_t* kmers, uint64_t n_anchors, uint32_t k, uint8_t* syms);
void launch_finalize_reads(hipStream_t s, ReadsDev R, DictDev D, ResolveDev V, uint64_t w0, uint64_t w1);
struct WalkCache { uint64_t* slots; uint64_t bucket_mask; uint32_t hop_shift, pad; };
void launch_walk_cache_init(hipStream_t s, WalkCache C, uint32_t k);
void launch_walk(hipStream_t s, ReadsDev R, BloomDev B, const uint16_t* rv16, const int32_t* anchor_pos, const uint8_t* flags,
                 const uint32_t* perm, uint64_t n_walk, uint8_t* events, const uint64_t* ev_off = nullptr ,
                 WalkCache wc = WalkCache{nullptr, 0, 28, 0});
void launch_lower_bound(hipStream_t s, const uint64_t* sorted, uint64_t n, uint64_t bound, unsigned long long* out);
void launch_slice_weights(hipStream_t s, const uint64_t* sorted_keys, uint64_t n, uint64_t* w );
void launch_slice_splits(hipStream_t s, const uint64_t* cum , uint64_t n, uint32_t world, unsigned long long* split );
void launch_slice_reads(hipStream_t s, ReadsDev R, const uint32_t* perm , uint64_t n_slice, uint64_t* len_out ,
                        uint32_t* slot_of );
void launch_ev_words(hipStream_t s, ReadsDev R, const uint32_t* slot_of, const uint64_t* ev_off, const uint8_t* events, uint64_t n, uint32_t rpb,
                     uint64_t n_blocks, uint32_t world, uint64_t* cnt_or_off , uint64_t* send );
void launch_ev_scatter(hipStream_t s, const uint64_t* words, uint64_t n_words, uint8_t* events, uint64_t n_bytes, int* err);
void launch_prev_anchored(hipStream_t s, const int32_t* anchor_pos, uint64_t n, uint32_t rpb, uint64_t first_block,
                          uint64_t n_blocks, int64_t* prev);
void launch_symbols(hipStream_t s, ReadsDev R, const int32_t* anchor_pos, const uint32_t* anchor_addr,
                    const uint8_t* flags, const int64_t* prev, const uint8_t* events, uint64_t r0, uint64_t n_local,
                    uint64_t* sym_off , uint32_t* n_err ,
                    uint8_t* syms );
void launch_block_ranges(hipStream_t s, const uint64_t* sym_off, uint64_t n_reads, uint32_t rpb, uint64_t n_blocks,
                         uint64_t* blk_begin , uint64_t* out_off );
void launch_max_block_syms(hipStream_t s, const uint64_t* sym_off , uint64_t n_reads, uint32_t rpb, uint64_t n_blocks,
                           unsigned long long* out_max );
void launch_rc_encode(hipStream_t s, const uint8_t* syms, const uint64_t* blk_begin, uint64_t n_blocks,
                      uint8_t* out, const uint64_t* out_off, uint64_t* out_size, uint32_t* model_scratch, int* err,
                      uint64_t max_block_syms, uint32_t small_sizes = SMALL_SIZES_DNA, bool counts_apart = false);
size_t rc_records_state_bytes(uint64_t n_blocks);
void launch_rc_records(hipStream_t s, const uint8_t* syms, const uint64_t* blk_begin, uint64_t n_blocks, uint32_t tile0, uint32_t tile1, uint64_t* recs,
                       const uint64_t* rec_off, uint32_t* state, uint32_t* model_scratch, int* err, uint32_t small_sizes);
void launch_hdr_symbols(hipStream_t s, const uint8_t* hdr, const uint64_t* off, uint64_t n, uint32_t rpb, const uint8_t* first,
                        uint32_t first_len, uint64_t* sym_off , uint8_t* syms );
size_t rc_model_scratch_bytes(uint64_t n_blocks);
void launch_gather_payload(hipStream_t s, const uint8_t* out, const uint64_t* out_off, const uint64_t* dst_off,
                           const uint64_t* sizes, uint64_t n_blocks, uint8_t* dst);

void launch_qual_smooth(hipStream_t s, ReadsDev R, BloomDev B, const uint16_t* rv16, uint8_t* quals);
void launch_read_minimizer(hipStream_t s, ReadsDev R, uint32_t* key , uint32_t* mpos );
void launch_mpos_from_anchors(hipStream_t s, ReadsDev R, const int32_t* anchor_pos, const uint32_t* anchor_addr, const uint8_t* flags, uint32_t* key, uint32_t* mpos);
void launch_solid_flags(hipStream_t s, ReadsDev R, BloomDev B, const uint16_t* rv16, const uint32_t* perm, const uint32_t* mpos,
                        uint32_t* flags );
void launch_qual_rewrite(hipStream_t s, ReadsDev R, const uint32_t* flags, uint8_t* quals);
struct PathCache { uint64_t* slots; uint64_t bucket_mask; };
size_t path_cache_slot_bytes(uint32_t k);
void launch_path_cache_init(hipStream_t s, PathCache C, uint32_t k);
void launch_path_cache_prewalk(hipStream_t s, BloomDev B, PathCache C, const uint16_t* rv16, const uint64_t* anchors, uint64_t n_anchors, uint32_t max_steps);
void launch_bloom_fingerprint(hipStream_t s, const uint8_t* bits, uint64_t n_bytes, uint64_t* d_sum );
size_t decode_scratch_bytes(uint64_t n_blocks);
void launch_hdr_decode_symbols(hipStream_t s, const uint8_t* payloads, const uint64_t* pay_off, const uint32_t* blk_reads, uint64_t n_blocks,
                               uint8_t* syms, const uint64_t* sym_begin, unsigned long long* sym_count, int* err);
constexpr uint32_t LEON_HT_HEADER_CAP = 4096;
enum : uint32_t { HT_OK = 0, HT_LONG = 1, HT_SHARE = 2, HT_SYMS = 3, HT_NOSYMS = 4, HT_INVALID = 16 };
void launch_hdr_text(hipStream_t s, const uint8_t* syms, const uint64_t* sym_begin, const unsigned long long* sym_count, const uint32_t* blk_reads,
                     const uint64_t* read0, const uint64_t* text_begin, uint64_t n_blocks, const uint8_t* first, uint32_t first_len,
                     uint8_t* text , uint64_t* off, uint32_t* status, uint64_t* text_size);
void launch_decode_blocks(hipStream_t s, BloomDev B, PathCache C, const uint16_t* rv16, const uint64_t* anchors, uint64_t n_anchors,
                          const uint8_t* payloads, const uint64_t* pay_off, const uint32_t* blk_reads, const uint64_t* blk_read0,
                          const uint64_t* blk_out0, uint64_t n_blocks, uint8_t* out, uint32_t* out_len, uint32_t* scratch,
                          uint32_t* pool, unsigned long long* pool_cursor, uint64_t pool_words, int* err,
                          unsigned long long* stats );

struct FmtLayout { uint64_t first_read_index, hdr_bytes; uint32_t wrap; uint8_t lead, fastq, plus_kind; };
struct FmtPair {
    uint64_t rec, base;
    FmtPair() = default;
    __host__ __device__ FmtPair(int v) : rec((uint64_t)v), base((uint64_t)v) {}
    __host__ __device__ FmtPair(uint64_t r, uint64_t b) : rec(r), base(b) {}
    __host__ __device__ FmtPair operator+(const FmtPair& o) const { return FmtPair(rec + o.rec, base + o.base); }
};
void launch_fmt_sizes(hipStream_t s, const FmtLayout& L, const uint32_t* len, const uint64_t* hdr_off, uint64_t n_reads, FmtPair* in, uint32_t* flags);
hipError_t fmt_scan(void* tmp, size_t& bytes, const FmtPair* in, FmtPair* out, uint64_t n_reads, hipStream_t s);
void launch_fmt_rec_off(hipStream_t s, const FmtPair* off, uint64_t n_reads, uint64_t* rec_off);
void launch_fmt_records(hipStream_t s, const FmtLayout& L, const FmtPair* off, const uint64_t* hdr_off, uint64_t n_reads, const uint8_t* bases,
                        const uint8_t* hdr, const uint8_t* quals, uint8_t* text, uint64_t text_size);

// ... 16 lines not shown
```

Before: 18550.

## Round-tag tentative slots, fuse check/reset/propose, overlap walk prep on side stream

Tentative dictionary entries now carry a round tag, so per-window and per-round resets and memsets are replaced by bumping a counter, with a full clear only when the tag space runs low. The check kernel can fuse the reset and propose steps, and the separate ins_flags pass and chain reset launches are removed. Walk setup (events memset, walk-cache init, iota) and prev_anchored now run on a second stream and overlap with resolution. This cuts launches and memsets, at the cost of more complex tag logic and a wider tent layout.

```diff
diff --git a/leon_amd/csrc/capi.hip b/leon_amd/csrc/capi.hip
--- a/leon_amd/csrc/capi.hip
+++ b/leon_amd/csrc/capi.hip
@@ -91,6 +91,8 @@
     leon_dna_cfg cfg{};
     int device = 0;
     hipStream_t stream = nullptr;
+    hipStream_t prep_stream = nullptr;
+    hipEvent_t prep_ev[4]{};
     uint64_t* h_rb = nullptr;
     std::string err;
     uint8_t* d_bloom = nullptr;
@@ -99,6 +101,7 @@
     uint16_t* d_rv16 = nullptr;
     DictDev D{};
     uint64_t dict_cap = 0;
+    uint32_t tent_round = 0;
     uint64_t n_keys = 0;
     unsigned long long* d_nkeys = nullptr;
     uint64_t n_anchors = 0;
@@ -162,7 +165,8 @@
 
 void dict_free(DictDev& D) {
     if (D.slots) (void)hipFree(D.slots);
-    if (D.tent && D.tstride == 1) (void)hipFree(D.tent);
+    if (D.tent && D.tstride == 2) (void)hipFree(D.tent);
+    if (D.tent1 && D.t1stride == 1) (void)hipFree(D.tent1);
     if (D.addr) (void)hipFree(D.addr);
     D = DictDev{};
 }
@@ -170,13 +174,15 @@
     const uint32_t W = kmer_words(c->cfg.kmer_size);
     D = DictDev{};
     hipError_t e = hipMalloc((void**)&D.slots, cap * 16 * W);
-    if (e == hipSuccess && W == 1) { D.tstride = 1; e = hipMalloc((void**)&D.tent, cap * 8); }
+    if (e == hipSuccess && W == 1) { D.tstride = 2; e = hipMalloc((void**)&D.tent, cap * 16); }
+    if (e == hipSuccess && W == 2) { D.t1stride = 1; e = hipMalloc((void**)&D.tent1, cap * 8); }
     if (e == hipSuccess) e = hipMalloc((void**)&D.addr, cap * 4);
     if (e != hipSuccess) {
         dict_free(D);
         return fail(c, LEON_E_HIP, std::string("anchor dictionary allocation: ") + hipGetErrorString(e));
     }
     if (W == 2) { D.tent = D.slots + 3; D.tstride = 4; }
+    else { D.tent1 = D.tent + 1; D.t1stride = 2; }
     D.mask = cap - 1;
     D.n_keys = c->d_nkeys;
     D.wbits = c->wbits.as<uint32_t>();
@@ -567,6 +573,8 @@
     } while (0)
     CREATE_CHK(hipSetDevice(c->device));
     CREATE_CHK(hipStreamCreateWithFlags(&c->stream, hipStreamNonBlocking));
+    CREATE_CHK(hipStreamCreateWithFlags(&c->prep_stream, hipStreamNonBlocking));
+    for (auto& e : c->prep_ev) CREATE_CHK(hipEventCreateWithFlags(&e, hipEventDisableTiming));
     CREATE_CHK(hipHostMalloc((void**)&c->h_rb, 4096, hipHostMallocDefault));
     for (auto& e : c->ev) CREATE_CHK(hipEventCreate(&e));
     uint64_t blk = 1ull << cfg->bloom_block_nbits;
@@ -607,6 +615,7 @@
     if (!c) return;
     delete c->anchor_worker;
     (void)hipSetDevice(c->device);
+    if (c->prep_stream) (void)hipStreamSynchronize(c->prep_stream);
     if (c->stream) (void)hipStreamSynchronize(c->stream);
     dict_free(c->D);
     DevBuf* bufs[] = { &c->anchor_kmers, &c->in_bases, &c->in_off, &c->slot_off, &c->packed, &c->nmask, &c->rlen, &c->ncount,
@@ -628,6 +637,8 @@
     for (auto& e : c->ev) if (e) (void)hipEventDestroy(e);
     for (auto& e : c->pack_ev) (void)hipEventDestroy(e);
     for (auto& e : c->chain_ev) (void)hipEventDestroy(e);
+    for (auto& e : c->prep_ev) if (e) (void)hipEventDestroy(e);
+    if (c->prep_stream) (void)hipStreamDestroy(c->prep_stream);
     if (c->stream) (void)hipStreamDestroy(c->stream);
     delete c;
 }
@@ -733,6 +744,7 @@
     uint32_t chain_chunk;
     bool xch_lookups, walk_cache;
     long walk_cache_log2, walk_hop_log2;
+    bool resolve_fused;
     bool trace_step, trace_resolve, trace_chain;
 };
 long env_num(const char* name, long dflt) { const char* e = getenv(name); return e ? atol(e) : dflt; }
@@ -746,6 +758,7 @@
     K.chain_chunk = chunk >= 1 && chunk <= (1l << CHAIN_LOG2) ? (uint32_t)chunk : 1u << CHAIN_LOG2;
     K.xch_lookups = env_num("LEON_XCH_LOOKUPS", 1) != 0; K.walk_cache = env_num("LEON_WALK_CACHE", 1) != 0;
     K.walk_cache_log2 = env_num("LEON_WALK_CACHE_LOG2", 0); K.walk_hop_log2 = hop >= 1 && hop <= 8 ? hop : 4;
+    K.resolve_fused = env_num("LEON_RESOLVE_FUSED", 1) != 0;
     K.trace_step = getenv("LEON_TRACE_STEP"); K.trace_resolve = getenv("LEON_TRACE_RESOLVE"); K.trace_chain = getenv("LEON_TRACE_CHAIN");
     return K;
 }
@@ -763,7 +776,8 @@
     ReadsDev R{}; ResolveDev V{};
     uint64_t packed_upto = 0; uint32_t n_pack_ev = 0;
     static constexpr uint32_t kRoundsMore = 2, kHist = 64;
-    uint32_t* counters = nullptr; uint32_t* lists[2] = {nullptr, nullptr}; uint32_t* d_hist = nullptr; unsigned long long* d_trace = nullptr;
+    bool prep_used = false, prep_prev = false;
+    uint32_t* lists[2] = {nullptr, nullptr}; uint32_t* d_hist = nullptr; unsigned long long* d_trace = nullptr;
     size_t scan_tmp = 0;
     struct Pending { int buf = -1; uint64_t n = 0; } pending;
     int anchor_buf = 0; bool share_lookups = false;
@@ -808,9 +822,11 @@
         V.cand_pos = c->cand_pos.as<uint32_t>(); V.cand_slot = c->cand_slot.as<uint32_t>();
         V.anchor_pos = c->anchor_pos.as<int32_t>(); V.anchor_addr = c->anchor_addr.as<uint32_t>(); V.flags = c->flags.as<uint8_t>();
         V.sort_key = c->sort_key.as<uint64_t>(); V.ins_flag = c->ins_flag.as<uint32_t>();
-        counters = c->counters.as<uint32_t>(); lists[0] = c->ulist0.as<uint32_t>(); lists[1] = c->ulist1.as<uint32_t>();
+        lists[0] = c->ulist0.as<uint32_t>(); lists[1] = c->ulist1.as<uint32_t>();
         HIPCHK(c, prim::ExclusiveSum(nullptr, scan_tmp, V.ins_flag, c->rank.as<uint32_t>(), W, s));
-        return ensure_cub(c, scan_tmp);
+        if (int rc = ensure_cub(c, scan_tmp)) return rc;
+        if (int rc = take_share()) return rc;
+        return queue_prep();
     }
     int pack_next_group() {
         const uint64_t a = packed_upto, b = group_end(a, n, c->cfg.resolve_window);
@@ -858,17 +874,22 @@
         }
         HIPCHK(c, hipGetLastError());
         HIPCHK(c, hipEventRecord(c->ev[2], s));
+        if (prep_prev) {
+            HIPCHK(c, hipEventRecord(c->prep_ev[2], s));
+            HIPCHK(c, hipStreamWaitEvent(c->prep_stream, c->prep_ev[2], 0));
+            launch_prev_anchored(c->prep_stream, V.anchor_pos, n, rpb, sh.lb0, sh.nbl, c->prev.as<int64_t>());
+            HIPCHK(c, hipEventRecord(c->prep_ev[3], c->prep_stream));
+        }
         mark("resolution launched to its end");
         return LEON_OK;
     }
     int resolve_window(uint64_t w0, uint64_t w1) {
         if (int rc = dict_reserve(c, c->n_keys + (w1 - w0))) return rc;
-        HIPCHK(c, hipMemsetAsync(counters, 0, 8, s));
-        HIPCHK(c, hipMemsetAsync(c->wbits.p, 0, (1ull << WBITS_LOG2) / 8, s));
-        HIPCHK(c, hipMemsetAsync(c->pbits.p, 0, (1ull << WBITS_LOG2) / 8, s));
-        if (!share_lookups) launch_lookup_cand(s, R, c->B, c->d_rv16, c->D, V, w0, w1, first_read_index, lists[0], counters, d_trace);
+        if (c->tent_round > TENT_TAG_MAX / 2) { launch_tent_clear(s, c->D, c->dict_cap); c->tent_round = 0; }
+        c->tent_round++;
+        launch_window_clear(s, c->D, d_hist, kHist);
+        if (!share_lookups) launch_lookup_cand(s, R, c->B, c->d_rv16, c->D, V, w0, w1, first_read_index, lists[0], d_hist, c->tent_round, d_trace);
         else if (int rc = look_up_shared(w0, w1)) return rc;
-        HIPCHK(c, hipMemcpyAsync(d_hist, counters, 4, hipMemcpyDeviceToDevice, s));
         uint32_t cnt0 = 0;
         if (int rc = fixpoint_rounds(w0, w1, cnt0)) return rc;
         hint = std::max<uint32_t>(2 * cnt0, 4096);
@@ -881,7 +902,7 @@
         auto run_of = [&](uint32_t r, uint64_t& a, uint64_t& b) { a = std::min(w1, w0 + (uint64_t)r * P); b = std::min(w1, a + P); };
         HIPCHK(c, c->xch_res.ensure((uint64_t)Wn * P * 8)); uint64_t* xres = c->xch_res.as<uint64_t>();
         uint64_t s0 = 0, s1 = 0; run_of(c->shard_rank, s0, s1);
-        launch_lookup_cand(s, R, c->B, c->d_rv16, c->D, V, s0, s1, first_read_index, lists[0], counters, d_trace, xres, w0, false);
+        launch_lookup_cand(s, R, c->B, c->d_rv16, c->D, V, s0, s1, first_read_index, lists[0], d_hist, c->tent_round, d_trace, xres, w0, false);
         HIPCHK(c, hipStreamSynchronize(s));
         const auto t_l0 = std::chrono::steady_clock::now();
         if (c->xch_mode == LEON_XCH_BY_ANCHOR) {
@@ -892,12 +913,12 @@
             for (uint32_t r = 0; r < Wn; r++) {
                 if (r == c->shard_rank) continue;
                 uint64_t a = 0, b = 0; run_of(r, a, b);
-                launch_lookup_cand(s, R, c->B, c->d_rv16, c->D, V, a, b, first_read_index, lists[0], counters, nullptr, xres, w0, true);
+                launch_lookup_cand(s, R, c->B, c->d_rv16, c->D, V, a, b, first_read_index, lists[0], d_hist, c->tent_round, nullptr, xres, w0, true);
             }
             HIPCHK(c, hipStreamSynchronize(s));
             lk_emul_ms += ms_since(t_l0);
         }
-        launch_lookup_apply(s, R, c->D, V, w0, w1, s0, s1, first_read_index, xres, lists[0], counters);
+        launch_lookup_apply(s, R, c->D, V, w0, w1, s0, s1, first_read_index, xres, lists[0], d_hist, c->tent_round);
         return LEON_OK;
     }
     int fixpoint_rounds(uint64_t w0, uint64_t w1, uint32_t& cnt0) {
@@ -908,11 +929,12 @@
             for (uint32_t r = 0; r < ahead && n_hist < kHist; r++) {
                 const int nxt = cur ^ 1;
                 const uint32_t h = std::max<uint32_t>(hint >> (2 * (n_hist - 1) < 31 ? 2 * (n_hist - 1) : 31), 4096);
-                HIPCHK(c, hipMemsetAsync(counters + nxt, 0, 4, s));
-                launch_check(s, R, c->D, V, first_read_index, lists[cur], counters + cur, h, lists[nxt], counters + nxt);
-                HIPCHK(c, hipMemcpyAsync(d_hist + n_hist, counters + nxt, 4, hipMemcpyDeviceToDevice, s));
-                launch_reset_tent(s, c->D, V, lists[cur], counters + cur, h);
-                launch_propose(s, c->D, V, first_read_index, lists[nxt], counters + nxt, h);
+                launch_check(s, R, c->D, V, first_read_index, lists[cur], d_hist + (n_hist - 1), h, lists[nxt], d_hist + n_hist, c->tent_round, knobs.resolve_fused);
+                if (!knobs.resolve_fused) {
+                    launch_reset_tent(s, c->D, V, lists[cur], d_hist + (n_hist - 1), h, c->tent_round);
+                    launch_propose(s, c->D, V, first_read_index, lists[nxt], d_hist + n_hist, h, c->tent_round + 1);
+                }
+                c->tent_round++;
                 cur = nxt; n_hist++;
             }
             HIPCHK(c, hipMemcpyAsync(c->h_rb + 8, d_hist, n_hist * 4, hipMemcpyDeviceToHost, s));
@@ -948,7 +970,10 @@
         if (knobs.trace_chain) { HIPCHK(c, c->chain_trace.ensure(8 * 8)); d_ctrace = c->chain_trace.as<unsigned long long>(); HIPCHK(c, hipMemsetAsync(d_ctrace, 0, 8 * 8, s)); }
         for (uint32_t c0 = 0; c0 < left; c0 += CH) {
             const uint32_t nc = std::min(CH, left - c0), nG = (nc + 63) / 64;
-            if (c0) launch_chain_repropose(s, c->D, V, first_read_index, clist + (c0 - CH), left - (c0 - CH), clist + c0, left - c0);
+            if (c0) {
+                if (c->tent_round >= TENT_TAG_MAX - 1) return fail(c, LEON_E_OVERFLOW, "anchor resolution: the round counter ran out inside one window");
+                launch_chain_repropose(s, c->D, V, first_read_index, clist + c0, left - c0, ++c->tent_round);
+            }
             HIPCHK(c, c->chain_cnt.ensure((uint64_t)nc * 4)); HIPCHK(c, c->chain_own.ensure((uint64_t)nc * 4));
             HIPCHK(c, c->chain_ins.ensure(((uint64_t)nG + 1) * 8)); HIPCHK(c, c->chain_rows.ensure(((uint64_t)nG + 1) * 8));
             HIPCHK(c, c->chain_dep.ensure((uint64_t)nc * 8)); HIPCHK(c, c->chain_xdep.ensure((uint64_t)nc * 8));
@@ -960,20 +985,19 @@
             size_t rows_tmp = 0;
             HIPCHK(c, prim::ExclusiveSum(nullptr, rows_tmp, rows, rows, nG + 1, s));
             if (rows_tmp > c->cub_tmp.cap) { HIPCHK(c, hipStreamSynchronize(s)); if (int rc = ensure_cub(c, std::max(rows_tmp, scan_tmp))) return rc; }
-            launch_chain_prep(s, false, R, c->D, V, first_read_index, w0, clist + c0, nc, c0, rank, cnt, own, nullptr, nullptr, nullptr, nullptr, nullptr, nullptr);
+            launch_chain_prep(s, false, c->tent_round, R, c->D, V, first_read_index, w0, clist + c0, nc, c0, rank, cnt, own, nullptr, nullptr, nullptr, nullptr, nullptr, nullptr);
             launch_chain_tables(s, cnt, own, nc, rows, om, late);
             HIPCHK(c, prim::ExclusiveSum(c->cub_tmp.p, rows_tmp, rows, rows, nG + 1, s));
             HIPCHK(c, hipMemcpyAsync(c->h_rb + 0, rows + nG, 8, hipMemcpyDeviceToHost, s));
             HIPCHK(c, spin_sync(s));
             const uint64_t total_rows = c->h_rb[0];
             HIPCHK(c, c->chain_ent.ensure(std::max<uint64_t>(total_rows, 1) * 64 * 4)); uint32_t* ent = c->chain_ent.as<uint32_t>();
-            launch_chain_prep(s, true, R, c->D, V, first_read_index, w0, clist + c0, nc, c0, rank, cnt, own, rows, ent, om, late, dep, xdep);
+            launch_chain_prep(s, true, c->tent_round, R, c->D, V, first_read_index, w0, clist + c0, nc, c0, rank, cnt, own, rows, ent, om, late, dep, xdep);
             if (launch_chain_seq(s, nc, cnt, own, dep, xdep, rows, ent, c->chain_ins.as<unsigned long long>(), d_ctrace))
                 return fail(c, LEON_E_HIP, "the sequential resolution pass could not be launched (its LDS request was refused)");
             launch_chain_apply(s, c->D, V, first_read_index, clist + c0, nc, c->chain_ins.as<unsigned long long>(), k);
             HIPCHK(c, hipGetLastError());
         }
-        { const uint32_t c_last = (left - 1) / CH * CH; launch_chain_repropose(s, c->D, V, first_read_index, clist + c_last, left - c_last, nullptr, 0); }
         HIPCHK(c, hipEventRecord(c->chain_ev[2 * n_chain_ev + 1], s));
         n_chain_ev++;
         c->stats.resolve_chain_reads += left; c->stats.resolve_chain_windows++;
@@ -990,7 +1014,6 @@
     }
     int settle(uint64_t w0, uint64_t w1) {
         launch_final_pos(s, R, c->D, V, w0, w1, first_read_index);
-        launch_ins_flags(s, V, w0, w1);
         HIPCHK(c, prim::ExclusiveSum(c->cub_tmp.p, scan_tmp, V.ins_flag, c->rank.as<uint32_t>(), w1 - w0, s));
         HIPCHK(c, hipMemcpyAsync(c->h_rb + 0, c->rank.as<uint32_t>() + (w1 - w0 - 1), 4, hipMemcpyDeviceToHost, s));
         HIPCHK(c, hipMemcpyAsync(c->h_rb + 1, V.ins_flag + (w1 - w0 - 1), 4, hipMemcpyDeviceToHost, s));
@@ -1036,20 +1059,33 @@
         }
         nl_bases = off_r1 - off_r0;
         R.ev_origin = sh.r0;
-        c->stats.n_reads = sh.nl; c->stats.n_bases = nl_bases; c->stats.n_blocks = sh.nbl; c->stats.n_anchors = c->n_anchors;
-        c->last_n = n; c->last_bases = nl_bases; c->last_d_bases = d_bases; c->last_d_off = d_off;
+        c->stats.n_reads = sh.nl; c->stats.n_bases = nl_bases; c->stats.n_blocks = sh.nbl;
         by_anchor = c->shard_world > 1 && c->xch_mode != LEON_XCH_OFF;
         return LEON_OK;
     }
+    bool nothing_to_encode() const { return sh.nl == 0 && !(by_anchor && c->xch_mode == LEON_XCH_BY_ANCHOR); }
+    int queue_prep() {
+        if (nothing_to_encode()) return LEON_OK;
+        HIPCHK(c, c->events.ensure(nl_bases + 16));
+        HIPCHK(c, c->perm.ensure(n * 4));
+        if (sh.nl) { HIPCHK(c, c->prev.ensure(n * 8)); HIPCHK(c, c->nerr.ensure(sh.nl * 8)); }
+        size_walk_cache();
+        const hipStream_t ps = c->prep_stream;
+        HIPCHK(c, hipEventRecord(c->prep_ev[0], s));
+        HIPCHK(c, hipStreamWaitEvent(ps, c->prep_ev[0], 0));
+        prep_used = true;
+        HIPCHK(c, hipMemsetAsync(c->events.p, 0, nl_bases + 16, ps));
+        if (wc.slots) launch_walk_cache_init(ps, wc, k);
+        hipLaunchKernelGGL(k_iota, dim3((uint32_t)std::min<uint64_t>((n + 255) / 256, 8192)), dim3(256), 0, ps, c->perm.as<uint32_t>(), n);
+        HIPCHK(c, hipEventRecord(c->prep_ev[1], ps));
+        prep_prev = sh.nl != 0;
+        return LEON_OK;
+    }
     int walk() {
-        HIPCHK(c, c->events.ensure(nl_bases + 16));
-        HIPCHK(c, hipMemsetAsync(c->events.p, 0, nl_bases + 16, s));
-        start_walk_cache();
-        HIPCHK(c, c->perm.ensure(n * 4));
-        hipLaunchKernelGGL(k_iota, dim3((uint32_t)std::min<uint64_t>((n + 255) / 256, 8192)), dim3(256), 0, s, c->perm.as<uint32_t>(), n);
+        HIPCHK(c, hipStreamWaitEvent(s, c->prep_ev[1], 0));
         return by_anchor ? walk_by_anchor() : walk_share();
     }
-    void start_walk_cache() {
+    void size_walk_cache() {
         uint64_t buckets = knobs.walk_cache ? walk_cache_buckets(c) : 0;
         if (!buckets) return;
         if (knobs.walk_cache_log2 >= 10 && knobs.walk_cache_log2 <= 31) buckets = 1ull << knobs.walk_cache_log2;
@@ -1057,7 +1093,6 @@
         if (hipMemGetInfo(&free_b, &total_b) == hipSuccess) while (buckets > 1024 && buckets * 64 > c->wcache.cap && buckets * 64 > free_b / 8) buckets >>= 1;
         if (c->wcache.ensure(buckets * 64) != hipSuccess) { (void)hipGetLastError(); return; }
         wc.slots = c->wcache.as<uint64_t>(); wc.bucket_mask = buckets - 1; wc.hop_shift = 32 - knobs.walk_hop_log2;
-        launch_walk_cache_init(s, wc, k);
     }
     int walk_share() {
         const uint64_t r0 = sh.r0, nl = sh.nl;
@@ -1175,9 +1210,7 @@
         return LEON_OK;
     }
     int code(CodedBlocks& out) {
-        HIPCHK(c, c->prev.ensure(n * 8));
-        HIPCHK(c, c->nerr.ensure(sh.nl * 8));
-        launch_prev_anchored(s, V.anchor_pos, n, rpb, sh.lb0, sh.nbl, c->prev.as<int64_t>());
+        HIPCHK(c, hipStreamWaitEvent(s, c->prep_ev[3], 0));
         auto symbols = [&](uint8_t* syms) {
             launch_symbols(s, R, V.anchor_pos, V.anchor_addr, V.flags, c->prev.as<int64_t>(), c->events.as<uint8_t>(), sh.r0, sh.nl,
                            c->sym_off.as<uint64_t>(), c->nerr.as<uint32_t>(), syms);
@@ -1216,20 +1249,26 @@
     if (!d_bases || !d_off || !sink) return fail(c, LEON_E_INVALID, "null argument");
     if (n > 0xFFFFFFF0ull) return fail(c, LEON_E_INVALID, "more than 2^32 reads in one batch");
     HIPCHK(c, hipSetDevice(c->device));
+    if (first_read_index + n > TENT_IDX_MASK) return fail(c, LEON_E_OVERFLOW, "more than 2^40 reads in one stream");
     EncodeBatch B{c, d_bases, d_off, n, first_read_index, sink, user, up, up_off};
-    if (int rc = B.start()) return rc;
-    c->poisoned = true;
-    if (int rc = B.resolve()) return rc;
-    if (int rc = B.take_share()) return rc;
-    if (B.sh.nl == 0 && !(B.by_anchor && c->xch_mode == LEON_XCH_BY_ANCHOR)) {
-        HIPCHK(c, hipStreamSynchronize(c->stream));
-        return B.finish(2);
-    }
-    if (int rc = B.walk()) return rc;
-    if (B.sh.nl == 0) return B.finish(5);
-    CodedBlocks out;
-    if (int rc = B.code(out)) return rc;
-    return B.finish(8, &out);
+    const int rc = [&]() -> int {
+        if (int rc = B.start()) return rc;
+        c->poisoned = true;
+        if (int rc = B.resolve()) return rc;
+        c->stats.n_anchors = c->n_anchors;
+        c->last_n = n; c->last_bases = B.nl_bases; c->last_d_bases = d_bases; c->last_d_off = d_off;
+        if (B.nothing_to_encode()) {
+            HIPCHK(c, hipStreamSynchronize(c->stream));
+            return B.finish(2);
+        }
+        if (int rc = B.walk()) return rc;
+        if (B.sh.nl == 0) return B.finish(5);
+        CodedBlocks out;
+        if (int rc = B.code(out)) return rc;
+        return B.finish(8, &out);
+    }();
+    if (rc != LEON_OK && B.prep_used) (void)hipStreamSynchronize(c->prep_stream);
+    return rc;
 }
 
 static int encode_batch_guarded(leon_dna_ctx* c, const uint8_t* d_bases, const uint64_t* d_off, uint64_t n,
@@ -1574,7 +1613,7 @@
         launch_dict_init(c->stream, c->D, c->dict_cap, kmer_words(c->cfg.kmer_size));
         HIPCHK(c, spin_sync(c->stream));
     }
-    c->n_keys = 0; c->n_anchors = 0;
+    c->n_keys = 0; c->n_anchors = 0; c->tent_round = 0;
     c->next_read = 0; c->next_block = 0; c->partial_seen = false; c->finished = false; c->poisoned = false;
     c->hdr_next_read = 0; c->hdr_next_block = 0; c->hdr_partial_seen = false;
     c->last_n = 0; c->last_bases = 0; c->last_d_bases = c->last_d_off = nullptr;
diff --git a/leon_amd/csrc/dna_kernels.hip b/leon_amd/csrc/dna_kernels.hip
--- a/leon_amd/csrc/dna_kernels.hip
+++ b/leon_amd/csrc/dna_kernels.hip
@@ -135,17 +135,44 @@
 template <> struct DS<u128> { static constexpr uint32_t STRIDE = 4, CLAIM = 1, FIN = 2; };
 template <typename K> __device__ inline uint64_t* slot_ptr(const DictDev& D, uint64_t slot) { return D.slots + slot * DS<K>::STRIDE; }
 template <typename K> __device__ inline uint64_t* fin_ptr(const DictDev& D, uint64_t slot) { return slot_ptr<K>(D, slot) + DS<K>::FIN; }
-__device__ inline uint64_t* tent_ptr(const DictDev& D, uint64_t slot) { return D.tent + slot * D.tstride; }
+__device__ inline uint64_t* tent_ptr(const DictDev& D, uint64_t slot, uint32_t round) { return (round & 1u) ? D.tent1 + slot * D.t1stride : D.tent + slot * D.tstride; }
+__device__ inline uint64_t tent_word(uint32_t round, uint64_t g) { return ((uint64_t)(TENT_TAG_MAX - round) << TENT_IDX_BITS) | g; }
+__device__ inline uint64_t tent_of(const DictDev& D, uint64_t slot, uint32_t round) {
+    const uint64_t v = *tent_ptr(D, slot, round);
+    return (uint32_t)(v >> TENT_IDX_BITS) == TENT_TAG_MAX - round ? (v & TENT_IDX_MASK) : IDX_INF;
+}
+__device__ inline void tent_propose(const DictDev& D, uint64_t slot, uint32_t round, uint64_t g) {
+    atomicMin((unsigned long long*)tent_ptr(D, slot, round), (unsigned long long)tent_word(round, g));
+}
 
 __global__ void k_dict_init(DictDev D, uint64_t cap, uint32_t W) {
     for (uint64_t i = blockIdx.x * (uint64_t)blockDim.x + threadIdx.x; i < cap; i += (uint64_t)gridDim.x * blockDim.x) {
-        if (W == 2) { D.slots[4 * i] = KEY_EMPTY; D.slots[4 * i + 1] = KEY_EMPTY; D.slots[4 * i + 2] = IDX_INF; D.slots[4 * i + 3] = IDX_INF; }
-        else { D.slots[2 * i] = KEY_EMPTY; D.slots[2 * i + 1] = IDX_INF; D.tent[i] = IDX_INF; }
+        if (W == 2) { D.slots[4 * i] = KEY_EMPTY; D.slots[4 * i + 1] = KEY_EMPTY; D.slots[4 * i + 2] = IDX_INF; }
+        else { D.slots[2 * i] = KEY_EMPTY; D.slots[2 * i + 1] = IDX_INF; }
+        *tent_ptr(D, i, 0) = IDX_INF; *tent_ptr(D, i, 1) = IDX_INF;
         D.addr[i] = 0;
     }
 }
 void launch_dict_init(hipStream_t s, DictDev D, uint64_t cap, uint32_t W) {
     hipLaunchKernelGGL(k_dict_init, dim3(grid_for(cap, 256)), dim3(256), 0, s, D, cap, W);
+}
+__global__ void k_tent_clear(DictDev D, uint64_t cap) {
+    for (uint64_t i = blockIdx.x * (uint64_t)blockDim.x + threadIdx.x; i < cap; i += (uint64_t)gridDim.x * blockDim.x) {
+        *tent_ptr(D, i, 0) = IDX_INF; *tent_ptr(D, i, 1) = IDX_INF;
+    }
+}
+void launch_tent_clear(hipStream_t s, DictDev D, uint64_t cap) {
+    hipLaunchKernelGGL(k_tent_clear, dim3(grid_for(cap, 256)), dim3(256), 0, s, D, cap);
+}
+__global__ void __launch_bounds__(256) k_window_clear(uint4* wbits, uint4* pbits, uint32_t n16, uint32_t* hist, uint32_t n_hist) {
+    const uint32_t t = blockIdx.x * blockDim.x + threadIdx.x;
+    const uint4 z = make_uint4(0u, 0u, 0u, 0u);
+    for (uint32_t j = t; j < n16; j += gridDim.x * blockDim.x) { wbits[j] = z; pbits[j] = z; }
+    if (t < n_hist) hist[t] = 0u;
+}
+void launch_window_clear(hipStream_t s, DictDev D, uint32_t* hist, uint32_t n_hist) {
+    const uint32_t n16 = (uint32_t)((1ull << WBITS_LOG2) / 8 / 16);
+    hipLaunchKernelGGL(k_window_clear, dim3(grid_for(n16 > n_hist ? n16 : n_hist, 256, 1u << 20)), dim3(256), 0, s, (uint4*)D.wbits, (uint4*)D.pbits, n16, hist, n_hist);
 }
 
 __device__ inline uint32_t dict_find(const DictDev& D, uint64_t key, uint64_t& fin) {
@@ -269,7 +296,8 @@
         bool created = false;
         if (i < from_cap && from.slots[i * DS<K>::STRIDE + DS<K>::CLAIM] != KEY_EMPTY) {
             uint32_t s = dict_find_or_insert<false>(to, dict_key<K>(from, (uint32_t)i), created);
-            *fin_ptr<K>(to, s) = *fin_ptr<K>(from, i); *tent_ptr(to, s) = IDX_INF; to.addr[s] = from.addr[i];
+            *fin_ptr<K>(to, s) = *fin_ptr<K>(from, i); to.addr[s] = from.addr[i];
+            *tent_ptr(to, s, 0) = *tent_ptr(from, i, 0); *tent_ptr(to, s, 1) = *tent_ptr(from, i, 1);
         }
         const unsigned long long cm = __ballot(created);
         if (cm && lane_id() == (uint32_t)__builtin_ctzll(cm)) atomicAdd(to.n_keys, (unsigned long long)__popcll(cm));
@@ -304,7 +332,7 @@
 template <typename K, bool TRACE>
 __global__ void __launch_bounds__(256, (KT<K>::W == 2 ? 5 : 8)) k_lookup_cand(ReadsDev R, BloomDev B, const uint16_t* rv16g, DictDev D, ResolveDev V,
                                                     uint64_t w0, uint64_t w1, uint64_t first_global,
-                                                    uint32_t* ulist, uint32_t* ucount, unsigned long long* trace,
+                                                    uint32_t* ulist, uint32_t* ucount, uint32_t round, unsigned long long* trace,
                                                     uint64_t* xres, uint64_t xbase, uint32_t dry) {
     __shared__ uint16_t rv16[256];
     load_rv16(rv16, rv16g);
@@ -426,7 +454,7 @@
                 if (want_insert && grp == q) {
                     const K ck = canon_at<K>(pk, cpos, k);
                     sl = dict_find_or_insert<true>(D, ck, created);
-                    atomicMin((unsigned long long*)tent_ptr(D, sl), (unsigned long long)g);
+                    tent_propose(D, sl, round, g);
                     const uint32_t pb = window_bit(ck);
                     atomicOr(&D.pbits[pb >> 5], 1u << (pb & 31));
                     V.status[i] = ST_UNRESOLVED; V.cand_pos[i] = cpos; V.cand_slot[i] = sl;
@@ -451,19 +479,19 @@
     }
 }
 void launch_lookup_cand(hipStream_t s, ReadsDev R, BloomDev B, const uint16_t* rv16, DictDev D, ResolveDev V,
-                        uint64_t w0, uint64_t w1, uint64_t first_global, uint32_t* ulist, uint32_t* ucount, unsigned long long* trace,
+                        uint64_t w0, uint64_t w1, uint64_t first_global, uint32_t* ulist, uint32_t* ucount, uint32_t round, unsigned long long* trace,
                         uint64_t* xres, uint64_t xbase, bool dry) {
     if (w1 <= w0) return;
     if (trace && !dry) { DISPATCH_K(R.k, hipLaunchKernelGGL((k_lookup_cand<K, true>), dim3(grid_for(w1 - w0, 16, 256 * 16)), dim3(256), 0, s, R, B, rv16, D, V, w0, w1,
-                                                           first_global, ulist, ucount, trace, xres, xbase, 0u)); return; }
+                                                           first_global, ulist, ucount, round, trace, xres, xbase, 0u)); return; }
     const uint32_t per_cu = [] { const char* e = getenv("LEON_LOOKUP_BLOCKS_PER_CU"); const int v = e ? atoi(e) : 0; return v > 0 && v <= 1024 ? (uint32_t)v : 16u; }();
     DISPATCH_K(R.k, hipLaunchKernelGGL((k_lookup_cand<K, false>), dim3(grid_for(w1 - w0, 16, 256 * per_cu)), dim3(256), 0, s, R, B, rv16, D, V, w0, w1,
-                                       first_global, ulist, ucount, trace, xres, xbase, dry ? 1u : 0u));
+                                       first_global, ulist, ucount, round, trace, xres, xbase, dry ? 1u : 0u));
 }
 
 template <typename K>
 __global__ void __launch_bounds__(256) k_lookup_apply(ReadsDev R, DictDev D, ResolveDev V, uint64_t w0, uint64_t w1, uint64_t s0, uint64_t s1,
-                                                     uint64_t first_global, const uint64_t* xres, uint32_t* ulist, uint32_t* ucount) {
+                                                     uint64_t first_global, const uint64_t* xres, uint32_t* ulist, uint32_t* ucount, uint32_t round) {
     __shared__ uint32_t wave_n[4], wave_new[4], block_at;
     const uint32_t lane = lane_id(), wv = threadIdx.x >> 6, k = R.k;
     const uint64_t before = s0 - w0, n_out = (w1 - w0) - (s1 - s0);
@@ -489,7 +517,7 @@
         auto propose = [&]() {
             const K ck = canon_at<K>(pk, pos, k);
             const uint32_t sl = dict_find_or_insert<true>(D, ck, created);
-            atomicMin((unsigned long long*)tent_ptr(D, sl), (unsigned long long)g);
+            tent_propose(D, sl, round, g);
             const uint32_t pb = window_bit(ck);
             atomicOr(&D.pbits[pb >> 5], 1u << (pb & 31));
             V.status[i] = ST_UNRESOLVED; V.cand_pos[i] = pos; V.cand_slot[i] = sl;
@@ -517,16 +545,16 @@
     }
 }
 void launch_lookup_apply(hipStream_t s, ReadsDev R, DictDev D, ResolveDev V, uint64_t w0, uint64_t w1, uint64_t s0, uint64_t s1,
-                         uint64_t first_global, const uint64_t* xres, uint32_t* ulist, uint32_t* ucount) {
+                         uint64_t first_global, const uint64_t* xres, uint32_t* ulist, uint32_t* ucount, uint32_t round) {
     if (w1 - w0 <= s1 - s0) return;
     DISPATCH_K(R.k, hipLaunchKernelGGL(k_lookup_apply<K>, dim3(grid_for((w1 - w0) - (s1 - s0), 256, 256 * 16)), dim3(256), 0, s, R, D, V, w0, w1, s0, s1,
-                                       first_global, xres, ulist, ucount));
-}
-
-template <typename K>
+                                       first_global, xres, ulist, ucount, round));
+}
+
+template <typename K, bool FUSED>
 __global__ void __launch_bounds__(256) k_check(ReadsDev R, DictDev D, ResolveDev V, uint64_t first_global,
                                               const uint32_t* ulist, const uint32_t* ucount,
-                                              uint32_t* next_list, uint32_t* next_count) {
+                                              uint32_t* next_list, uint32_t* next_count, uint32_t round) {
     const uint32_t lane = lane_id(), k = R.k;
     const uint32_t grp = lane >> 4, l = lane & 15, gbase = grp * 16;
     const uint64_t wave = (blockIdx.x * (uint64_t)blockDim.x + threadIdx.x) >> 6;
@@ -569,7 +597,7 @@
                     const uint32_t slot = dict_find(D, cn, fin);
                     if (slot != 0xFFFFFFFFu) {
                         f = fin < g;
-                        t = *tent_ptr(D, slot) < g;
+                        t = tent_of(D, slot, round) < g;
                     }
                 }
             }
@@ -584,7 +612,10 @@
         const bool blocked = have && !anyfin && anyblock;
         const unsigned long long bm = __ballot(blocked && l == 0);
         if (bm) {
-            if (blocked && l == 0) my_list[n_list + (uint32_t)__popcll(bm & ((1ull << lane) - 1))] = i;
+            if (blocked && l == 0) {
+                my_list[n_list + (uint32_t)__popcll(bm & ((1ull << lane) - 1))] = i;
+                if (FUSED) tent_propose(D, V.cand_slot[i], round + 1u, g);
+            }
             n_list += (uint32_t)__popcll(bm);
             if (n_list > 64 - 4) flush_list();
         }
@@ -610,32 +641,34 @@
     flush_list();
 }
 void launch_check(hipStream_t s, ReadsDev R, DictDev D, ResolveDev V, uint64_t first_global, const uint32_t* ulist,
-                  const uint32_t* ucount, uint32_t max_count, uint32_t* next_list, uint32_t* next_count) {
+                  const uint32_t* ucount, uint32_t max_count, uint32_t* next_list, uint32_t* next_count, uint32_t round, bool fused) {
     if (!max_count) return;
-    DISPATCH_K(R.k, hipLaunchKernelGGL(k_check<K>, dim3(grid_for(max_count, 16, 256 * 16)), dim3(256), 0, s, R, D, V, first_global, ulist,
-                                       ucount, next_list, next_count));
-}
-
-__global__ void k_reset_tent(DictDev D, ResolveDev V, const uint32_t* list, const uint32_t* count) {
+    if (fused) DISPATCH_K(R.k, hipLaunchKernelGGL((k_check<K, true>), dim3(grid_for(max_count, 16, 256 * 16)), dim3(256), 0, s, R, D, V, first_global, ulist,
+                                                  ucount, next_list, next_count, round));
+    else DISPATCH_K(R.k, hipLaunchKernelGGL((k_check<K, false>), dim3(grid_for(max_count, 16, 256 * 16)), dim3(256), 0, s, R, D, V, first_global, ulist,
+                                            ucount, next_list, next_count, round));
+}
+
+__global__ void k_reset_tent(DictDev D, ResolveDev V, const uint32_t* list, const uint32_t* count, uint32_t round) {
     uint32_t n = *count;
     for (uint64_t e = blockIdx.x * (uint64_t)blockDim.x + threadIdx.x; e < n; e += (uint64_t)gridDim.x * blockDim.x)
-        *tent_ptr(D, V.cand_slot[list[e]]) = IDX_INF;
-}
-void launch_reset_tent(hipStream_t s, DictDev D, ResolveDev V, const uint32_t* list, const uint32_t* count, uint32_t max_count) {
+        *tent_ptr(D, V.cand_slot[list[e]], round) = IDX_INF;
+}
+void launch_reset_tent(hipStream_t s, DictDev D, ResolveDev V, const uint32_t* list, const uint32_t* count, uint32_t max_count, uint32_t round) {
     if (!max_count) return;
-    hipLaunchKernelGGL(k_reset_tent, dim3(grid_for(max_count, 256)), dim3(256), 0, s, D, V, list, count);
-}
-__global__ void k_propose(DictDev D, ResolveDev V, uint64_t first_global, const uint32_t* list, const uint32_t* count) {
+    hipLaunchKernelGGL(k_reset_tent, dim3(grid_for(max_count, 256)), dim3(256), 0, s, D, V, list, count, round);
+}
+__global__ void k_propose(DictDev D, ResolveDev V, uint64_t first_global, const uint32_t* list, const uint32_t* count, uint32_t round) {
     uint32_t n = *count;
     for (uint64_t e = blockIdx.x * (uint64_t)blockDim.x + threadIdx.x; e < n; e += (uint64_t)gridDim.x * blockDim.x) {
         uint32_t i = list[e];
-        atomicMin((unsigned long long*)tent_ptr(D, V.cand_slot[i]), (unsigned long long)(first_global + i));
+        tent_propose(D, V.cand_slot[i], round, first_global + i);
     }
 }
 void launch_propose(hipStream_t s, DictDev D, ResolveDev V, uint64_t first_global, const uint32_t* list,
-                    const uint32_t* count, uint32_t max_count) {
+                    const uint32_t* count, uint32_t max_count, uint32_t round) {
     if (!max_count) return;
-    hipLaunchKernelGGL(k_propose, dim3(grid_for(max_count, 256)), dim3(256), 0, s, D, V, first_global, list, count);
+    hipLaunchKernelGGL(k_propose, dim3(grid_for(max_count, 256)), dim3(256), 0, s, D, V, first_global, list, count, round);
 }
 
 template <typename K>
@@ -649,6 +682,7 @@
         const bool have = i < w1;
         const uint8_t st = have ? V.status[i] : (uint8_t)ST_NOANCHOR;
         const bool mine = st == ST_HIT || st == ST_HITNEW;
+        if (have && l == 0) V.ins_flag[i - w0] = st == ST_INSERTER ? 1u : 0u;
         const uint64_t g = first_global + i;
         const uint32_t limit = !mine ? 0u : (st == ST_HIT ? V.hit_pos[i] : R.len[i] - k + 1);
         const uint32_t* pk = R.packed + 2 * (mine ? R.slot_off[i] : 0);
@@ -687,14 +721,6 @@
     DISPATCH_K(R.k, hipLaunchKernelGGL(k_final_pos<K>, dim3(grid_for(w1 - w0, 16, 256 * 16)), dim3(256), 0, s, R, D, V, w0, w1, first_global));
 }
 
-__global__ void k_ins_flags(ResolveDev V, uint64_t w0, uint64_t w1) {
-    for (uint64_t i = w0 + blockIdx.x * (uint64_t)blockDim.x + threadIdx.x; i < w1; i += (uint64_t)gridDim.x * blockDim.x)
-        V.ins_flag[i - w0] = V.status[i] == ST_INSERTER ? 1u : 0u;
-}
-void launch_ins_flags(hipStream_t s, ResolveDev V, uint64_t w0, uint64_t w1) {
-    if (w1 <= w0) return;
-    hipLaunchKernelGGL(k_ins_flags, dim3(grid_for(w1 - w0, 256)), dim3(256), 0, s, V, w0, w1);
-}
 template <typename K>
 __global__ void k_assign_addr(DictDev D, ResolveDev V, uint64_t w0, uint64_t w1, const uint32_t* rank, uint64_t addr_base,
                               uint64_t* anchor_kmers) {
@@ -753,24 +779,18 @@
     if (w1 <= w0) return;
     hipLaunchKernelGGL(k_chain_compact, dim3(grid_for(w1 - w0, 256)), dim3(256), 0, s, V.status, w0, w1, rank, list);
 }
-__global__ void k_chain_reset(DictDev D, ResolveDev V, const uint32_t* list, uint32_t n) {
-    for (uint64_t e = blockIdx.x * (uint64_t)blockDim.x + threadIdx.x; e < n; e += (uint64_t)gridDim.x * blockDim.x)
-        *tent_ptr(D, V.cand_slot[list[e]]) = IDX_INF;
-}
-__global__ void k_chain_propose(DictDev D, ResolveDev V, uint64_t first_global, const uint32_t* list, uint32_t n) {
+__global__ void k_chain_propose(DictDev D, ResolveDev V, uint64_t first_global, const uint32_t* list, uint32_t n, uint32_t round) {
     for (uint64_t e = blockIdx.x * (uint64_t)blockDim.x + threadIdx.x; e < n; e += (uint64_t)gridDim.x * blockDim.x) {
         const uint32_t i = list[e];
-        atomicMin((unsigned long long*)tent_ptr(D, V.cand_slot[i]), (unsigned long long)(first_global + i));
-    }
-}
-void launch_chain_repropose(hipStream_t s, DictDev D, ResolveDev V, uint64_t first_global, const uint32_t* reset_list, uint32_t n_reset,
-                            const uint32_t* list, uint32_t n) {
-    if (n_reset) hipLaunchKernelGGL(k_chain_reset, dim3(grid_for(n_reset, 256)), dim3(256), 0, s, D, V, reset_list, n_reset);
-    if (n) hipLaunchKernelGGL(k_chain_propose, dim3(grid_for(n, 256)), dim3(256), 0, s, D, V, first_global, list, n);
+        tent_propose(D, V.cand_slot[i], round, first_global + i);
+    }
+}
+void launch_chain_repropose(hipStream_t s, DictDev D, ResolveDev V, uint64_t first_global, const uint32_t* list, uint32_t n, uint32_t round) {
+    if (n) hipLaunchKernelGGL(k_chain_propose, dim3(grid_for(n, 256)), dim3(256), 0, s, D, V, first_global, list, n, round);
 }
 
 template <typename K, bool FILL>
-__global__ void __launch_bounds__(256) k_chain_prep(ReadsDev R, DictDev D, ResolveDev V, uint64_t first_global, uint64_t w0,
+__global__ void __launch_bounds__(256) k_chain_prep(uint32_t round, ReadsDev R, DictDev D, ResolveDev V, uint64_t first_global, uint64_t w0,
                                                    const uint32_t* list, uint32_t n, uint32_t c0, const uint32_t* rank,
                                                    uint32_t* cnt, uint32_t* own, const uint64_t* gbase, uint32_t* ent,
                                                    const unsigned long long* om, const unsigned long long* late, unsigned long long* dep_out,
@@ -815,7 +835,7 @@
                     const uint32_t slot = dict_find(D, cn, fin);
                     if (slot != 0xFFFFFFFFu) {
                         f = fin < g;
-                        const uint64_t tv = *tent_ptr(D, slot);
+                        const uint64_t tv = tent_of(D, slot, round);
                         t = tv < g;
                         if (t) kid = rank[tv - first_global - w0] - c0;
                     }
@@ -849,16 +869,16 @@
             if (have && l == 0) { const bool dd = (cnt[e] >> 31) != 0; dep_out[e] = dd ? 0ull : dep & ((1ull << le) - 1ull); xdep_out[e] = dd ? 0ull : xdep; }
         } else if (have && l == 0) {
             cnt[e] = dead ? 0x80000000u : total;
-            own[e] = rank[*tent_ptr(D, V.cand_slot[i]) - first_global - w0] - c0;
-        }
-    }
-}
-void launch_chain_prep(hipStream_t s, bool fill, ReadsDev R, DictDev D, ResolveDev V, uint64_t first_global, uint64_t w0, const uint32_t* list,
+            own[e] = rank[tent_of(D, V.cand_slot[i], round) - first_global - w0] - c0;
+        }
+    }
+}
+void launch_chain_prep(hipStream_t s, bool fill, uint32_t round, ReadsDev R, DictDev D, ResolveDev V, uint64_t first_global, uint64_t w0, const uint32_t* list,
                        uint32_t n, uint32_t c0, const uint32_t* rank, uint32_t* cnt, uint32_t* own, const uint64_t* gbase, uint32_t* ent,
                        const unsigned long long* om, const unsigned long long* late, unsigned long long* dep, unsigned long long* xdep) {
     if (!n) return;
-    if (fill) DISPATCH_K(R.k, hipLaunchKernelGGL((k_chain_prep<K, true>), dim3(grid_for(n, 16, 256 * 16)), dim3(256), 0, s, R, D, V, first_global, w0, list, n, c0, rank, cnt, own, gbase, ent, om, late, dep, xdep));
-    else DISPATCH_K(R.k, hipLaunchKernelGGL((k_chain_prep<K, false>), dim3(grid_for(n, 16, 256 * 16)), dim3(256), 0, s, R, D, V, first_global, w0, list, n, c0, rank, cnt, own, gbase, ent, om, late, dep, xdep));
+    if (fill) DISPATCH_K(R.k, hipLaunchKernelGGL((k_chain_prep<K, true>), dim3(grid_for(n, 16, 256 * 16)), dim3(256), 0, s, round, R, D, V, first_global, w0, list, n, c0, rank, cnt, own, gbase, ent, om, late, dep, xdep));
+    else DISPATCH_K(R.k, hipLaunchKernelGGL((k_chain_prep<K, false>), dim3(grid_for(n, 16, 256 * 16)), dim3(256), 0, s, round, R, D, V, first_global, w0, list, n, c0, rank, cnt, own, gbase, ent, om, late, dep, xdep));
 }
 __global__ void __launch_bounds__(256) k_chain_tables(const uint32_t* cnt, const uint32_t* own, uint32_t n, uint64_t* rows, unsigned long long* om, unsigned long long* late) {
     __shared__ unsigned long long tab[4][64];
diff --git a/leon_amd/csrc/kernels.h b/leon_amd/csrc/kernels.h
--- a/leon_amd/csrc/kernels.h
+++ b/leon_amd/csrc/kernels.h
@@ -21,6 +21,8 @@
     uint64_t* slots;
     uint64_t* tent;
     uint64_t tstride;
+    uint64_t* tent1;
+    uint64_t t1stride;
     uint32_t* addr;
     uint64_t mask;
     unsigned long long* n_keys;
@@ -31,6 +33,8 @@
     uint32_t mm_m, mm_P, mm_c;
     int* err;
 };
+constexpr uint32_t TENT_IDX_BITS = 40, TENT_TAG_MAX = (1u << 24) - 1u;
+constexpr uint64_t TENT_IDX_MASK = (1ull << TENT_IDX_BITS) - 1ull;
 constexpr uint32_t WBITS_LOG2 = 23;
 inline void minimizer_geometry(uint32_t k, uint32_t& m, uint32_t& P, uint32_t& c) {
     if (k <= 16) { m = k; P = 1; c = 0; return; }
@@ -65,18 +69,21 @@
 void launch_dict_rehash(hipStream_t s, DictDev from, uint64_t from_cap, DictDev to, uint32_t k);
 void launch_lookup_cand(hipStream_t s, ReadsDev R, BloomDev B, const uint16_t* rv16, DictDev D, ResolveDev V,
                         uint64_t w0, uint64_t w1, uint64_t first_global, uint32_t* ulist, uint32_t* ucount,
+                        uint32_t round ,
                         unsigned long long* trace = nullptr ,
                         uint64_t* xres = nullptr ,
                         uint64_t xbase = 0, bool dry = false );
 void launch_lookup_apply(hipStream_t s, ReadsDev R, DictDev D, ResolveDev V, uint64_t w0, uint64_t w1, uint64_t s0, uint64_t s1,
-                         uint64_t first_global, const uint64_t* xres, uint32_t* ulist, uint32_t* ucount);
+                         uint64_t first_global, const uint64_t* xres, uint32_t* ulist, uint32_t* ucount, uint32_t round);
+void launch_window_clear(hipStream_t s, DictDev D, uint32_t* hist, uint32_t n_hist);
+void launch_tent_clear(hipStream_t s, DictDev D, uint64_t cap);
 void launch_check(hipStream_t s, ReadsDev R, DictDev D, ResolveDev V, uint64_t first_global,
-                  const uint32_t* ulist, const uint32_t* ucount, uint32_t max_count, uint32_t* next_list, uint32_t* next_count);
-void launch_reset_tent(hipStream_t s, DictDev D, ResolveDev V, const uint32_t* list, const uint32_t* count, uint32_t max_count);
+                  const uint32_t* ulist, const uint32_t* ucount, uint32_t max_count, uint32_t* next_list, uint32_t* next_count,
+                  uint32_t round, bool fused);
+void launch_reset_tent(hipStream_t s, DictDev D, ResolveDev V, const uint32_t* list, const uint32_t* count, uint32_t max_count, uint32_t round);
 void launch_propose(hipStream_t s, DictDev D, ResolveDev V, uint64_t first_global, const uint32_t* list,
-                    const uint32_t* count, uint32_t max_count);
+                    const uint32_t* count, uint32_t max_count, uint32_t round);
 void launch_final_pos(hipStream_t s, ReadsDev R, DictDev D, ResolveDev V, uint64_t w0, uint64_t w1, uint64_t first_global);
-void launch_ins_flags(hipStream_t s, ResolveDev V, uint64_t w0, uint64_t w1);
 void launch_assign_addr(hipStream_t s, DictDev D, ResolveDev V, uint64_t w0, uint64_t w1, const uint32_t* rank,
                         uint64_t addr_base, uint64_t* anchor_kmers, uint32_t k);
 constexpr uint32_t CHAIN_LOG2 = 19;
@@ -84,9 +91,8 @@
 constexpr uint32_t CHAIN_DEPTH = 3;
 void launch_chain_flags(hipStream_t s, ResolveDev V, uint64_t w0, uint64_t w1, uint32_t* flag);
 void launch_chain_compact(hipStream_t s, ResolveDev V, uint64_t w0, uint64_t w1, const uint32_t* rank, uint32_t* list);
-void launch_chain_repropose(hipStream_t s, DictDev D, ResolveDev V, uint64_t first_global, const uint32_t* reset_list, uint32_t n_reset,
-                            const uint32_t* list, uint32_t n);
-void launch_chain_prep(hipStream_t s, bool fill, ReadsDev R, DictDev D, ResolveDev V, uint64_t first_global, uint64_t w0, const uint32_t* list,
+void launch_chain_repropose(hipStream_t s, DictDev D, ResolveDev V, uint64_t first_global, const uint32_t* list, uint32_t n, uint32_t round);
+void launch_chain_prep(hipStream_t s, bool fill, uint32_t round, ReadsDev R, DictDev D, ResolveDev V, uint64_t first_global, uint64_t w0, const uint32_t* list,
                        uint32_t n, uint32_t c0, const uint32_t* rank, uint32_t* cnt, uint32_t* own, const uint64_t* gbase, uint32_t* ent,
                        const unsigned long long* om, const unsigned long long* late, unsigned long long* dep, unsigned long long* xdep);
 void launch_chain_tables(hipStream_t s, const uint32_t* cnt, const uint32_t* own, uint32_t n, uint64_t* rows ,
```

Result: no change. 18540 (-0.1%).
